# Krabbens/edge-diffusion-tts

Measured on AMD Instinct MI355X. Metric: mel-frames/sec (whole node), 4-step DDIM, hidden=160 L=4, B=256 T=512, higher is better.
Workload: dtype f32

## Files before the change

### edge-diffusion-tts_amd/csrc/edtts_device.h

```cpp
#pragma once
#include <hip/hip_runtime.h>
#include <stdint.h>
#include <type_traits>

#if !defined(EDTTS_EXPERIMENTS) && (                                                                                               \
    defined(EDTTS_ABLATE_QKVSTORES) || defined(EDTTS_ABLATE_KVLOADS) || defined(EDTTS_DIAG) || defined(EDTTS_KV2) ||                \
    defined(EDTTS_H_DMA) || defined(EDTTS_SPLITLOAD) || defined(EDTTS_STAMPS) || defined(EDTTS_DS_ABL) ||                           \
    defined(EDTTS_FAST_BUILD) || defined(EDTTS_W2) || defined(EDTTS_WAVELOG) || defined(EDTTS_PIN_MASK) || defined(EDTTS_HANDOVER) || defined(EDTTS_DS_BURST) || defined(EDTTS16_MFMA_SUM) || defined(EDTTS_DS_STAMPS) || defined(EDTTS_TAIL_RING2) || defined(EDTTS_RB) || defined(EDTTS_WMAX) ||        \
    defined(EDTTS_STAMP_THREAD) || defined(EDTTS_STAMP_HEAD) ||                                                                     \
    defined(EDTTS16_ABLATE_BARRIER) || defined(EDTTS16_ABLATE_DMA) || defined(EDTTS16_PHASES) || defined(EDTTS16_NF) ||             \
    defined(EDTTS16_W1) || defined(EDTTS16_QLDS) || defined(EDTTS16_KVDEPTH) || defined(EDTTS16_IMG) || defined(EDTTS16_HP) ||      \
    defined(EDTTS16_EVEN_STEPS))
#error "tuning / ablation / diagnostic / measured-and-rejected variant switches are scratch-only: add -DEDTTS_EXPERIMENTS"
#endif

#ifndef EDTTS_PIN_MASK
#define EDTTS_PIN_MASK 0x4
#endif
#ifndef EDTTS_W2
#define EDTTS_W2 0
#endif
#if EDTTS_W2
#define EDTTS_PIN_ACC(x) asm volatile("" : "+v"(x))
#else
// ... 57 lines not shown
}

template <int NT, int NF>
EDTTS_DEV void dma_tile_to_lds(const float* src, int ld, f4* lds_wave) {
  typedef __attribute__((address_space(3))) char* lds_char_t;
  const unsigned base = __builtin_amdgcn_readfirstlane((unsigned)(size_t)(lds_char_t)(char*)lds_wave);
#pragma unroll
  for (int nt = 0; nt < NT; ++nt)
#pragma unroll
    for (int ft = 0; ft < NF; ++ft) {
      const float* p = src + 16 * nt + (size_t)ft * 16 * ld;
      asm volatile("s_mov_b32 m0, %1\n\ts_nop 0\n\tglobal_load_lds_dwordx4 %0, off" ::"v"(p), "s"(base + (unsigned)(nt * NF + ft) * 1024u) : "m0", "memory");
    }
}

typedef unsigned u4v __attribute__((ext_vector_type(4)));
typedef unsigned u2v __attribute__((ext_vector_type(2)));
EDTTS_DEV __amdgpu_buffer_rsrc_t make_rsrc(const void* base) {
  return __builtin_amdgcn_make_buffer_rsrc(const_cast<void*>(base), 0, 0xFFFFFFFF, 0x00020000);
}
EDTTS_DEV f4 bufld4(__amdgpu_buffer_rsrc_t r, unsigned voff, unsigned soff) {
  return __builtin_bit_cast(f4, __builtin_amdgcn_raw_buffer_load_b128(r, voff, soff, 0));
}
EDTTS_DEV f2 bufld2(__amdgpu_buffer_rsrc_t r, unsigned voff, unsigned soff) {
  return __builtin_bit_cast(f2, __builtin_amdgcn_raw_buffer_load_b64(r, voff, soff, 0));
}

EDTTS_DEV float sqrt_rn(float x) { return (float)sqrt((double)x); }
EDTTS_DEV float div_rn(float a, float b) { return (float)((double)a / (double)b); }

EDTTS_DEV float group_sum(float v) {
  unsigned u = __float_as_uint(v);
  auto a = __builtin_amdgcn_permlane16_swap(u, u, false, false);
  v = __uint_as_float(a[0]) + __uint_as_float(a[1]);
  u = __float_as_uint(v);
  auto b = __builtin_amdgcn_permlane32_swap(u, u, false, false);
  return __uint_as_float(b[0]) + __uint_as_float(b[1]);
}
EDTTS_DEV float group_max(float v) {
  unsigned u = __float_as_uint(v);
  auto a = __builtin_amdgcn_permlane16_swap(u, u, false, false);
  v = fmaxf(__uint_as_float(a[0]), __uint_as_float(a[1]));
  u = __float_as_uint(v);
  auto b = __builtin_amdgcn_permlane32_swap(u, u, false, false);
  return fmaxf(__uint_as_float(b[0]), __uint_as_float(b[1]));
}
EDTTS_DEV float hsum(f4 v) { return (v[0] + v[1]) + (v[2] + v[3]); }
EDTTS_DEV float hmax(f4 v) { return fmaxf(fmaxf(v[0], v[1]), fmaxf(v[2], v[3])); }

#ifndef EDTTS_RB
#define EDTTS_RB 2
#endif
constexpr int kRefillBurst = EDTTS_RB;
template <int RN>
struct FragRing {
  static constexpr int RN_ = RN;
  __amdgpu_buffer_rsrc_t rs;
  unsigned soff;
  unsigned voff;
  f4 r[RN];
  EDTTS_DEV f4 frag(int i) const {
    return bufld4(rs, voff, soff + (unsigned)i * 1024u);
  }
  EDTTS_DEV void prime(const float* base, int lane) {
    rs = make_rsrc(base);
    soff = 0;
    voff = (unsigned)lane * 16u;
#pragma unroll
    for (int i = 0; i < RN; ++i) r[i] = frag(i);
  }
  EDTTS_DEV const f4& at(int i) const { return r[i % RN]; }
  EDTTS_DEV void refill(int lo, int hi) {
#pragma unroll
    for (int i = lo; i < hi; ++i) r[i % RN] = frag(i + RN);
    __builtin_amdgcn_sched_barrier(0);
  }
  template <int N>
  EDTTS_DEV void refill_after(int i) {
    constexpr int B = kRefillBurst < RN ? kRefillBurst : RN;
    if ((i + 1) % B == 0) refill(i + 1 - B, i + 1);
    else if (i == N - 1) refill(N - N % B, N);
  }
  EDTTS_DEV void advance(int n) { soff += (unsigned)n * 1024u; }
};

template <int KT, int RN, int NF>
EDTTS_DEV void gemm_phase(FragRing<RN>& ring, const f4 (&in)[KT][NF], f4 (&acc)[NF]) {
  static_assert(KT % RN == 0, "phase length must be a multiple of the ring size");
  constexpr bool SPLIT = NF < 4;
  f4 b[NF];
  if (SPLIT) {
#pragma unroll
    for (int ft = 0; ft < NF; ++ft) b[ft] = splat(0.f);
  }
#pragma unroll
  for (int kt = 0; kt < KT; ++kt) {
    const f4& a = ring.at(kt);
#pragma unroll
    for (int r = 0; r < 4; ++r)
#pragma unroll
      for (int ft = 0; ft < NF; ++ft) {
        if (SPLIT && (kt & 1)) b[ft] = EDTTS_MFMA(a[r], in[kt][ft][r], b[ft]);
        else acc[ft] = EDTTS_MFMA(a[r], in[kt][ft][r], acc[ft]);
      }
    ring.template refill_after<KT>(kt);
  }
  if (SPLIT) {
#pragma unroll
    for (int ft = 0; ft < NF; ++ft) acc[ft] += b[ft];
  }
  ring.advance(KT);
}

template <int KT, int RN, int NF>
EDTTS_DEV void gemm_phase_pair(FragRing<RN>& ring, const f4 (&in)[KT][NF], f4 (&a)[NF], f4 (&b)[NF]) {
  static_assert((2 * KT) % RN == 0, "phase length must be a multiple of the ring size");
#pragma unroll
  for (int kt = 0; kt < KT; ++kt) {
    const f4& fa = ring.at(2 * kt);
    const f4& fb = ring.at(2 * kt + 1);
#pragma unroll
    for (int r = 0; r < 4; ++r) {
#pragma unroll
      for (int ft = 0; ft < NF; ++ft) a[ft] = EDTTS_MFMA(fa[r], in[kt][ft][r], a[ft]);
#pragma unroll
      for (int ft = 0; ft < NF; ++ft) b[ft] = EDTTS_MFMA(fb[r], in[kt][ft][r], b[ft]);
    }
    ring.template refill_after<2 * KT>(2 * kt);
    ring.template refill_after<2 * KT>(2 * kt + 1);
  }
  ring.advance(2 * KT);
}

template <int NT, int RN, int NF, int NR = 4>
EDTTS_DEV void ktile_phase(FragRing<RN>& ring, const f4 (&in)[NF], f4 (&acc)[NT][NF]) {
  static_assert(NT % RN == 0, "phase length must be a multiple of the ring size");
  constexpr int STEP = NF < 4 ? 2 : 1;
#pragma unroll
  for (int nt = 0; nt < NT; nt += STEP) {
#pragma unroll
    for (int r = 0; r < NR; ++r)
#pragma unroll
      for (int u = 0; u < STEP; ++u)
        if (nt + u < NT) {
          const f4& fa = ring.at(nt + u);
#pragma unroll
          for (int ft = 0; ft < NF; ++ft) acc[nt + u][ft] = EDTTS_MFMA(fa[r], in[ft][r], acc[nt + u][ft]);
        }
#pragma unroll
    for (int u = 0; u < STEP; ++u)
      if (nt + u < NT) ring.template refill_after<NT>(nt + u);
  }
  ring.advance(NT);
}

template <int NT, int NF>
EDTTS_DEV void rms_norm_tile(const f4 (&x)[NT][NF], const float* __restrict__ w, const float* __restrict__ mod, int g,
                             f4 (&y)[NT][NF]) {
  constexpr int N = NT * 16;
  float rs[NF];
#pragma unroll
  for (int ft = 0; ft < NF; ++ft) {
    float ss = 0.f;
#pragma unroll
    for (int t = 0; t < NT; ++t) ss += hsum(x[t][ft] * x[t][ft]);
    rs[ft] = rsqrtf(group_sum(ss) * (1.0f / N) + 1e-6f);
  }
#pragma unroll
  for (int t = 0; t < NT; ++t) {
    const f4 wv = ldg4(w + 16 * t + 4 * g);
    f4 sc = splat(1.f), sh = splat(0.f);
    if (mod != nullptr) {
      sc = ldg4(mod + 16 * t + 4 * g);
      sh = ldg4(mod + N + 16 * t + 4 * g);
    }
#pragma unroll
    for (int ft = 0; ft < NF; ++ft) {
      f4 a = x[t][ft] * rs[ft] * wv;
      if (mod != nullptr) a = a * sc + sh;
      y[t][ft] = a;
    }
  }
}

template <int NT, int NF>
EDTTS_DEV void layer_norm_tile(const f4 (&x)[NT][NF], const float* __restrict__ w, const float* __restrict__ b, int g,
                               f4 (&y)[NT][NF]) {
  constexpr int N = NT * 16;
  float mu[NF], rs[NF];
#pragma unroll
  for (int ft = 0; ft < NF; ++ft) {
    float s = 0.f;
#pragma unroll
    for (int t = 0; t < NT; ++t) s += hsum(x[t][ft]);
// ... 419 lines not shown
#endif
      };
      const int cd = q.cdiag;
      auto chunk_of = [&](int st) { return st >= nchunk ? nchunk - 1 : (st == 0 ? cd : (st <= cd ? st - 1 : st)); };
#if EDTTS_KV2
      step(No{}, cd, chunk_of(2), KA, VA, hd);
      for (int st = 1; st < nchunk; st += 2) {
        step(Yes{}, chunk_of(st), chunk_of(st + 2), KB, VB, hd);
        if (st + 1 < nchunk) step(Yes{}, chunk_of(st + 1), chunk_of(st + 3), KA, VA, hd);
      }
#else
#ifndef EDTTS_HANDOVER
#define EDTTS_HANDOVER 1
#endif
      constexpr bool HANDOVER = EDTTS_HANDOVER && NHALF == 1;
      const bool more = HANDOVER && hd + hstep < C::HEADS;
      auto req_head = [&](int st) { return (more && st == nchunk - 1) ? hd + hstep : hd; };
      auto req_chunk = [&](int st) { return (more && st == nchunk - 1) ? cd : chunk_of(st + 1); };
      step(No{}, cd, req_chunk(0), KA, VA, req_head(0));
      for (int st = 1; st < nchunk; ++st) step(Yes{}, chunk_of(st), req_chunk(st), KA, VA, req_head(st));
#endif
#pragma unroll
      for (int ft = 0; ft < QT; ++ft) {
        const float lt = group_sum(hsum(lvec[ft]));
        const float inv = lt > 0.f ? 1.0f / lt : 0.f;
#pragma unroll
        for (int dt = 0; dt < DT; ++dt) O[dt][QT * hf + ft] *= inv;
      }
    }
#ifdef EDTTS_STAMPS
    if (hd == STAMP_SEL_HEAD(stamp_sel)) STAMPX(stamps, sidx++, stamp_sel);
#endif
    if (hd + hstep < C::HEADS) {
      if constexpr (EDTTS_HANDOVER && NHALF == 1) {
        load_q(hd + hstep, 0);
        __builtin_amdgcn_sched_barrier(0);
      } else {
        prefetch(geo[0], hd + hstep, 0);
      }
    }
    if constexpr (OMODE != O_FUSED) {
      char* ob = obuf + hd * C::OHEAD_BYTES;
#pragma unroll
      for (int dt = 0; dt < DT; ++dt)
#pragma unroll
        for (int ft = 0; ft < NF; ++ft) {
          if (DREM && dt == DT - 1) reinterpret_cast<f2*>(ob + DFULL * NF * 1024 + ft * 512)[lane] = f2{O[dt][ft][0], O[dt][ft][1]};
          else reinterpret_cast<f4*>(ob + (dt * NF + ft) * 1024)[lane] = O[dt][ft];
        }
    } else {
#pragma unroll
      for (int dt = 0; dt < DT; ++dt) {
        if (DREM && dt == DT - 1) ktile_phase<C::HT, WStream<C>::RN_, NF, 2>(ring, O[dt], h);
        else ktile_phase<C::HT>(ring, O[dt], h);
      }
    }
#ifdef EDTTS_STAMPS
    if (hd == STAMP_SEL_HEAD(stamp_sel)) STAMPX(stamps, sidx++, stamp_sel);
#endif
  }
  if constexpr (OMODE == O_DEFER) {
    before_project();
    for (int hd = 0; hd < C::HEADS; ++hd) {
      const char* ob = obuf + hd * C::OHEAD_BYTES;
#pragma unroll
      for (int dt = 0; dt < DT; ++dt) {
        f4 in[NF];
#pragma unroll
        for (int ft = 0; ft < NF; ++ft) {
          if (DREM && dt == DT - 1) {
            const f2 t = reinterpret_cast<const f2*>(ob + DFULL * NF * 1024 + ft * 512)[lane];
            in[ft] = f4{t[0], t[1], 0.f, 0.f};
          } else {
            in[ft] = reinterpret_cast<const f4*>(ob + (dt * NF + ft) * 1024)[lane];
          }
        }
        if (DREM && dt == DT - 1) ktile_phase<C::HT, WStream<C>::RN_, NF, 2>(ring, in, h);
        else ktile_phase<C::HT>(ring, in, h);
      }
    }
  }
}

EDTTS_DEV void ddim_elem(float x, float e, float s1m, float sab, float sabp, float cdir, float& x0, float& xp) {
#pragma clang fp contract(off)
  float t1 = s1m * e;
  float t2 = x - t1;
  float v = div_rn(t2, sab);
  v = fminf(fmaxf(v, -3.0f), 3.0f);
  x0 = v;
  float t3 = sabp * v;
  float t4 = cdir * e;
  xp = t3 + t4;
}
struct DdimCoef {
  float s1m, sab, sabp, cdir, sigma;
};
EDTTS_DEV DdimCoef ddim_coef(float ab, float abp, float eta) {
#pragma clang fp contract(off)
  DdimCoef c;
  c.s1m = sqrt_rn(1.0f - ab);
  c.sab = sqrt_rn(ab);
  float r1 = div_rn(1.0f - abp, 1.0f - ab);
  float r2 = 1.0f - div_rn(ab, abp);
  float pr = r1 * r2;
  c.sigma = eta * sqrt_rn(pr);
  float s2 = c.sigma * c.sigma;
  float in = 1.0f - abp;
  in = in - s2;
  c.cdir = sqrt_rn(in);
  c.sabp = sqrt_rn(abp);
  return c;
}
EDTTS_DEV float add_mul_rn(float p, float s, float n) {
#pragma clang fp contract(off)
  float t = s * n;
  return p + t;
}

struct DdpmCoef {
  float coef1, coef2, sd;
};
EDTTS_DEV DdpmCoef ddpm_coef(float al, float ab, float be, float var, bool nonzero) {
#pragma clang fp contract(off)
  DdpmCoef c;
  c.coef1 = div_rn(1.0f, sqrt_rn(al));
  float om = 1.0f - ab;
  c.coef2 = div_rn(be, sqrt_rn(om));
  c.sd = (nonzero ? 1.0f : 0.0f) * sqrt_rn(var);
  return c;
}
EDTTS_DEV float ddpm_elem(float x, float e, float n, DdpmCoef c) {
#pragma clang fp contract(off)
  float t1 = c.coef2 * e;
  float t2 = x - t1;
  float mean = c.coef1 * t2;
  float t3 = c.sd * n;
  return mean + t3;
}

struct LmsCoef {
  int mode;
  float p0, p1, c0, c1, rinv, cB, cC;
};
EDTTS_DEV void lms_elem(float x, float out, float h_new, float h_old, const LmsCoef& k, float& x0, float& xn) {
#pragma clang fp contract(off)
  float a = k.p0 * x;
  float b = k.p1 * out;
  float v = a + b;
  v = fminf(fmaxf(v, -3.0f), 3.0f);
  x0 = v;
  float t0 = k.c0 * x;
  float t1 = k.c1 * v;
  float acc = t0 + t1;
  if (k.mode == 2) {
    float d = v - h_new;
    float d1 = k.rinv * d;
    float t2 = k.cB * d1;
    t2 = t2 * 0.5f;
    acc = acc + t2;
  } else if (k.mode == 3) {
    float d1 = v - h_old;
    float two = 2.0f * h_old;
    float d2 = v - two;
    d2 = d2 + h_new;
    float t2 = k.cB * d1;
    t2 = t2 * 0.5f;
    float t3 = k.cC * d2;
    t3 = t3 / 6.0f;
    acc = acc + t2;
    acc = acc + t3;
// ... 114 lines not shown
```

### edge-diffusion-tts_amd/csrc/edtts_generic.h

```cpp
#pragma once

namespace edtts_gen {

enum { EPI_BIAS = 0, EPI_PE = 1, EPI_RESID = 2, EPI_SWIGLU = 3 };

struct GemmArgs {
  const float* X;
  const float* W;
  const float* bias;
  float* Y;
  const float* pe;
  int M, N, K, ldx, ldy, T;
  int vec_x, vec_w, vec_y;
  DropArgs dr;
};
constexpr int kGBM = 64, kGBN = 64, kGBK = 16, kGLd = kGBK + 1;

template <int EPI, bool DROP = false>
__global__ __launch_bounds__(256) void k_gen_gemm(GemmArgs a) {
  __shared__ float xs[kGBM][kGLd];
  __shared__ float ws[kGBN][kGLd];
  const int tid = threadIdx.x, lane = tid & 63, w = tid >> 6, fq = lane & 15, g = lane >> 4;
  const int m0 = blockIdx.x * kGBM;
  const int n0 = blockIdx.y * (EPI == EPI_SWIGLU ? kGBN / 2 : kGBN);
// ... 249 lines not shown
      const f4 dm = drop_attn_keys4(a.dr, (unsigned)(b * gridDim.y + hd), qi, j0 + 4 * g, (lo & 3) == 0);
#pragma unroll
      for (int r = 0; r < 4; ++r) p[r] *= dm[r];
    }
#pragma unroll
    for (int s = 0; s < 4; ++s) {
      const int key = j0 + 4 * g + s;
      const float* vrow = vb + (size_t)(key < hi ? key : 0) * a.ldkv;
#pragma unroll
      for (int t = 0; t < DT; ++t) {
        const int d = 16 * t + fq;
        const float va = (key < hi && d < a.DH) ? vrow[d] : 0.f;
        acc[t] = EDTTS_MFMA(va, p[s], acc[t]);
      }
    }
  }
  if (!qok) return;
  if (a.lse != nullptr && g == 0) a.lse[((size_t)b * gridDim.y + hd) * a.Tq + qi] = m + log2f(l);
  const float inv = 1.0f / l;
  float* orow = a.o + (size_t)(b * a.Tq + qi) * a.ldo + hd * a.DH;
#pragma unroll
  for (int t = 0; t < DT; ++t)
#pragma unroll
    for (int r = 0; r < 4; ++r) {
      const int d = 16 * t + 4 * g + r;
      if (d < a.DH) orow[d] = acc[t][r] * inv;
    }
}

__global__ __launch_bounds__(256) void k_gen_embed(const int64_t* sem_idx, const float* tok, const float* cpe, float* ctx, int rows, int S,
                                                   int H, int n_tok, unsigned* err, const int64_t* s_len) {
  const size_t n = (size_t)rows * H;
  for (size_t i = (size_t)blockIdx.x * blockDim.x + threadIdx.x; i < n; i += (size_t)gridDim.x * blockDim.x) {
    const size_t row = i / H;
    const int c = (int)(i - row * H);
    long tk = (s_len && (int)(row % S) >= utt_len_lane(s_len, (int)(row / S), S)) ? 0 : (long)sem_idx[row];
    if (tk < 0 || tk >= n_tok) {
      if (c == 0) atomicOr(err, (unsigned)EDTTS_IDX_SEM);
      tk = tk < 0 ? 0 : n_tok - 1;
    }
    ctx[i] = tok[(size_t)tk * H + c] + cpe[(size_t)(row % S) * H + c];
  }
}

template <int TAIL>
EDTTS_DEV void tail_elem(const KArgs& a, size_t idx, float e) {
  if (TAIL == TAIL_LMS) {
    const float hn = a.lms.mode >= 2 ? a.h_new[idx] : 0.f, ho = a.lms.mode >= 3 ? a.h_old[idx] : 0.f;
    float v0, vn;
    lms_elem(a.x[idx], e, hn, ho, a.lms, v0, vn);
    a.x0_hist[idx] = v0;
    if (a.x0_all) a.x0_all[idx] = v0;
    a.x_prev[idx] = vn;
  } else if (TAIL == TAIL_VLMS) {
    const float v = a.v_uncond ? cfg_combine(e, a.v_uncond[idx], a.vp.cfg) : e;
    const float hn = a.lms.mode >= 2 ? a.h_new[idx] : 0.f, ho = a.lms.mode >= 3 ? a.h_old[idx] : 0.f;
    float v0, vn;
    lms_elem(a.x[idx], v, hn, ho, a.lms, v0, vn);
    a.x0_hist[idx] = v0;
    if (a.x0_all) a.x0_all[idx] = v0;
    if (a.known != nullptr) {
      const size_t row = (size_t)a.T * a.inj_mel, b = idx / row, r = idx - b * row, per = (size_t)a.inj_frames * a.inj_mel;
      if (r < per) {
        const size_t ki = b * per + r;
        vn = a.known[ki];
        if (a.p_coef2 != 0.f) {
          const float nz = a.noise ? a.noise[ki]
                                   : (a.seeds ? philox_normal4(a.seeds[b], a.step, r >> 2)[(int)(r & 3)] : philox_normal4(a.seed, a.step, ki >> 2)[(int)(ki & 3)]);
          vn = qsample_elem(vn, a.p_coef1, nz, a.p_coef2);
        }
      }
    }
    a.x_prev[idx] = vn;
  } else if (TAIL == TAIL_VPRED) {
    const float v = a.v_uncond ? cfg_combine(e, a.v_uncond[idx], a.vp.cfg) : e;
    a.x_prev[idx] = vpred_elem(a.x[idx], v, a.vp);
  } else if (TAIL == TAIL_DDPM) {
    const unsigned long long ge = a.philox_base + idx;
    const float nz = a.noise ? a.noise[idx] : philox_normal4(a.seed, a.step, ge >> 2)[(int)(ge & 3)];
    const DdpmCoef cf{a.p_coef1, a.p_coef2, a.p_sd};
    a.x_prev[idx] = ddpm_elem(a.x[idx], e, nz, cf);
  } else {
    float v0, vp;
    ddim_elem(a.x[idx], e, a.c_s1m, a.c_sab, a.c_sabp, a.c_dir, v0, vp);
    a.x0[idx] = v0;
    a.x_prev[idx] = vp;
  }
}
template <int TAIL>
EDTTS_DEV void tail_zero_elem(const KArgs& a, size_t idx) {
  if (TAIL == TAIL_LMS || TAIL == TAIL_VLMS) {
    a.x0_hist[idx] = 0.f;
    if (a.x0_all) a.x0_all[idx] = 0.f;
  } else if (TAIL == TAIL_DDIM) {
    a.x0[idx] = 0.f;
  }
  a.x_prev[idx] = 0.f;
}
EDTTS_DEV bool past_len(const int64_t* t_len, bool dbl, size_t idx, int T, int MEL) {
  if (t_len == nullptr) return false;
  const size_t row = idx / MEL;
  return (int)(row % T) >= utt_len_lane(t_len, (int)(row / T), T, dbl);
}
template <int TAIL>
__global__ __launch_bounds__(256) void k_gen_tail(KArgs a, const float* eps, size_t n, int vec, int MEL) {
  const size_t stride = (size_t)gridDim.x * blockDim.x;
  if (vec) {
    for (size_t i = (size_t)blockIdx.x * blockDim.x + threadIdx.x; i < n / 4; i += stride) {
      if constexpr (TAIL == TAIL_VLMS) {
        const size_t row = 4 * i / MEL;
        const int f = (int)(row % a.T);
        const int Tb = a.t_len ? utt_len_of(a.t_len[row / a.T], a.T, a.t_dbl) : a.T;
        tail_store<TAIL>(a, f, Tb, 4 * i, ldg4(eps + 4 * i));
        continue;
      }
      if (past_len(a.t_len, a.t_dbl, 4 * i, a.T, MEL)) tail_zero<TAIL>(a, 4 * i);
      else tail_apply<TAIL>(a, 4 * i, ldg4(eps + 4 * i));
    }
  } else {
    for (size_t i = (size_t)blockIdx.x * blockDim.x + threadIdx.x; i < n; i += stride) {
      if (past_len(a.t_len, a.t_dbl, i, a.T, MEL)) tail_zero_elem<TAIL>(a, i);
      else tail_elem<TAIL>(a, i, eps[i]);
    }
  }
}
__global__ __launch_bounds__(256) void k_gen_zero_past(float* y, const int64_t* t_len, int dbl, size_t n, int T, int MEL) {
  for (size_t i = (size_t)blockIdx.x * blockDim.x + threadIdx.x; i < n; i += (size_t)gridDim.x * blockDim.x)
    if (past_len(t_len, dbl, i, T, MEL)) y[i] = 0.f;
}

}

struct GenericLauncher {
  static int set_attrs() { return EDTTS_OK; }

  static bool al16(const void* p) { return ((uintptr_t)p & 15) == 0; }
  static unsigned grid_1d(size_t n) { const size_t nb = (n + 255) / 256; return (unsigned)(nb > 4096 ? 4096 : (nb < 1 ? 1 : nb)); }
  template <int EPI>
  static int gemm(hipStream_t st, const float* X, int ldx, const float* W, const float* bias, float* Y, int ldy, int M, int N, int K,
                  const float* pe = nullptr, int T = 1, const edtts::DropArgs* dr = nullptr) {
    using namespace edtts_gen;
    GemmArgs a;
    a.X = X; a.W = W; a.bias = bias; a.Y = Y; a.pe = pe; a.M = M; a.N = N; a.K = K; a.ldx = ldx; a.ldy = ldy; a.T = T;
    a.vec_x = (K % 4 == 0) && (ldx % 4 == 0) && al16(X);
    a.vec_w = (K % 4 == 0) && al16(W);
    a.vec_y = (ldy % 4 == 0) && al16(Y);
    const int nb = EPI == EPI_SWIGLU ? kGBN / 2 : kGBN;
    a.dr = dr ? *dr : edtts::DropArgs{};
    const dim3 grid((M + kGBM - 1) / kGBM, (N + nb - 1) / nb);
    if constexpr (EPI == EPI_SWIGLU || EPI == EPI_RESID) {
      if (dr) {
        hipLaunchKernelGGL((k_gen_gemm<EPI, true>), grid, dim3(256), 0, st, a);
        LAUNCH_CHECK("k_gen_gemm");
        return EDTTS_OK;
      }
    }
    hipLaunchKernelGGL(k_gen_gemm<EPI>, grid, dim3(256), 0, st, a);
    LAUNCH_CHECK("k_gen_gemm");
    return EDTTS_OK;
  }
  template <int MODE>
  static int norm(hipStream_t st, const float* x, float* y, int rows, int W, const float* w, const float* b, float eps,
                  const float* mod = nullptr, int rows_per_b = 1, int mod_bstride = 0) {
    edtts_gen::NormArgs a{x, y, w, b, mod, rows, W, W, rows_per_b, mod_bstride, eps};
    hipLaunchKernelGGL(edtts_gen::k_gen_norm<MODE>, dim3((rows + 3) / 4), dim3(256), 0, st, a);
    LAUNCH_CHECK("k_gen_norm");
    return EDTTS_OK;
// ... 121 lines not shown
```

### edge-diffusion-tts_amd/csrc/edtts_kernels.hip

```cpp
#include <hip/hip_runtime.h>
#include <math.h>
#include <stdarg.h>
#include <stdlib.h>
#include <stdio.h>
#include <string.h>

#include "../../include/edtts.h"
#include "edtts_device.h"

using namespace edtts;

static thread_local char g_err[512] = "";
static int fail(int code, const char* fmt, ...) __attribute__((format(printf, 2, 3)));
static int fail(int code, const char* fmt, ...) {
  va_list ap;
  va_start(ap, fmt);
  vsnprintf(g_err, sizeof(g_err), fmt, ap);
  va_end(ap);
  return code;
}
#define HIP_TRY(expr)                                                                                   \
  do {                                                                                                  \
    hipError_t e_ = (expr);                                                                             \
    if (e_ != hipSuccess) return fail(EDTTS_ERR_HIP, "%s failed: %s", #expr, hipGetErrorString(e_));    \
// ... 331 lines not shown
  float* e = sm;
  float* u = sm + a.H;
  const int row = blockIdx.x, tid = threadIdx.x, H = a.H, half = H / 2;
  const float tf = a.use_host ? (float)a.t_host[row] : (float)a.t[row];
  for (int j = tid; j < H; j += blockDim.x) {
    const float arg = tf * a.freqs[j < half ? j : j - half];
    e[j] = j < half ? sinf(arg) : cosf(arg);
  }
  __syncthreads();
  for (int n = tid; n < H; n += blockDim.x) {
    float acc = a.t1b[n];
#pragma unroll 8
    for (int k = 0; k < H; ++k) acc = fmaf(e[k], a.t1T[(size_t)k * H + n], acc);
    u[n] = 0.5f * acc * (1.0f + erff(acc * 0.70710678118654752440f));
  }
  __syncthreads();
  long sidx = -1;
  if (a.use_host ? a.host_has_step : (a.step_idx != nullptr)) {
    sidx = a.use_host ? (long)a.step_host[row] : (long)a.step_idx[row];
    if (sidx < 0 || sidx >= a.n_step) {
      if (tid == 0) atomicOr(a.err, (unsigned)EDTTS_IDX_STEP);
      sidx = sidx < 0 ? 0 : a.n_step - 1;
    }
  }
  for (int n = tid; n < H; n += blockDim.x) {
    float acc = a.t3b[n];
#pragma unroll 8
    for (int k = 0; k < H; ++k) acc = fmaf(u[k], a.t3T[(size_t)k * H + n], acc);
    if (sidx >= 0) acc += a.step[(size_t)sidx * H + n];
    a.tcond[(size_t)row * H + n] = acc;
  }
}
__global__ __launch_bounds__(256) void k_cond_ada(CondArgs a) {
  extern __shared__ float sm[];
  const int row = blockIdx.x, lw = blockIdx.y, l = lw >> 1, which = lw & 1, H = a.H;
  for (int k = threadIdx.x; k < H; k += blockDim.x) sm[k] = a.tcond[(size_t)row * H + k];
  __syncthreads();
  const float* WT = a.blob + (which ? a.ada3T[l] : a.ada1T[l]);
  const float* bb = a.blob + (which ? a.ada3b[l] : a.ada1b[l]);
  float* out = a.cond + (((size_t)row * a.L + l) * 2 + which) * 2 * H;
  for (int n = blockIdx.z * blockDim.x + threadIdx.x; n < 2 * H; n += gridDim.z * blockDim.x) {
    float acc = bb[n];
#pragma unroll 8
    for (int k = 0; k < H; ++k) acc = fmaf(sm[k], WT[(size_t)k * 2 * H + n], acc);
    out[n] = n < H ? 1.0f + acc : acc;
  }
}

struct KArgs {
  int B, T, Tp, S, Sp, window, max_pos, max_cpos, n_tok, SD, L;
  const float* x;
  float* h;
  const float *q, *k, *vT;
  float *q_out, *k_out, *vT_out;
  float *kc, *vcT;
  const float* known;
  const unsigned long long* seeds;
  int inj_frames, inj_mel;
  const int64_t* sem_idx;
  const float* sem_feat;
  const float* cond;
  int cond_bstride;
  int layer;
  int ffn_tiles;
  int diag_skip;
  unsigned long long* stamps;
  const float *tok, *semp, *semp_b, *cpe, *inp, *inp_b, *pe;
  const float *n1w, *proj_b, *n2w, *n3w, *up_b, *down_b, *fnw, *fnb, *outp_b;
  const float* stream;
  float *eps, *x_prev, *x0;
  float c_s1m, c_sab, c_sabp, c_dir;
  float p_coef1, p_coef2, p_sd;
  const float* noise;
  unsigned long long seed;
  unsigned long long philox_base;
  unsigned step;
  LmsCoef lms;
  VpredCoef vp;
  const float* v_uncond;
  const float *h_new, *h_old;
  float *x0_hist, *x0_all;
  const int64_t *t_len, *s_len;
  int t_dbl;
};

EDTTS_DEV int utt_len_of(int64_t v, int full, bool dbl) {
  const int hi = dbl ? full >> 1 : full;
  const int n = v < 1 ? 1 : (v > hi ? hi : (int)v);
  return dbl ? 2 * n : n;
}
EDTTS_DEV int utt_len(const int64_t* len, int b, int full, bool dbl = false) {
  if (len == nullptr) return full;
  return utt_len_of(len[__builtin_amdgcn_readfirstlane(b)], full, dbl);
}
EDTTS_DEV int utt_len_lane(const int64_t* len, int b, int full, bool dbl = false) {
  return len == nullptr ? full : utt_len_of(len[b], full, dbl);
}
EDTTS_DEV int live_end(int n) { return (n + 31) & ~31; }

EDTTS_DEV int remap_block(int bid, int nblk) {
  const int q = nblk >> 3, r = nblk & 7, xcd = bid & 7, idx = bid >> 3;
  const int base = xcd < r ? xcd * (q + 1) : r * (q + 1) + (xcd - r) * q;
  return base + idx;
}

struct TileId {
  int b, m0;
  bool valid;
};
EDTTS_DEV TileId wave_tile(int B, int Tp, int waves_per_block, int wave_frames) {
  const int wave = __builtin_amdgcn_readfirstlane(threadIdx.x >> 6);
  const int tpu = Tp / wave_frames;
  int w = remap_block(blockIdx.x, gridDim.x) * waves_per_block + wave;
  TileId t;
  t.valid = w < B * tpu;
  w = t.valid ? w : B * tpu - 1;
  t.b = w / tpu;
  t.m0 = (w - t.b * tpu) * wave_frames;
  return t;
}

#ifndef EDTTS_TAIL_RING2
#define EDTTS_TAIL_RING2 1
#endif
template <class C>
EDTTS_DEV void qkv_tail(WStream<C>& ring0, const f4 (&hn)[C::HT][C::NF], const KArgs& a, int b, int m0, int lane) {
  constexpr int NF = C::NF;
  static_assert(C::HT % 2 == 0, "hidden must be a multiple of 32 (n-tile pairs)");
#if EDTTS_TAIL_RING2
  constexpr int RN0 = WStream<C>::RN_;
  static_assert((2 * C::HT) % (2 * RN0) == 0, "a pair phase must be a whole number of turns of the doubled ring");
  FragRing<2 * RN0> ring;
  ring.rs = ring0.rs; ring.soff = ring0.soff; ring.voff = ring0.voff;
#pragma unroll
  for (int i = 0; i < RN0; ++i) ring.r[i] = ring0.at(i);
#pragma unroll
  for (int i = RN0; i < 2 * RN0; ++i) ring.r[i] = ring.frag(i);
  __builtin_amdgcn_sched_barrier(0);
#else
  WStream<C>& ring = ring0;
#endif
  const int fq = lane & 15, g = lane >> 4;
  const size_t rowbase = (size_t)b * a.Tp + m0 + fq;
#pragma unroll
  for (int which = 0; which < 3; ++which) {
    for (int nt = 0; nt < C::HT; nt += 2) {
      f4 acc[2][NF];
#pragma unroll
      for (int ft = 0; ft < NF; ++ft) acc[0][ft] = acc[1][ft] = splat(0.f);
      gemm_phase_pair<C::HT>(ring, hn, acc[0], acc[1]);
#ifdef EDTTS_ABLATE_QKVSTORES
      if (a.T > 0) continue;
#endif
#pragma unroll
      for (int u = 0; u < 2; ++u) {
        if (which < 2) {
          float* dst = (which == 0 ? a.q_out : a.k_out) + rowbase * C::H + 16 * (nt + u) + 4 * g;
#pragma unroll
          for (int ft = 0; ft < NF; ++ft) {
            __builtin_nontemporal_store(acc[u][ft], reinterpret_cast<f4*>(dst + (size_t)ft * 16 * C::H));
          }
        } else {
          float* dst = a.vT_out + ((size_t)b * C::VR + 16 * (nt + u) + 4 * g) * a.Tp + m0 + fq;
#pragma unroll
          for (int r = 0; r < 4; ++r)
#pragma unroll
            for (int ft = 0; ft < NF; ++ft) {
              __builtin_nontemporal_store(acc[u][ft][r], dst + (size_t)r * a.Tp + 16 * ft);
            }
        }
      }
    }
  }
}

template <class C>
__global__ __launch_bounds__(C::THREADS) void k_prologue(KArgs a) {
  constexpr int NF = C::NF;
  const TileId tl = wave_tile(a.B, a.Tp, C::WAVES, C::WF);
  if (!tl.valid) return;
  const int lane = threadIdx.x & 63, fq = lane & 15, g = lane >> 4;
  const int b = tl.b, m0 = tl.m0;
  const int Tb = utt_len(a.t_len, b, a.T, a.t_dbl);
  if (m0 >= live_end(Tb)) return;
  WStream<C> ring;
  ring.prime(a.stream, lane);
  f4 xin[C::MT][NF];
#pragma unroll
  for (int ft = 0; ft < NF; ++ft) {
    const int f = m0 + 16 * ft + fq;
#pragma unroll
    for (int t = 0; t < C::MT; ++t)
      xin[t][ft] = f < Tb ? ldg4(a.x + ((size_t)b * a.T + f) * C::MEL + 16 * t + 4 * g) : splat(0.f);
  }
  f4 h[C::HT][NF];
#pragma unroll
  for (int nt = 0; nt < C::HT; ++nt) {
    const f4 bias = ldg4(a.inp_b + 16 * nt + 4 * g);
#pragma unroll
    for (int ft = 0; ft < NF; ++ft) h[nt][ft] = bias;
  }
  {
    constexpr int N = C::HT * C::MT;
    static_assert(N % WStream<C>::RN_ == 0 && C::HT % 2 == 0, "in_proj must be a whole number of ring turns");
#pragma unroll
    for (int nt = 0; nt < C::HT; nt += 2)
#pragma unroll
      for (int kt = 0; kt < C::MT; ++kt) {
        const int i = nt * C::MT + 2 * kt;
        const f4& fa = ring.at(i);
        const f4& fb = ring.at(i + 1);
#pragma unroll
        for (int r = 0; r < 4; ++r) {
#pragma unroll
          for (int ft = 0; ft < NF; ++ft) h[nt][ft] = EDTTS_MFMA(fa[r], xin[kt][ft][r], h[nt][ft]);
#pragma unroll
          for (int ft = 0; ft < NF; ++ft) h[nt + 1][ft] = EDTTS_MFMA(fb[r], xin[kt][ft][r], h[nt + 1][ft]);
        }
        ring.template refill_after<N>(i);
        ring.template refill_after<N>(i + 1);
      }
    ring.advance(N);
  }
#pragma unroll
  for (int ft = 0; ft < NF; ++ft) {
    int f = m0 + 16 * ft + fq;
    f = f < a.max_pos ? f : a.max_pos - 1;
#pragma unroll
    for (int nt = 0; nt < C::HT; ++nt) h[nt][ft] += ldg4(a.pe + (size_t)f * C::H + 16 * nt + 4 * g);
  }
  {
    float* hp = a.h + ((size_t)b * a.Tp + m0 + fq) * C::H + 4 * g;
#pragma unroll
    for (int nt = 0; nt < C::HT; ++nt)
#pragma unroll
      for (int ft = 0; ft < NF; ++ft) stg4(hp + 16 * nt + (size_t)ft * 16 * C::H, h[nt][ft]);
  }
  f4 hn[C::HT][NF];
  const float* mod = a.cond + (size_t)b * a.cond_bstride;
  rms_norm_tile<C::HT, NF>(h, a.n1w, mod, g, hn);
  qkv_tail<C>(ring, hn, a, b, m0, lane);
}

enum { TAIL_QKV = 0, TAIL_EPS = 1, TAIL_DDIM = 2, TAIL_DDPM = 3, TAIL_LMS = 4, TAIL_VPRED = 5, TAIL_VLMS = 6 };

template <int TAIL>
EDTTS_DEV void tail_apply(const KArgs& a, size_t idx, f4 ev, bool blend = false) {
  if (TAIL == TAIL_EPS) {
    stg4(a.eps + idx, ev);
  } else if (TAIL == TAIL_LMS) {
    const f4 xv = ldg4(a.x + idx);
    f4 hn = splat(0.f), ho = splat(0.f);
    if (a.lms.mode >= 2) hn = ldg4(a.h_new + idx);
    if (a.lms.mode >= 3) ho = ldg4(a.h_old + idx);
    f4 x0, xn;
#pragma unroll
    for (int r = 0; r < 4; ++r) {
      float v0, vn;
      lms_elem(xv[r], ev[r], hn[r], ho[r], a.lms, v0, vn);
      x0[r] = v0;
      xn[r] = vn;
    }
    stg4(a.x0_hist + idx, x0);
    if (a.x0_all) stg4(a.x0_all + idx, x0);
    stg4(a.x_prev + idx, xn);
  } else if (TAIL == TAIL_VLMS) {
    const bool guided = a.v_uncond != nullptr;
    const f4 xv = ldg4(a.x + idx);
    const f4 vu = ldg4((guided ? a.v_uncond : a.x) + idx);
    f4 hn = splat(0.f), ho = splat(0.f);
    if (a.lms.mode >= 2) hn = ldg4(a.h_new + idx);
    if (a.lms.mode >= 3) ho = ldg4(a.h_old + idx);
    f4 x0, xn;
#pragma unroll
    for (int r = 0; r < 4; ++r) {
      const float v = guided ? cfg_combine(ev[r], vu[r], a.vp.cfg) : ev[r];
      float v0, vn;
      lms_elem(xv[r], v, hn[r], ho[r], a.lms, v0, vn);
      x0[r] = v0;
      xn[r] = vn;
    }
    stg4(a.x0_hist + idx, x0);
    if (a.x0_all) stg4(a.x0_all + idx, x0);
    if (!blend) stg4(a.x_prev + idx, xn);
  } else if (TAIL == TAIL_VPRED) {
    const bool guided = a.v_uncond != nullptr;
    const f4 xv = ldg4(a.x + idx);
    const f4 vu = ldg4((guided ? a.v_uncond : a.x) + idx);
    f4 v, xn;
#pragma unroll
    for (int r = 0; r < 4; ++r) v[r] = guided ? cfg_combine(ev[r], vu[r], a.vp.cfg) : ev[r];
#pragma unroll
    for (int r = 0; r < 4; ++r) xn[r] = vpred_elem(xv[r], v[r], a.vp);
    stg4(a.x_prev + idx, xn);
  } else if (TAIL == TAIL_DDPM) {
    const f4 xv = ldg4(a.x + idx);
    const f4 nz = a.noise ? ldg4(a.noise + idx) : philox_normal4(a.seed, a.step, (a.philox_base + idx) >> 2);
    const DdpmCoef cf{a.p_coef1, a.p_coef2, a.p_sd};
    f4 xp;
#pragma unroll
    for (int r = 0; r < 4; ++r) xp[r] = ddpm_elem(xv[r], ev[r], nz[r], cf);
    stg4(a.x_prev + idx, xp);
  } else {
    const f4 xv = ldg4(a.x + idx);
    f4 x0, xp;
#pragma unroll
    for (int r = 0; r < 4; ++r) {
      float v0, vp;
      ddim_elem(xv[r], ev[r], a.c_s1m, a.c_sab, a.c_sabp, a.c_dir, v0, vp);
      x0[r] = v0;
      xp[r] = vp;
    }
    stg4(a.x0 + idx, x0);
    stg4(a.x_prev + idx, xp);
  }
}
template <int TAIL>
EDTTS_DEV void tail_zero(const KArgs& a, size_t idx) {
  const f4 z = splat(0.f);
  if (TAIL == TAIL_EPS) {
    stg4(a.eps + idx, z);
  } else if (TAIL == TAIL_LMS || TAIL == TAIL_VLMS) {
    stg4(a.x0_hist + idx, z);
    if (a.x0_all) stg4(a.x0_all + idx, z);
    stg4(a.x_prev + idx, z);
  } else if (TAIL == TAIL_DDIM) {
    stg4(a.x0 + idx, z);
    stg4(a.x_prev + idx, z);
  } else {
    stg4(a.x_prev + idx, z);
  }
}
EDTTS_DEV void vlms_blend(const KArgs& a, size_t idx) {
  const size_t row = (size_t)a.T * a.inj_mel, b = idx / row, r = idx - b * row;
  const size_t ki = b * ((size_t)a.inj_frames * a.inj_mel) + r;
  const f4 kv = ldg4(a.known + ki);
  f4 o = kv;
  if (a.p_coef2 != 0.f) {
    const unsigned long long sd = a.seeds ? a.seeds[b] : a.seed;
    const f4 nz = a.noise ? ldg4(a.noise + ki) : philox_normal4(sd, a.step, (a.seeds ? r : ki) >> 2);
#pragma unroll
    for (int e = 0; e < 4; ++e) o[e] = qsample_elem(kv[e], a.p_coef1, nz[e], a.p_coef2);
  }
  stg4(a.x_prev + idx, o);
}
template <int TAIL>
EDTTS_DEV void tail_store(const KArgs& a, int f, int Tb, size_t idx, f4 ev) {
  if constexpr (TAIL == TAIL_VLMS) {
    const bool blend = a.known != nullptr && f < Tb && f < a.inj_frames;
    if (f < Tb) tail_apply<TAIL>(a, idx, ev, blend);
    else tail_zero<TAIL>(a, idx);
    if (blend) vlms_blend(a, idx);
  } else {
    if (f < Tb) tail_apply<TAIL>(a, idx, ev);
    else tail_zero<TAIL>(a, idx);
  }
}

struct QGlobal {
  __amdgpu_buffer_rsrc_t rs;
  unsigned v4, v2;
  int H;
  EDTTS_DEV QGlobal(const float* row_m0, int H_, int fq, int g) : rs(make_rsrc(row_m0)), v4((unsigned)(fq * H_ + 4 * g) * 4u), v2((unsigned)(fq * H_ + 2 * g) * 4u), H(H_) {}
  EDTTS_DEV f4 q4(int ft, int col) const { return bufld4(rs, v4, (unsigned)(ft * 16 * H + col) * 4u); }
  EDTTS_DEV f2 q2(int ft, int col) const { return bufld2(rs, v2, (unsigned)(ft * 16 * H + col) * 4u); }
};
struct QLds {
  const float* b4;
  const float* b2;
  int ld;
  EDTTS_DEV QLds(const float* tile, int ld_, int fq, int g) : b4(tile + fq * ld_ + 4 * g), b2(tile + fq * ld_ + 2 * g), ld(ld_) {}
  EDTTS_DEV f4 q4(int ft, int col) const { return *reinterpret_cast<const f4*>(b4 + ft * 16 * ld + col); }
  EDTTS_DEV f2 q2(int ft, int col) const { return *reinterpret_cast<const f2*>(b2 + ft * 16 * ld + col); }
};

template <class C, int TAIL>
EDTTS_DEV void layer_tile(const KArgs& a, float* smem, int wave, int lane, int b, int m0, int Tb, int Sb) {
  constexpr int NF = C::NF;
  const int fq = lane & 15, g = lane >> 4;
  f4* const stash = reinterpret_cast<f4*>(smem) + (size_t)wave * C::HT * NF * 64 + lane;
  char* const obuf = reinterpret_cast<char*>(smem) + (size_t)wave * C::HT * NF * 1024;
  static_assert(!C::DEFER || C::HEADS * C::OHEAD_BYTES <= C::HT * NF * 1024, "attention outputs must fit the wave's parking place");
  constexpr int QLDS = C::H;
  float* qtile = smem + (size_t)C::WAVES * C::HT * NF * 256 + (size_t)wave * C::WF * QLDS;
  const size_t rowbase = (size_t)b * a.Tp + m0 + fq;

  STAMPX(a.stamps, 0, a.diag_skip);
  WStream<C> ring;
  ring.prime(a.stream, lane);

  f4 h[C::HT][NF];
  float* const hp = a.h + rowbase * C::H + 4 * g;
  auto park_h = [&]() {
#pragma unroll
    for (int nt = 0; nt < C::HT; ++nt)
#pragma unroll
      for (int ft = 0; ft < NF; ++ft) stash[(nt * NF + ft) * 64] = h[nt][ft];
  };
  auto add_parked_h = [&]() {
#pragma unroll
    for (int nt = 0; nt < C::HT; ++nt)
#pragma unroll
      for (int ft = 0; ft < NF; ++ft) h[nt][ft] += stash[(nt * NF + ft) * 64];
  };
#ifdef EDTTS_DIAG
#define DIAG_ON(bit) (!(a.diag_skip & (bit)))
#else
#define DIAG_ON(bit) true
#endif
  {
#ifndef EDTTS_H_DMA
#define EDTTS_H_DMA 0
#endif
#if EDTTS_H_DMA
    dma_tile_to_lds<C::HT, NF>(hp, C::H, reinterpret_cast<f4*>(smem) + (size_t)wave * C::HT * NF * 64);
#else
    if constexpr (!C::DEFER) {
#pragma unroll
      for (int nt = 0; nt < C::HT; ++nt)
#pragma unroll
        for (int ft = 0; ft < NF; ++ft) h[nt][ft] = ldg4(hp + 16 * nt + (size_t)ft * 16 * C::H);
      park_h();
    }
#endif
    auto init_proj_bias = [&]() {
#pragma unroll
      for (int nt = 0; nt < C::HT; ++nt) {
        const f4 pb = ldg4(a.proj_b + 16 * nt + 4 * g);
#pragma unroll
        for (int ft = 0; ft < NF; ++ft) h[nt][ft] = pb;
      }
    };
    if constexpr (!C::DEFER) init_proj_bias();
    if (DIAG_ON(1)) {
      QGlobal ql(a.q + ((size_t)b * a.Tp + m0) * C::H, C::H, fq, g);
      attention_fused<C, true, C::DEFER ? O_DEFER : O_FUSED>(ql, a.k + (size_t)b * a.Tp * C::H, a.vT + (size_t)b * C::VR * a.Tp, a.Tp, Tb, a.window, m0,
                               lane, ring, h, obuf, init_proj_bias, a.stamps ? a.stamps + 8 : nullptr, a.diag_skip);
    }
    if constexpr (C::DEFER) {
// ... 18 lines not shown
      } else {
        park_h();
      }
      for (int nt = 0; nt < C::HT; nt += 2) {
        f4 acc[2][NF];
#pragma unroll
        for (int ft = 0; ft < NF; ++ft) acc[0][ft] = acc[1][ft] = splat(0.f);
        gemm_phase_pair<C::HT>(ring, hn, acc[0], acc[1]);
#pragma unroll
        for (int u = 0; u < 2; ++u)
#pragma unroll
          for (int ft = 0; ft < NF; ++ft) {
            if (C::Q_IN_LDS) stg4(qtile + (16 * ft + fq) * QLDS + 16 * (nt + u) + 4 * g, acc[u][ft]);
            else stg4(const_cast<float*>(a.q) + (rowbase + 16 * ft) * C::H + 16 * (nt + u) + 4 * g, acc[u][ft]);
          }
      }
    }
    STAMPX(a.stamps, 2, a.diag_skip);
    auto zero_h = [&]() {
#pragma unroll
      for (int nt = 0; nt < C::HT; ++nt)
#pragma unroll
        for (int ft = 0; ft < NF; ++ft) h[nt][ft] = splat(0.f);
    };
    if constexpr (!C::DEFER) zero_h();
    if constexpr (C::Q_IN_LDS) {
      QLds ql(qtile, QLDS, fq, g);
      attention_fused<C, false, C::DEFER ? O_DEFER : O_FUSED>(ql, a.kc + (size_t)b * a.Sp * C::H, a.vcT + (size_t)b * C::VR * a.Sp, a.Sp, Sb, -1, m0, lane,
                                ring, h, obuf, zero_h, a.stamps ? a.stamps + 40 : nullptr, a.diag_skip);
    } else {
      QGlobal ql(a.q + ((size_t)b * a.Tp + m0) * C::H, C::H, fq, g);
      attention_fused<C, false, C::DEFER ? O_DEFER : O_FUSED>(ql, a.kc + (size_t)b * a.Sp * C::H, a.vcT + (size_t)b * C::VR * a.Sp, a.Sp, Sb, -1, m0, lane,
                                ring, h, obuf, zero_h);
    }
    if constexpr (C::DEFER) {
#pragma unroll
      for (int nt = 0; nt < C::HT; ++nt)
#pragma unroll
        for (int ft = 0; ft < NF; ++ft) h[nt][ft] += ldg4(hp + 16 * nt + (size_t)ft * 16 * C::H);
    } else {
      add_parked_h();
    }
    STAMPX(a.stamps, 3, a.diag_skip);
  }
  if (DIAG_ON(4)) {
    f4 hn[C::HT][NF];
    const float* mod = a.cond + (size_t)b * a.cond_bstride + ((size_t)a.layer * 2 + 1) * 2 * C::H;
    rms_norm_tile<C::HT, NF>(h, a.n3w, mod, g, hn);
    park_h();
#pragma unroll
    for (int nt = 0; nt < C::HT; ++nt) {
      const f4 db = ldg4(a.down_b + 16 * nt + 4 * g);
#pragma unroll
      for (int ft = 0; ft < NF; ++ft) h[nt][ft] = db;
    }
    for (int j = 0; j < a.ffn_tiles; ++j) {
      const f4 vb = ldg4(a.up_b + 32 * j + 4 * g), gb = ldg4(a.up_b + 32 * j + 16 + 4 * g);
      f4 v[NF], gt[NF], act[NF];
#pragma unroll
      for (int ft = 0; ft < NF; ++ft) v[ft] = gt[ft] = splat(0.f);
      gemm_phase_pair<C::HT>(ring, hn, v, gt);
      __builtin_amdgcn_sched_barrier(0);
#pragma unroll
      for (int ft = 0; ft < NF; ++ft) act[ft] = swiglu_tile(v[ft], gt[ft], vb, gb);
      __builtin_amdgcn_sched_barrier(0);
      ktile_phase<C::HT>(ring, act, h);
    }
    add_parked_h();
    STAMPX(a.stamps, 4, a.diag_skip);
  }
  if (!DIAG_ON(8)) return;
  if (TAIL == TAIL_QKV) {
    {
      float* hp = a.h + rowbase * C::H + 4 * g;
#pragma unroll
      for (int nt = 0; nt < C::HT; ++nt)
#pragma unroll
        for (int ft = 0; ft < NF; ++ft) stg4(hp + 16 * nt + (size_t)ft * 16 * C::H, h[nt][ft]);
    }
    const float* mod = a.cond + (size_t)b * a.cond_bstride + ((size_t)(a.layer + 1) * 2) * 2 * C::H;
    rms_norm_tile<C::HT, NF>(h, a.n1w, mod, g, h);
    qkv_tail<C>(ring, h, a, b, m0, lane);
  } else {
    f4 hn[C::HT][NF];
    layer_norm_tile<C::HT, NF>(h, a.fnw, a.fnb, g, hn);
#pragma unroll
    for (int nt = 0; nt < C::MT; ++nt) {
      const f4 ob = ldg4(a.outp_b + 16 * nt + 4 * g);
      f4 e[NF];
#pragma unroll
      for (int ft = 0; ft < NF; ++ft) e[ft] = splat(0.f);
      gemm_phase<C::HT>(ring, hn, e);
#pragma unroll
      for (int ft = 0; ft < NF; ++ft) {
        const int f = m0 + 16 * ft + fq;
        if (f >= a.T) continue;
        const size_t idx = ((size_t)b * a.T + f) * C::MEL + 16 * nt + 4 * g;
        tail_store<TAIL>(a, f, Tb, idx, e[ft] + ob);
      }
    }
  }
  STAMPX(a.stamps, 5, a.diag_skip);
#ifdef EDTTS_STAMPS
  asm volatile("s_waitcnt vmcnt(0)" ::: "memory");
#endif
  STAMPX(a.stamps, 6, a.diag_skip);
}

template <class C, int TAIL>
EDTTS_DEV void tail_zero_tile(const KArgs& a, int b, int m0, int lane) {
  const int fq = lane & 15, g = lane >> 4;
#pragma unroll
  for (int ft = 0; ft < C::NF; ++ft) {
    const int f = m0 + 16 * ft + fq;
    if (f >= a.T) continue;
#pragma unroll
    for (int nt = 0; nt < C::MT; ++nt) tail_zero<TAIL>(a, ((size_t)b * a.T + f) * C::MEL + 16 * nt + 4 * g);
  }
}
template <class C, int TAIL>
__global__ __launch_bounds__(C::THREADS, C::DEFER ? 2 : 1) void k_layer(KArgs a) {
  extern __shared__ __attribute__((aligned(16))) float smem[];
  const int lane = threadIdx.x & 63;
  const int wave = __builtin_amdgcn_readfirstlane(threadIdx.x >> 6);
  const TileId tl = wave_tile(a.B, a.Tp, C::WAVES, C::WF);
  if (!tl.valid) return;
  const int Tb = utt_len(a.t_len, tl.b, a.T, a.t_dbl);
  if (tl.m0 >= live_end(Tb)) {
    if constexpr (TAIL != TAIL_QKV) tail_zero_tile<C, TAIL>(a, tl.b, tl.m0, lane);
    return;
  }
  const int Sb = utt_len(a.s_len, tl.b, a.S);
#ifdef EDTTS_WAVELOG
  const unsigned long long wl_r0 = __builtin_amdgcn_s_memrealtime(), wl_c0 = __builtin_amdgcn_s_memtime();
#endif
  layer_tile<C, TAIL>(a, smem, wave, lane, tl.b, tl.m0, Tb, Sb);
#ifdef EDTTS_WAVELOG
  if (a.stamps && lane == 0) {
    asm volatile("s_waitcnt vmcnt(0)" ::: "memory");
    unsigned long long* p = a.stamps + 6 * ((size_t)a.diag_skip + (size_t)tl.b * (a.Tp / C::WF) + tl.m0 / C::WF);
    p[0] = wl_r0; p[1] = wl_c0; p[2] = __builtin_amdgcn_s_memrealtime(); p[3] = __builtin_amdgcn_s_memtime();
    p[4] = __builtin_amdgcn_s_getreg((31 << 11) | 4);
    p[5] = __builtin_amdgcn_s_getreg((31 << 11) | 20);
  }
#endif
}

#include "edtts_coop.h"
#include "edtts_bf16.h"
#include "edtts_melpost.h"

struct CtxArgs {
  int B, S, Sp, L, SD, n_tok, max_cpos;
  const int64_t* sem_idx;
  const float* sem_feat;
  const float *tok, *semp, *semp_b, *cpe;
  const float* blob;
  unsigned kvd[kMaxLayers], kvn[kMaxLayers], kvu[kMaxLayers];
  float *kc, *vcT;
  unsigned* err;
  const float* stream16;
  const int64_t* s_len;
};
template <class C>
__global__ __launch_bounds__(64 * kCtxWaves) void k_ctx(CtxArgs a) {
  const TileId tl = wave_tile(a.B, a.Sp, kCtxWaves, 32);
  if (!tl.valid) return;
  const int lane = threadIdx.x & 63, fq = lane & 15, g = lane >> 4;
  const int b = tl.b, m0 = tl.m0;
  const int Sb = utt_len(a.s_len, b, a.S);
  if (m0 >= live_end(Sb)) return;
  f4 ctx[C::HT][2];
  if (a.sem_feat != nullptr) {
    const int KT = a.SD / 16;
    const f4* wp = reinterpret_cast<const f4*>(a.semp) + lane;
#pragma unroll
    for (int nt = 0; nt < C::HT; ++nt) ctx[nt][0] = ctx[nt][1] = ldg4(a.semp_b + 16 * nt + 4 * g);
    for (int kt = 0; kt < KT; ++kt) {
      f4 xin[2];
#pragma unroll
      for (int ft = 0; ft < 2; ++ft) {
        const int s = m0 + 16 * ft + fq;
        xin[ft] = s < Sb ? ldg4(a.sem_feat + ((size_t)b * a.S + s) * a.SD + 16 * kt + 4 * g) : splat(0.f);
      }
#pragma unroll
      for (int nt = 0; nt < C::HT; ++nt) {
        const f4 w = wp[(nt * KT + kt) * 64];
#pragma unroll
        for (int r = 0; r < 4; ++r) {
          ctx[nt][0] = EDTTS_MFMA(w[r], xin[0][r], ctx[nt][0]);
          ctx[nt][1] = EDTTS_MFMA(w[r], xin[1][r], ctx[nt][1]);
        }
      }
    }
  } else {
#pragma unroll
    for (int ft = 0; ft < 2; ++ft) {
      const int s = m0 + 16 * ft + fq;
      long tk = s < Sb ? (long)a.sem_idx[(size_t)b * a.S + s] : 0;
      if (tk < 0 || tk >= a.n_tok) {
        atomicOr(a.err, (unsigned)EDTTS_IDX_SEM);
        tk = tk < 0 ? 0 : a.n_tok - 1;
      }
      const float* row = a.tok + (size_t)tk * C::H + 4 * g;
#pragma unroll
      for (int nt = 0; nt < C::HT; ++nt) ctx[nt][ft] = ldg4(row + 16 * nt);
    }
  }
#pragma unroll
  for (int ft = 0; ft < 2; ++ft) {
    int s = m0 + 16 * ft + fq;
    s = s < a.max_cpos ? s : a.max_cpos - 1;
// ... 119 lines not shown
#pragma unroll
      for (int ft = 0; ft < 2; ++ft) {
        float ss = 0.f;
#pragma unroll
        for (int t = 0; t < RT; ++t) ss += hsum(c[t][ft] * c[t][ft]);
        rs[ft] = rsqrtf(group_sum(ss) * (1.0f / C::R) + 1e-6f);
      }
      const float* w = a.blob + a.kvn[l];
#pragma unroll
      for (int kt = 0; kt < RK; ++kt) {
        const f4 w0 = ldg4(w + 32 * kt + 4 * g), w1 = ldg4(w + 32 * kt + 16 + 4 * g);
#pragma unroll
        for (int ft = 0; ft < 2; ++ft) cn[kt][ft] = pack8(c[2 * kt][ft] * rs[ft] * w0, c[2 * kt + 1][ft] * rs[ft] * w1);
      }
    }
    __bf16* const kimg = reinterpret_cast<__bf16*>(a.kc) + ((size_t)l * a.B + b) * a.Sp * C::H;
    __bf16* const vimg = reinterpret_cast<__bf16*>(a.vcT) + ((size_t)l * a.B + b) * a.Sp * C::H;
    for (int ph = 0; ph < 2 * C::HEADS / PPP; ++ph) {
      const lds_cf4_t fr = phase_base(ring.acquire());
      f4 fg[C::PH];
#pragma unroll
      for (int i = 0; i < C::PH; ++i) fg[i] = fr[i * 64];
      __builtin_amdgcn_sched_barrier(0);
      const bool isv = ph >= C::HEADS / PPP;
#pragma unroll
      for (int pp = 0; pp < PPP; ++pp) {
        const int head = (isv ? ph - C::HEADS / PPP : ph) * PPP + pp;
        f4 acc[2][2] = {{splat(0.f), splat(0.f)}, {splat(0.f), splat(0.f)}};
        if (!isv) {
#pragma unroll
          for (int kt = 0; kt < RK; ++kt)
#pragma unroll
            for (int u = 0; u < 2; ++u)
#pragma unroll
              for (int ft = 0; ft < 2; ++ft)
                acc[u][ft] = EDTTS_MFMA16(as_bf8(fg[pp * 2 * RK + 2 * kt + u]), cn[kt][ft], acc[u][ft]);
          __bf16* d = kimg + head * hstride + (size_t)(m0 >> 4) * 512 + fq * 32 + 8 * g;
          if (valid)
#pragma unroll
            for (int ft = 0; ft < 2; ++ft) *reinterpret_cast<f4*>(d + ft * 512) = as_f4(pack8(acc[0][ft], acc[1][ft]));
        } else {
#pragma unroll
          for (int kt = 0; kt < RK; ++kt)
#pragma unroll
            for (int u = 0; u < 2; ++u)
#pragma unroll
              for (int ft = 0; ft < 2; ++ft)
                acc[u][ft] = EDTTS_MFMA16(cn[kt][ft], as_bf8(fg[pp * 2 * RK + 2 * kt + u]), acc[u][ft]);
          __bf16* d = vimg + head * hstride + (size_t)(m0 >> 5) * 1024 + fq * 32 + 8 * g;
          if (valid)
#pragma unroll
            for (int u = 0; u < 2; ++u) *reinterpret_cast<f4*>(d + u * 512) = as_f4(pack8(acc[u][0], acc[u][1]));
        }
      }
    }
  }
  ring.drain();
}


struct StepArgs {
  const float *alphas, *alpha_bar, *betas, *post_var;
  int n_table;
  const float *x, *eps, *noise;
  const int64_t *t, *t_prev;
  size_t n_per_batch;
  float eta;
  float *x_prev, *x0;
  int vec4;
};
static int step_vec4(size_t n_per_batch, std::initializer_list<const void*> ptrs) {
  uintptr_t m = 0;
  for (const void* p : ptrs) m |= (uintptr_t)p;
  return (n_per_batch & 3) == 0 && (m & 15) == 0;
}
EDTTS_DEV long clamp_idx(long v, int n) { return v < 0 ? 0 : (v >= n ? n - 1 : v); }

__global__ __launch_bounds__(256) void k_ddim(StepArgs a) {
  const int b = blockIdx.y;
  const float ab = a.alpha_bar[clamp_idx((long)a.t[b], a.n_table)];
  const long tp = (long)a.t_prev[b];
  const float abp = tp >= 0 ? a.alpha_bar[clamp_idx(tp, a.n_table)] : 1.0f;
  const DdimCoef cf = ddim_coef(ab, abp, a.eta);
  const float s1m = cf.s1m, sab = cf.sab, sabp = cf.sabp, cdir = cf.cdir, sigma = cf.sigma;
  const size_t base = (size_t)b * a.n_per_batch;
  const size_t n4 = a.vec4 ? a.n_per_batch >> 2 : 0;
  for (size_t i = (size_t)blockIdx.x * blockDim.x + threadIdx.x; i < n4; i += (size_t)gridDim.x * blockDim.x) {
    const size_t o = base + 4 * i;
    const f4 xv = ldg4(a.x + o), e = ldg4(a.eps + o);
    f4 nz = splat(0.f);
    if (a.noise) nz = ldg4(a.noise + o);
    f4 x0, xp;
#pragma unroll
    for (int r = 0; r < 4; ++r) {
      float v, p;
      ddim_elem(xv[r], e[r], s1m, sab, sabp, cdir, v, p);
      if (a.noise) p = add_mul_rn(p, sigma, nz[r]);
      x0[r] = v;
      xp[r] = p;
    }
    stg4(a.x0 + o, x0);
    stg4(a.x_prev + o, xp);
  }
  for (size_t i = (n4 << 2) + (size_t)blockIdx.x * blockDim.x + threadIdx.x; i < a.n_per_batch; i += (size_t)gridDim.x * blockDim.x) {
    const size_t o = base + i;
    float v, p;
    ddim_elem(a.x[o], a.eps[o], s1m, sab, sabp, cdir, v, p);
    if (a.noise) p = add_mul_rn(p, sigma, a.noise[o]);
    a.x0[o] = v;
    a.x_prev[o] = p;
  }
}

__global__ __launch_bounds__(256) void k_ddpm(StepArgs a) {
  const int b = blockIdx.y;
  const long tt = clamp_idx((long)a.t[b], a.n_table);
  const float al = a.alphas[tt], ab = a.alpha_bar[tt], be = a.betas[tt];
  const DdpmCoef cf = ddpm_coef(al, ab, be, a.post_var[tt], (long)a.t[b] > 0);
  const size_t base = (size_t)b * a.n_per_batch;
  const size_t n4 = a.vec4 ? a.n_per_batch >> 2 : 0;
  for (size_t i = (size_t)blockIdx.x * blockDim.x + threadIdx.x; i < n4; i += (size_t)gridDim.x * blockDim.x) {
    const size_t o = base + 4 * i;
    const f4 xv = ldg4(a.x + o), e = ldg4(a.eps + o), nz = ldg4(a.noise + o);
    f4 xp;
#pragma unroll
    for (int r = 0; r < 4; ++r) xp[r] = ddpm_elem(xv[r], e[r], nz[r], cf);
    stg4(a.x_prev + o, xp);
  }
  for (size_t i = (n4 << 2) + (size_t)blockIdx.x * blockDim.x + threadIdx.x; i < a.n_per_batch; i += (size_t)gridDim.x * blockDim.x) {
    const size_t o = base + i;
    a.x_prev[o] = ddpm_elem(a.x[o], a.eps[o], a.noise[o], cf);
  }
}

constexpr int kDsTileT = 64, kDsLd = kDsTileT + 4;
__global__ __launch_bounds__(256) void k_dsconv_pw(const float* __restrict__ x, const float* __restrict__ dw, const float* __restrict__ pw,
                                                   const float* __restrict__ pb, int B, int Ci, int Co, int Tin, int T, int ks, int stride,
                                                   float* __restrict__ z) {
  extern __shared__ float dsm[];
  const int b = blockIdx.y, t0 = blockIdx.x * kDsTileT, pad = ks / 2;
  const int Cip = (Ci + 15) & ~15;
  for (int i = threadIdx.x; i < Cip * kDsTileT; i += blockDim.x) {
    const int ci = i / kDsTileT, tl = i % kDsTileT, tt = t0 + tl;
    float acc = 0.f;
    if (ci < Ci && tt < T) {
      const float* xr = x + ((size_t)b * Ci + ci) * Tin;
      for (int j = 0; j < ks; ++j) {
        const int ts = tt * stride + j - pad;
        if (ts >= 0 && ts < Tin) acc = fmaf(xr[ts], dw[ci * ks + j], acc);
      }
    }
    dsm[ci * kDsLd + tl] = acc;
  }
  __syncthreads();
  const int lane = threadIdx.x & 63, wave = threadIdx.x >> 6, fq = lane & 15, g = lane >> 4;
  const int tl = 16 * wave + fq, tt = t0 + tl;
  const int KT = Cip >> 4;
  constexpr int kMaxKT = 16;
  f4 bt[kMaxKT];
#pragma unroll
  for (int kt = 0; kt < kMaxKT; ++kt) {
    if (kt < KT) {
#pragma unroll
      for (int r = 0; r < 4; ++r) bt[kt][r] = dsm[(16 * kt + 4 * g + r) * kDsLd + tl];
    }
  }
  for (int co0 = 0; co0 < Co; co0 += 16) {
    const int row = co0 + fq;
    const float* wr = pw + (size_t)(row < Co ? row : Co - 1) * Ci;
    f4 acc = splat(0.f);
#pragma unroll
    for (int kt = 0; kt < kMaxKT; ++kt) {
      if (kt < KT) {
        const int c0 = 16 * kt + 4 * g;
        f4 a;
        if (row < Co && c0 + 3 < Ci && (Ci & 3) == 0) a = ldg4(wr + c0);
        else {
#pragma unroll
          for (int r = 0; r < 4; ++r) a[r] = (row < Co && c0 + r < Ci) ? wr[c0 + r] : 0.f;
        }
#pragma unroll
        for (int r = 0; r < 4; ++r) acc = EDTTS_MFMA(a[r], bt[kt][r], acc);
      }
    }
    if (tt < T) {
#pragma unroll
      for (int r = 0; r < 4; ++r) {
        const int co = co0 + 4 * g + r;
        if (co < Co) z[((size_t)b * Co + co) * T + tt] = acc[r] + pb[co];
      }
// ... 625 lines not shown
      }
    });
    DS_SUB(t, 7);
    dsg_static_for<0, t + 1>([&](auto uc) {
      constexpr int tt = decltype(uc)::value;
      if constexpr ((CPG * ((16 * tt + 15) / CPG) + CPG - 1) / 16 == t) store_tile(tt);
    });
    DS_SUB(t, 8);
    DS_TILE(t);
  });
#ifdef EDTTS_DS_STAMPS
  __builtin_amdgcn_s_waitcnt(0);
  DS_STAMP(13);
  if (threadIdx.x == 0) g_ds_stamps[blockIdx.x * 16 + 15] = __builtin_amdgcn_s_memrealtime();
#endif
}

struct Workspace {
  size_t err, h, q, k, vT, kc, vcT, cond, total;
  size_t g_xn, g_big, g_att, g_ctx, g_cr, g_kv, g_eps;
  int Tp, Sp, VR;
  unsigned* errp;
};
constexpr int kWaveFrames = 32;

static void make_workspace(const Layout& lo, int B, int T, int S, int cond_rows, Workspace* w) {
  const size_t H = lo.H;
  if (lo.GEN) {
    memset(w, 0, sizeof(*w));
    w->Tp = T; w->Sp = S; w->VR = lo.H;
    const size_t M = (size_t)B * T, CS = (size_t)B * S, FH = (size_t)lo.FM * H;
    size_t o = 0;
    auto take = [&](size_t n) { size_t r = o; o = align64(o + n); return r; };
    w->err = take(64);
    w->h = take(M * H); w->g_xn = take(M * H); w->g_big = take(M * (FH > 3 * H ? FH : 3 * H)); w->g_att = take(M * H);
    w->g_ctx = take(CS * H); w->g_cr = take(CS * lo.R); w->g_kv = take((size_t)lo.L * CS * 2 * H); w->g_eps = take(M * lo.MEL);
    w->cond = take((size_t)cond_rows * lo.L * 2 * 2 * H + (size_t)cond_rows * H);
    w->total = o;
    w->errp = nullptr;
    return;
  }
  w->Tp = (T + kWaveFrames - 1) / kWaveFrames * kWaveFrames;
  w->Sp = (S + 31) / 32 * 32;
  w->VR = (lo.HEADS - 1) * lo.DH + lo.DHP;
  size_t o = 0;
  auto take = [&](size_t n) { size_t r = o; o = align64(o + n); return r; };
  w->err = take(64);
  const size_t es = lo.BF16 ? 2 : 1;
  w->h = take((size_t)B * w->Tp * H);
  w->q = take((size_t)2 * B * w->Tp * H / es);
  w->k = take((size_t)2 * B * w->Tp * H / es);
  w->vT = take((size_t)2 * B * w->VR * w->Tp / es);
  w->kc = take((size_t)lo.L * B * w->Sp * H / es);
  w->vcT = take((size_t)lo.L * B * w->VR * w->Sp / es);
  w->cond = take((size_t)cond_rows * lo.L * 2 * 2 * H + (size_t)cond_rows * H);
  w->total = o;
  w->errp = nullptr;
}

static int device_simds() {
  static std::atomic<int> n[64];
  int dev = 0;
  if (hipGetDevice(&dev) != hipSuccess || dev < 0 || dev >= 64) return 1024;
  int v = n[dev].load(std::memory_order_relaxed);
  if (!v) {
    int cus = 0;
    v = (hipDeviceGetAttribute(&cus, hipDeviceAttributeMultiprocessorCount, dev) == hipSuccess && cus > 0) ? 4 * cus : 1024;
    n[dev].store(v, std::memory_order_relaxed);
  }
  return v;
}

constexpr int kMaxSub = 8;
struct SubBatches {
  int n;
  int B[kMaxSub], off[kMaxSub];
  Workspace ws[kMaxSub];
  size_t base[kMaxSub];
  size_t cond;
  size_t total;
};
static std::atomic<int> g_coop{[] { const char* e = getenv("EDTTS_COOP"); return e ? atoi(e) : -1; }()};
static std::atomic<int> g_substreams{[] { const char* e = getenv("EDTTS_SUBSTREAMS"); const int v = e ? atoi(e) : 4; return v < 1 ? 1 : (v > kMaxSub ? kMaxSub : v); }()};
struct Settings {
  int substreams, coop;
};
static thread_local const Settings* t_settings = nullptr;
struct SettingsScope {
  Settings snap;
  const Settings* prev;
  SettingsScope() : snap{g_substreams.load(std::memory_order_relaxed), g_coop.load(std::memory_order_relaxed)}, prev(t_settings) {
    t_settings = &snap;
  }
  ~SettingsScope() { t_settings = prev; }
};
static Settings current_settings() {
  return t_settings ? *t_settings : Settings{g_substreams.load(std::memory_order_relaxed), g_coop.load(std::memory_order_relaxed)};
}

static void plan_sub(const Layout& lo, int B, int T, int S, int cond_rows, int n, SubBatches* sb) {
  sb->n = n;
  if (n == 1) {
    make_workspace(lo, B, T, S, cond_rows, &sb->ws[0]);
    sb->B[0] = B; sb->off[0] = 0; sb->base[0] = 0; sb->cond = sb->ws[0].cond; sb->total = sb->ws[0].total;
    return;
  }
  size_t o = 0;
  int off = 0;
  for (int j = 0; j < n; ++j) {
    sb->B[j] = B / n + (j < B % n ? 1 : 0);
    sb->off[j] = off;
    off += sb->B[j];
    make_workspace(lo, sb->B[j], T, S, 1, &sb->ws[j]);
    sb->base[j] = o;
    o += sb->ws[j].total;
  }
  sb->cond = o;
  sb->total = align64(o + (size_t)cond_rows * lo.L * 2 * 2 * lo.H + (size_t)cond_rows * lo.H);
}
static int substreams_for(const Layout& lo, int B, int T, int S) {
  if (lo.GEN) return 1;
  Workspace w;
  make_workspace(lo, 1, T, S, 1, &w);
  const long waves = (long)B * (w.Tp / 32), slots = device_simds();
  const int max_sub = current_settings().substreams;
  if (max_sub < 2 || B < 2 || waves < 2 * slots) return 1;
  long n = waves / (2 * slots);
  if (n < 2) n = 2;
  if (n > max_sub) n = max_sub;
  if (n > B) n = B;
  return (int)n;
}
static void plan_call(const Layout& lo, int B, int T, int S, int cond_rows, float* wsb, SubBatches* sb) {
  plan_sub(lo, B, T, S, cond_rows, substreams_for(lo, B, T, S), sb);
  for (int j = 0; j < sb->n; ++j) sb->ws[j].errp = reinterpret_cast<unsigned*>(wsb);
}

struct SideStream {
  int dev = -1;
  hipStream_t caller = nullptr;
  bool bound = false;
  unsigned long long last_use = 0;
  hipStream_t s[kMaxSub - 1] = {};
  hipEvent_t fork = nullptr, join[kMaxSub - 1] = {};
};
constexpr int kSideSets = 8;
static std::mutex g_side_pool_mu;
static std::vector<SideStream>& side_pool() {
  static auto* pool = new std::vector<SideStream>;
  return *pool;
}
struct ThreadSides {
  SideStream set[kSideSets];
  unsigned long long tick = 0;
  ~ThreadSides() {
    std::lock_guard<std::mutex> lock(g_side_pool_mu);
    for (SideStream& sd : set)
      if (sd.dev >= 0) release(sd);
  }
  static void release(SideStream& sd) {
    sd.bound = false;
    side_pool().push_back(sd);
    sd = SideStream();
  }
  SideStream& get(int dev, hipStream_t caller) {
    SideStream* pick = nullptr;
    for (SideStream& sd : set) {
      if (sd.bound && sd.dev == dev && sd.caller == caller) { pick = &sd; break; }
      if (!pick || (pick->bound && (!sd.bound || sd.last_use < pick->last_use))) pick = &sd;
    }
    if (!(pick->bound && pick->dev == dev && pick->caller == caller)) {
      if (pick->dev != dev) {
        std::lock_guard<std::mutex> lock(g_side_pool_mu);
        if (pick->dev >= 0) release(*pick);
        auto& pool = side_pool();
        for (size_t i = 0; i < pool.size(); ++i)
          if (pool[i].dev == dev) {
            *pick = pool[i];
            pool.erase(pool.begin() + (long)i);
            break;
          }
      }
      pick->caller = caller;
      pick->bound = true;
    }
    pick->last_use = ++tick;
    return *pick;
  }
};
static thread_local ThreadSides g_sides;
struct ForkJoin {
  hipStream_t st[kMaxSub];
  SideStream* side = nullptr;
  int n = 1;
  int init(const SubBatches& sb, hipStream_t main) {
    for (int j = 0; j < kMaxSub; ++j) st[j] = main;
    if (sb.n < 2) return EDTTS_OK;
    int dev = 0;
    HIP_TRY(hipGetDevice(&dev));
    if (dev < 0 || dev >= 64) return fail(EDTTS_ERR_UNSUPPORTED, "device ordinal %d out of range", dev);
    SideStream& sd = g_sides.get(dev, main);
    sd.dev = dev;
    if (!sd.fork) HIP_TRY(hipEventCreateWithFlags(&sd.fork, hipEventDisableTiming));
    for (int j = 0; j + 1 < sb.n; ++j) {
      if (!sd.s[j]) HIP_TRY(hipStreamCreateWithFlags(&sd.s[j], hipStreamNonBlocking));
      if (!sd.join[j]) HIP_TRY(hipEventCreateWithFlags(&sd.join[j], hipEventDisableTiming));
    }
    HIP_TRY(hipEventRecord(sd.fork, main));
    side = &sd;
    for (int j = 0; j + 1 < sb.n; ++j) {
      HIP_TRY(hipStreamWaitEvent(sd.s[j], sd.fork, 0));
      st[j + 1] = sd.s[j];
      n = j + 2;
    }
    return EDTTS_OK;
  }
  ~ForkJoin() {
    if (side)
      for (int j = 0; j + 1 < n; ++j) {
        (void)hipEventRecord(side->join[j], side->s[j]);
        (void)hipStreamWaitEvent(st[0], side->join[j], 0);
      }
  }
};

constexpr unsigned kStreamDdpmStep = 0x10000u;
constexpr unsigned kStreamInpaintStep = 0x20000u;
struct DdpmStepArgs {
  const float* noise;
  unsigned long long seed, base;
  unsigned step;
};
struct VpredStepArgs {
  VpredCoef k;
  const float* v_uncond;
};
struct LmsStepArgs {
  LmsCoef k;
  const float *h_new, *h_old;
  float *x0_hist, *x0_all;
};
struct BlendStepArgs {
  const float *known, *noise;
  int frames, mel;
  float c_known, c_noise;
  unsigned long long seed;
  const unsigned long long* seeds;
  unsigned step;
};
struct StepTail {
  int kind = TAIL_EPS;
  float* eps = nullptr;
  float* x_prev = nullptr;
  float* x0 = nullptr;
  const float* coef = nullptr;
  DdpmStepArgs ddpm{};
  LmsStepArgs lms{};
  VpredStepArgs vp{};
  BlendStepArgs blend{};
};
static void set_tail_args(const StepTail& t, KArgs* a) {
  if (t.kind == TAIL_EPS) {
    a->eps = t.eps;
    return;
  }
  a->x_prev = t.x_prev;
  if (t.kind == TAIL_LMS || t.kind == TAIL_VLMS) {
    a->lms = t.lms.k; a->h_new = t.lms.h_new; a->h_old = t.lms.h_old; a->x0_hist = t.lms.x0_hist; a->x0_all = t.lms.x0_all;
    if (t.kind == TAIL_LMS) return;
    a->vp = t.vp.k; a->v_uncond = t.vp.v_uncond;
    a->known = t.blend.known; a->noise = t.blend.noise; a->inj_frames = t.blend.frames; a->inj_mel = t.blend.mel;
    a->p_coef1 = t.blend.c_known; a->p_coef2 = t.blend.c_noise; a->seed = t.blend.seed; a->seeds = t.blend.seeds; a->step = t.blend.step;
  } else if (t.kind == TAIL_VPRED) {
    a->vp = t.vp.k; a->v_uncond = t.vp.v_uncond;
  } else if (t.kind == TAIL_DDPM) {
    a->p_coef1 = t.coef[0]; a->p_coef2 = t.coef[1]; a->p_sd = t.coef[2];
    a->noise = t.ddpm.noise; a->seed = t.ddpm.seed; a->philox_base = t.ddpm.base; a->step = t.ddpm.step;
  } else {
    a->x0 = t.x0;
    a->c_s1m = t.coef[0]; a->c_sab = t.coef[1]; a->c_sabp = t.coef[2]; a->c_dir = t.coef[3];
  }
}
template <class F>
static int with_tail(int kind, F&& f) {
  switch (kind) {
    case TAIL_QKV: return f(std::integral_constant<int, TAIL_QKV>{});
    case TAIL_EPS: return f(std::integral_constant<int, TAIL_EPS>{});
    case TAIL_LMS: return f(std::integral_constant<int, TAIL_LMS>{});
    case TAIL_DDPM: return f(std::integral_constant<int, TAIL_DDPM>{});
    case TAIL_VPRED: return f(std::integral_constant<int, TAIL_VPRED>{});
    case TAIL_VLMS: return f(std::integral_constant<int, TAIL_VLMS>{});
    default: return f(std::integral_constant<int, TAIL_DDIM>{});
  }
}
#define TRY_G(x) do { int rc_ = (x); if (rc_) return rc_; } while (0)
#define TRY(x) do { int rc_ = (x); if (rc_) return rc_; } while (0)
template <class F>
static int for_each_tail(F&& f) {
  for (int kind : {TAIL_QKV, TAIL_EPS, TAIL_DDIM, TAIL_DDPM, TAIL_LMS, TAIL_VPRED, TAIL_VLMS}) TRY_G(with_tail(kind, f));
  return EDTTS_OK;
}
struct Lens {
  const int64_t *t = nullptr, *s = nullptr;
  bool t_dbl = false;
  Lens at(int off) const { return Lens{t ? t + off : nullptr, s ? s + off : nullptr, t_dbl}; }
};
struct CallCtx {
  const Layout& lo;
  const float* blob;
  Workspace ws;
  float* wsb;
  int B, T, S, window;
  Lens ln;
  hipStream_t st;
};

#ifdef EDTTS_STAMPS
static unsigned long long* g_stamps_fwd = nullptr;
#endif
#ifdef EDTTS_WAVELOG
static unsigned long long* g_wavelog = nullptr;
static thread_local int g_wavelog_base = 0;
#endif

static CtxArgs ctx_args(const CallCtx& c, const int64_t* sem_idx, const float* sem_feat) {
  const Layout& lo = c.lo;
  CtxArgs a;
  memset(&a, 0, sizeof(a));
  a.B = c.B; a.S = c.S; a.Sp = c.ws.Sp; a.L = lo.L; a.SD = lo.SD; a.n_tok = lo.NTOK; a.max_cpos = lo.MAXCPOS;
  a.sem_idx = sem_idx; a.sem_feat = sem_feat; a.s_len = c.ln.s;
  a.tok = c.blob + lo.tok; a.semp = c.blob + lo.semp; a.semp_b = c.blob + lo.semp_b; a.cpe = c.blob + lo.cpe; a.blob = c.blob;
  for (int l = 0; l < lo.L; ++l) {
    a.kvd[l] = (unsigned)lo.layer[l].kvd; a.kvn[l] = (unsigned)lo.layer[l].kvn; a.kvu[l] = (unsigned)lo.layer[l].kvu;
  }
  a.kc = c.wsb + c.ws.kc; a.vcT = c.wsb + c.ws.vcT;
  a.err = c.ws.errp ? c.ws.errp : reinterpret_cast<unsigned*>(c.wsb + c.ws.err);
  return a;
}

template <int ES>
struct ForwardArgs {
  KArgs a;
  const CallCtx& c;
  size_t qk_set, v_set;
  ForwardArgs(const CallCtx& c_, const float* x, const float* cond_row, int cond_bstride) : c(c_) {
    const Layout& lo = c.lo;
    const float* blob = c.blob;
    memset(&a, 0, sizeof(a));
    a.B = c.B; a.T = c.T; a.Tp = c.ws.Tp; a.S = c.S; a.Sp = c.ws.Sp; a.window = c.window; a.max_pos = lo.MAXPOS;
    a.max_cpos = lo.MAXCPOS; a.n_tok = lo.NTOK; a.SD = lo.SD; a.L = lo.L; a.ffn_tiles = lo.FM * lo.HT;
    a.h = c.wsb + c.ws.h;
    a.inp = blob + lo.inp; a.inp_b = blob + lo.inp_b; a.pe = blob + lo.pe;
    a.fnw = blob + lo.fnw; a.fnb = blob + lo.fnb; a.outp_b = blob + lo.outp_b;
#ifdef EDTTS_DIAG
    const char* e = getenv("EDTTS_DIAG_SKIP");
    a.diag_skip = e ? atoi(e) : 0;
#endif
#ifdef EDTTS_STAMPS
    {
      auto env = [](const char* n, int d) { const char* e = getenv(n); return e ? atoi(e) : d; };
      a.diag_skip = env("EDTTS_STAMP_HEAD", 1) | (env("EDTTS_STAMP_WAVE", 0) << 8) | (env("EDTTS_STAMP_BLOCK", 8) << 16);
    }
#endif
    a.x = x; a.cond = cond_row; a.cond_bstride = cond_bstride;
    a.t_len = c.ln.t; a.s_len = c.ln.s; a.t_dbl = c.ln.t_dbl;
    qk_set = (size_t)c.B * c.ws.Tp * lo.H / ES;
    v_set = (size_t)c.B * c.ws.VR * c.ws.Tp / ES;
    set_qkv(1, 0);
    a.n1w = blob + lo.layer[0].n1w; a.stream = blob + lo.inp; a.layer = 0;
  }
  void set_qkv(int in_set, int out_set) {
    const Workspace& ws = c.ws;
    a.q = c.wsb + ws.q + in_set * qk_set; a.k = c.wsb + ws.k + in_set * qk_set; a.vT = c.wsb + ws.vT + in_set * v_set;
    a.q_out = c.wsb + ws.q + out_set * qk_set; a.k_out = c.wsb + ws.k + out_set * qk_set; a.vT_out = c.wsb + ws.vT + out_set * v_set;
  }
  int layer(int l, const StepTail& tail) {
    const Layout& lo = c.lo;
    const LayerLayout& y = lo.layer[l];
    a.layer = l;
    set_qkv(l & 1, (l + 1) & 1);
    a.proj_b = c.blob + y.proj_b; a.n2w = c.blob + y.n2w; a.n3w = c.blob + y.n3w; a.up_b = c.blob + y.up_b;
    a.down_b = c.blob + y.down_b; a.stream = c.blob + y.s_body;
    a.kc = c.wsb + c.ws.kc + (size_t)l * c.B * c.ws.Sp * lo.H / ES;
    a.vcT = c.wsb + c.ws.vcT + (size_t)l * c.B * c.ws.VR * c.ws.Sp / ES;
#ifdef EDTTS_WAVELOG
    a.stamps = g_wavelog ? g_wavelog + (size_t)6 * 8192 * l : nullptr;
    a.diag_skip = g_wavelog_base;
#endif
#ifdef EDTTS_STAMPS
    a.stamps = g_stamps_fwd ? g_stamps_fwd + 128 * l : nullptr;
#endif
    if (l + 1 < lo.L) {
      a.n1w = c.blob + lo.layer[l + 1].n1w;
      return TAIL_QKV;
    }
    set_tail_args(tail, &a);
    return tail.kind;
  }
};

template <class LN>
static int set_attrs_once() {
  static std::atomic<bool> done[64];
  int dev = 0;
  HIP_TRY(hipGetDevice(&dev));
  if (dev < 0 || dev >= 64) return fail(EDTTS_ERR_UNSUPPORTED, "device ordinal %d out of range", dev);
  if (done[dev].load(std::memory_order_acquire)) return EDTTS_OK;
  TRY_G(LN::set_attrs());
  done[dev].store(true, std::memory_order_release);
  return EDTTS_OK;
}

template <class C>
struct Launcher {
  static size_t occupancy_lds() { return C::DEFER ? 0 : (size_t)C::WAVES * 40 * 1024; }
  static size_t ring_lds() { return occupancy_lds(); }
  template <class CC> static size_t stash_lds() { return (size_t)CC::WAVES * CC::HT * CC::NF * 1024; }
  static size_t layer_lds() {
    const size_t need = stash_lds<C>() + (C::Q_IN_LDS ? (size_t)C::WAVES * C::WF * C::H * sizeof(float) : 0);
    return need > occupancy_lds() ? need : occupancy_lds();
  }
  static int grid(int B, int Tp) { return (B * (Tp / C::WF) + C::WAVES - 1) / C::WAVES; }
  static int ctx_grid(int B, int Sp) { return (B * (Sp / 32) + kCtxWaves - 1) / kCtxWaves; }
  using C2 = Cfg<C::H, C::HEADS, C::MEL, 2>;
  static constexpr bool HAS_SMALL = C::NF == 2 && (C::H == 160 || C::H == 256);
  using Small = Cfg<C::H, C::HEADS, C::MEL, 1>;
  static int wave_slots() { return device_simds(); }

  static int ctx(const CallCtx& c, const int64_t* sem_idx, const float* sem_feat) {
    const CtxArgs a = ctx_args(c, sem_idx, sem_feat);
    const int gx = ctx_grid(c.B, c.ws.Sp);
    const int gy = (gx * 4 <= wave_slots() / 4) ? c.lo.L : 1;
    hipLaunchKernelGGL(k_ctx<C2>, dim3(gx, gy), dim3(64 * kCtxWaves), 0, c.st, a);
    LAUNCH_CHECK("k_ctx");
    return EDTTS_OK;
  }

  static constexpr bool HAS_COOP = C::NF == 2 && ((C::H == 160 && C::HEADS == 4) || (C::H == 256 && C::HEADS == 8)) && C::MEL == 80;
  static constexpr bool HAS_CO22 = HAS_COOP && Coop<C, 2>::FITS;
  static int coop_choice(int B, int Tp) {
    int co = current_settings().coop;
    if (co < 0) {
      const int t32 = B * (Tp / 32), slots = wave_slots();
      co = 8 * t32 <= slots ? 14 : (4 * t32 <= slots ? 24 : (2 * t32 <= slots ? 22 : 0));
    }
    return (co == 22 && !HAS_CO22) ? 0 : co;
  }
  template <int COW = 0>
  static int forward(const CallCtx& c, const float* x, const float* cond_row, int cond_bstride, const StepTail& tail) {
    if constexpr (HAS_COOP && COW == 0) {
      const int co = coop_choice(c.B, c.ws.Tp);
      if (co == 14) return Launcher<Small>::template forward<4>(c, x, cond_row, cond_bstride, tail);
      if (co == 24) return forward<4>(c, x, cond_row, cond_bstride, tail);
      if constexpr (HAS_CO22) {
        if (co == 22) return forward<2>(c, x, cond_row, cond_bstride, tail);
      }
    }
    if constexpr (HAS_SMALL && COW == 0) {
      if (2 * c.B * (c.ws.Tp / C::WF) <= wave_slots())
        return Launcher<Small>::template forward<0>(c, x, cond_row, cond_bstride, tail);
    }
    ForwardArgs<1> f(c, x, cond_row, cond_bstride);
    const KArgs& a = f.a;
    const hipStream_t st = c.st;
    const int g = grid(c.B, c.ws.Tp);
    if constexpr (COW != 0) {
      hipLaunchKernelGGL((k_prologue_co<C, COW>), dim3(c.B * (c.ws.Tp / C::WF)), dim3(64 * COW), C::HT * C::NF * 1024, st, a);
    } else {
      hipLaunchKernelGGL(k_prologue<C>, dim3(g), dim3(C::THREADS), ring_lds(), st, a);
    }
    LAUNCH_CHECK("k_prologue");
    for (int l = 0; l < c.lo.L; ++l) {
      TRY_G(with_tail(f.layer(l, tail), [&](auto t) -> int {
        constexpr int TL = decltype(t)::value;
        if constexpr (COW != 0) {
          using CO = Coop<C, COW>;
          const int tiles = c.B * (c.ws.Tp / C::WF);
          PROF_LAUNCH(st, hipLaunchKernelGGL((k_layer_co<C, TL, COW>), dim3((tiles + CO::TILES - 1) / CO::TILES), dim3(CO::THREADS), CO::LDS_BYTES, st, a));
        } else {
          PROF_LAUNCH(st, hipLaunchKernelGGL((k_layer<C, TL>), dim3(g), dim3(C::THREADS), layer_lds(), st, a));
        }
        LAUNCH_CHECK("k_layer");
        return EDTTS_OK;
      }));
    }
    return EDTTS_OK;
  }

  static int set_attrs() {
    if constexpr (HAS_SMALL) TRY_G(Launcher<Small>::set_attrs());
    const int lds = (int)layer_lds();
    HIP_TRY(hipFuncSetAttribute((const void*)k_prologue<C>, hipFuncAttributeMaxDynamicSharedMemorySize, (int)ring_lds()));
    return for_each_tail([&](auto t) -> int {
      constexpr int TL = decltype(t)::value;
      HIP_TRY(hipFuncSetAttribute((const void*)k_layer<C, TL>, hipFuncAttributeMaxDynamicSharedMemorySize, lds));
      if constexpr (HAS_COOP) {
        HIP_TRY(hipFuncSetAttribute((const void*)k_layer_co<Small, TL, 4>, hipFuncAttributeMaxDynamicSharedMemorySize, Coop<Small, 4>::LDS_BYTES));
        HIP_TRY(hipFuncSetAttribute((const void*)k_layer_co<C, TL, 4>, hipFuncAttributeMaxDynamicSharedMemorySize, Coop<C, 4>::LDS_BYTES));
        if constexpr (HAS_CO22)
          HIP_TRY(hipFuncSetAttribute((const void*)k_layer_co<C, TL, 2>, hipFuncAttributeMaxDynamicSharedMemorySize, Coop<C, 2>::LDS_BYTES));
      }
      return EDTTS_OK;
    });
  }
};

#ifndef EDTTS16_NF
#define EDTTS16_NF 2
#endif
template <class C>
struct Launcher16 {
  static int grid(int B, int Tp) { return (B * (Tp / C::WF) + C::WAVES - 1) / C::WAVES; }
  static constexpr bool HAS_SMALL = C::NF == 2 && C::H == 256;
  using Small = edtts16::Cfg16<C::H, C::HEADS, C::MEL, 1>;
  static int simds() { return device_simds(); }
  static int set_attrs() {
    if constexpr (HAS_SMALL) TRY_G(Launcher16<Small>::set_attrs());
    const int lds = C::LDS_BYTES;
    HIP_TRY(hipFuncSetAttribute((const void*)edtts16::k_prologue16<C>, hipFuncAttributeMaxDynamicSharedMemorySize, lds));
    if constexpr (C::NF == 2) HIP_TRY(hipFuncSetAttribute((const void*)k_ctx16<C>, hipFuncAttributeMaxDynamicSharedMemorySize, lds));
    return for_each_tail([&](auto t) -> int {
      HIP_TRY(hipFuncSetAttribute((const void*)edtts16::k_layer16<C, decltype(t)::value>, hipFuncAttributeMaxDynamicSharedMemorySize, lds));
      return EDTTS_OK;
    });
  }
  static int ctx(const CallCtx& c, const int64_t* sem_idx, const float* sem_feat) {
    if constexpr (C::NF == 2) {
      CtxArgs a = ctx_args(c, sem_idx, sem_feat);
      a.stream16 = c.blob + c.lo.s_ctx16;
      hipLaunchKernelGGL((k_ctx16<C>), dim3((c.B * (c.ws.Sp / 32) + C::WAVES - 1) / C::WAVES), dim3(C::THREADS), C::LDS_BYTES, c.st, a);
      LAUNCH_CHECK("k_ctx16");
      return EDTTS_OK;
    } else {
      return fail(EDTTS_ERR_UNSUPPORTED, "internal: context cache requested from the 16-frame launcher");
    }
  }
  static int forward(const CallCtx& c, const float* x, const float* cond_row, int cond_bstride, const StepTail& tail) {
    if constexpr (HAS_SMALL) {
      if (2 * c.B * (c.ws.Tp / C::WF) <= simds())
        return Launcher16<Small>::forward(c, x, cond_row, cond_bstride, tail);
    }
    ForwardArgs<2> f(c, x, cond_row, cond_bstride);
    const KArgs& a = f.a;
    const hipStream_t st = c.st;
    const int g = grid(c.B, c.ws.Tp);
    hipLaunchKernelGGL(edtts16::k_prologue16<C>, dim3(g), dim3(C::THREADS), C::LDS_BYTES, st, a);
    LAUNCH_CHECK("k_prologue16");
    for (int l = 0; l < c.lo.L; ++l) {
      TRY_G(with_tail(f.layer(l, tail), [&](auto t) -> int {
        PROF_LAUNCH(st, hipLaunchKernelGGL((edtts16::k_layer16<C, decltype(t)::value>), dim3(g), dim3(C::THREADS), C::LDS_BYTES, st, a));
        LAUNCH_CHECK("k_layer16");
        return EDTTS_OK;
      }));
    }
    return EDTTS_OK;
  }
};

#include "edtts_generic.h"
#include "edtts_generic_bwd.h"
#include "edtts_semantic.h"
#include "edtts_semantic_bwd.h"
#include "edtts_hubert.h"
#include "edtts_hubert16.h"
#include "edtts_audio.h"
#include "edtts_optim.h"

static int no_instance16(const Layout& lo);
static int no_instance32(const Layout& lo);
#ifdef EDTTS_FAST_BUILD
#define EDTTS_FUSED_CHAIN(lo, MISS16, MISS32, ...)                                                       \
    if (!(lo).BF16 && (lo).H == 160 && (lo).HEADS == 4 && (lo).MEL == 80) { using LN = Launcher<Cfg<160, 4, 80>>; __VA_ARGS__; } \
    else if ((lo).BF16) { MISS16; }                                                                      \
    else { MISS32; }
static int no_instance16(const Layout&) { return fail(EDTTS_ERR_UNSUPPORTED, "EDTTS_FAST_BUILD: only the 160/4/80 fp32 instance is compiled"); }
// ... 5 lines not shown
#endif
#ifndef EDTTS_EXTRA_INSTANCES16
#define EDTTS_EXTRA_INSTANCES16(lo, ...)
#define EDTTS_EXTRA_NAMES16 ""
#endif
#define EDTTS_X16(lo, HH, HD, MM, ...) else if ((lo).H == HH && (lo).HEADS == HD && (lo).MEL == MM) { using LN = Launcher16<edtts16::Cfg16<HH, HD, MM>>; __VA_ARGS__; }
#define EDTTS_X(lo, HH, HD, MM, ...) else if ((lo).H == HH && (lo).HEADS == HD && (lo).MEL == MM) { using LN = Launcher<Cfg<HH, HD, MM>>; __VA_ARGS__; }
#define EDTTS_FUSED_CHAIN(lo, MISS16, MISS32, ...)                                                       \
    if ((lo).BF16) {                                                                                     \
      if ((lo).H == 256 && (lo).HEADS == 8 && (lo).MEL == 80) { using LN = Launcher16<edtts16::Cfg16<256, 8, 80, EDTTS16_NF>>; __VA_ARGS__; } \
      else if ((lo).H == 64 && (lo).HEADS == 2 && (lo).MEL == 80) { using LN = Launcher16<edtts16::Cfg16<64, 2, 80>>; __VA_ARGS__; } \
      EDTTS_EXTRA_INSTANCES16(lo, __VA_ARGS__)                                                           \
      else { MISS16; }                                                                                   \
    }                                                                                                    \
    else if ((lo).H == 160 && (lo).HEADS == 4 && (lo).MEL == 80) { using LN = Launcher<Cfg<160, 4, 80>>; __VA_ARGS__; } \
    else if ((lo).H == 256 && (lo).HEADS == 8 && (lo).MEL == 80) { using LN = Launcher<Cfg<256, 8, 80>>; __VA_ARGS__; }     \
    else if ((lo).H == 32 && (lo).HEADS == 2 && (lo).MEL == 80) { using LN = Launcher<Cfg<32, 2, 80>>; __VA_ARGS__; }       \
    else if ((lo).H == 64 && (lo).HEADS == 4 && (lo).MEL == 16) { using LN = Launcher<Cfg<64, 4, 16>>; __VA_ARGS__; }       \
    EDTTS_EXTRA_INSTANCES(lo, __VA_ARGS__)                                                               \
    else { MISS32; }
static int no_instance16(const Layout& lo) {
  return fail(EDTTS_ERR_UNSUPPORTED, "no bf16 kernel instance for hidden=%d heads=%d n_mels=%d "
              "(compiled: 256/8/80, 64/2/80" EDTTS_EXTRA_NAMES16 "; more: EDTTS_INSTANCES_BF16 at build time)", lo.H, lo.HEADS, lo.MEL);
}
static int no_instance32(const Layout& lo) {
  return fail(EDTTS_ERR_UNSUPPORTED, "no kernel instance for hidden=%d heads=%d n_mels=%d "
              "(compiled: 160/4/80, 256/8/80, 32/2/80, 64/4/16" EDTTS_EXTRA_NAMES "; more: EDTTS_INSTANCES at build time)", lo.H, lo.HEADS, lo.MEL);
}
#endif
#define EDTTS_DISPATCH(lo, ...)                                                                          \
  do {                                                                                                   \
    if ((lo).GEN) { using LN = GenericLauncher; __VA_ARGS__; }                                           \
    else { EDTTS_FUSED_CHAIN(lo, return no_instance16(lo), return no_instance32(lo), __VA_ARGS__) }      \
  } while (0)
static bool has_instance(const Layout& lo) {
  EDTTS_FUSED_CHAIN(lo, return false, return false, return true)
}

static int launch_cond(const Layout& lo, const float* blob, const int64_t* t, const int64_t* step_idx, const int64_t* t_host,
                       int rows, float* cond, float* wsb, hipStream_t st) {
  CondArgs a;
  memset(&a, 0, sizeof(a));
  a.t = t; a.step_idx = step_idx; a.H = lo.H; a.L = lo.L; a.n_step = lo.NSTEP;
  if (t_host) {
    if (rows > kMaxHostRows) return fail(EDTTS_ERR_ARG, "num_steps=%d > %d", rows, kMaxHostRows);
    a.use_host = 1; a.host_has_step = 1;
    for (int i = 0; i < rows; ++i) { a.t_host[i] = (int)t_host[i]; a.step_host[i] = i; }
  }
  a.freqs = blob + lo.freqs; a.t1T = blob + lo.t1T; a.t1b = blob + lo.t1b; a.t3T = blob + lo.t3T; a.t3b = blob + lo.t3b;
  a.step = blob + lo.step; a.blob = blob;
  for (int l = 0; l < lo.L; ++l) {
    a.ada1T[l] = (unsigned)lo.layer[l].ada1T; a.ada1b[l] = (unsigned)lo.layer[l].ada1b;
    a.ada3T[l] = (unsigned)lo.layer[l].ada3T; a.ada3b[l] = (unsigned)lo.layer[l].ada3b;
  }
  a.cond = cond;
  a.err = reinterpret_cast<unsigned*>(wsb);
  a.tcond = cond + (size_t)rows * lo.L * 2 * 2 * lo.H;
  hipLaunchKernelGGL(k_cond_mlp, dim3(rows), dim3(256), 2 * lo.H * sizeof(float), st, a);
  LAUNCH_CHECK("k_cond_mlp");
  hipLaunchKernelGGL(k_cond_ada, dim3(rows, 2 * lo.L, (2 * lo.H + 255) / 256), dim3(256), lo.H * sizeof(float), st, a);
  LAUNCH_CHECK("k_cond_ada");
  return EDTTS_OK;
}

extern "C" __global__ __launch_bounds__(256) void k_len_check(const int64_t* t_len, const int64_t* s_len, int B, int T, int S, int t_min, unsigned* err) {
  const int i = blockIdx.x * blockDim.x + threadIdx.x;
  if (i >= B) return;
  if ((t_len && (t_len[i] < t_min || t_len[i] > T)) || (s_len && (s_len[i] < 1 || s_len[i] > S))) atomicOr(err, (unsigned)EDTTS_IDX_LEN);
}
static int launch_len_check(const int64_t* t_len, const int64_t* s_len, int B, int T, int S, float* wsb, hipStream_t st, int t_min = 1) {
  if (!t_len && !s_len) return EDTTS_OK;
  hipLaunchKernelGGL(k_len_check, dim3((B + 255) / 256), dim3(256), 0, st, t_len, s_len, B, T, S, t_min, reinterpret_cast<unsigned*>(wsb));
  LAUNCH_CHECK("k_len_check");
  return EDTTS_OK;
}

static int check_shapes(const Layout& lo, int B, int T, int S) {
  if (B < 1 || T < 1 || S < 1) return fail(EDTTS_ERR_ARG, "B=%d T=%d S=%d must be positive", B, T, S);
  if (T > lo.MAXPOS) return fail(EDTTS_ERR_ARG, "T=%d exceeds the positional table (%d rows) -- the reference raises here too", T, lo.MAXPOS);
  if (S > lo.MAXCPOS) return fail(EDTTS_ERR_ARG, "S=%d exceeds the context positional table (%d rows)", S, lo.MAXCPOS);
  return EDTTS_OK;
}

struct SamplerInputs {
  const int64_t* t_dev = nullptr;
  const int64_t* t_host = nullptr;
  const int64_t* sem_idx = nullptr;
  const float* sem_features = nullptr;
  Lens ln;
  const float* x_T = nullptr;
  const float* x = nullptr;
};
template <class TailOf>
static int run_sampler(const EdttsDims* dims, const Layout& lo, const void* packed, void* workspace, int B, int T, int S, int num_steps,
                       const SamplerInputs& in, void* stream, TailOf&& tail_of) {
  hipStream_t st = (hipStream_t)stream;
  const float* blob = (const float*)packed;
  float* wsb = (float*)workspace;
  SubBatches sb;
  plan_call(lo, B, T, S, num_steps, wsb, &sb);
  TRY(launch_len_check(in.ln.t_dbl ? nullptr : in.ln.t, in.ln.s, B, T, S, wsb, st));
  TRY(launch_cond(lo, blob, in.t_dev, nullptr, in.t_host, num_steps, wsb + sb.cond, wsb, st));
  const size_t row = (size_t)lo.L * 2 * 2 * lo.H;
  const size_t per_utt = (size_t)T * lo.MEL;
  ForkJoin fj;
  TRY(fj.init(sb, st));
  auto call = [&](int j) { return CallCtx{lo, blob, sb.ws[j], wsb + sb.base[j], sb.B[j], T, S, dims->window, in.ln.at(sb.off[j]), fj.st[j]}; };
  EDTTS_DISPATCH(lo, {
    TRY(set_attrs_once<LN>());
    for (int j = 0; j < sb.n; ++j) {
      const size_t off = sb.off[j];
      TRY(LN::ctx(call(j), (in.sem_features || !in.sem_idx) ? nullptr : in.sem_idx + off * S,
                  in.sem_features ? in.sem_features + off * S * lo.SD : nullptr));
    }
    for (int i = 0; i < num_steps; ++i)
      for (int j = 0; j < sb.n; ++j) {
        const size_t o = (size_t)sb.off[j] * per_utt;
#ifdef EDTTS_WAVELOG
        g_wavelog_base = sb.off[j] * (sb.ws[j].Tp / 32);
#endif
        TRY(LN::forward(call(j), (i == 0 ? in.x_T : in.x) + o, wsb + sb.cond + i * row, 0, tail_of(i, sb.off[j], o)));
      }
  });
  return EDTTS_OK;
}

static int check_lms_modes(const float* coef_host, int num_steps) {
  for (int i = 0; i < num_steps; ++i) {
    const int mode = (int)coef_host[8 * i];
    if (mode < 1 || mode > 3 || mode > i + 1) return fail(EDTTS_ERR_ARG, "step %d: bad solver mode %d", i, mode);
  }
  return EDTTS_OK;
}
static LmsStepArgs lms_step_args(const float* c, float* hist, float* x0_all, size_t per, int i, size_t o) {
  LmsStepArgs ls;
  ls.k = LmsCoef{(int)c[0], c[1], c[2], c[3], c[4], c[5], c[6], c[7]};
  ls.x0_hist = hist + (size_t)(i & 1) * per + o;
  ls.h_new = hist + (size_t)((i + 1) & 1) * per + o;
  ls.h_old = hist + (size_t)(i & 1) * per + o;
  ls.x0_all = x0_all ? x0_all + (size_t)i * per + o : nullptr;
  return ls;
}

struct InpaintArgs {
  const EdttsDims* dims; const void* packed; void *workspace, *workspace_uncond; int B, T, S;
  const float *sem_features, *zero_features; float* x; int num_steps; const int64_t *t_all, *step_all;
  const float *coef_host, *known_mel; int overlap_len; const float* noise_k; uint64_t seed; float cfg_scale; float* v_uncond;
  const int64_t *t_len, *s_len; const uint64_t* seeds; void* stream;
};
template <class Checks, class InjectBefore, class TailOf, class InjectAfter>
static int run_inpaint(const InpaintArgs& a, const Layout& lo, bool own_ptrs, Checks&& own_checks, InjectBefore&& inject_before,
                       TailOf&& tail_of, InjectAfter&& inject_after) {
  if (!a.packed || !a.workspace || !a.sem_features || !a.x || !a.t_all || !a.step_all || !a.coef_host || !own_ptrs) return fail(EDTTS_ERR_ARG, "NULL pointer argument");
  if (a.num_steps < 1) return fail(EDTTS_ERR_ARG, "num_steps=%d < 1", a.num_steps);
  const bool guided = a.cfg_scale != 1.0f;
  if (guided && (!a.workspace_uncond || !a.zero_features || !a.v_uncond)) return fail(EDTTS_ERR_ARG, "cfg_scale != 1 needs workspace_uncond, zero_features and v_uncond");
  if (a.known_mel && (a.overlap_len < 1 || a.overlap_len > a.T)) return fail(EDTTS_ERR_ARG, "overlap_len=%d outside [1,%d]", a.overlap_len, a.T);
  TRY(check_shapes(lo, a.B, a.T, a.S));
  TRY(own_checks());
  hipStream_t st = (hipStream_t)a.stream;
  const float* blob = (const float*)a.packed;
  float* wsb = (float*)a.workspace;
  Workspace ws;
  make_workspace(lo, a.B, a.T, a.S, a.num_steps, &ws);
  TRY(launch_len_check(a.t_len, a.s_len, a.B, a.T, a.S, wsb, st, a.known_mel ? a.overlap_len : 1));
  TRY(launch_cond(lo, blob, a.t_all, a.step_all, nullptr, a.num_steps, wsb + ws.cond, wsb, st));
  const size_t row = (size_t)lo.L * 2 * 2 * lo.H;
  const CallCtx c{lo, blob, ws, wsb, a.B, a.T, a.S, a.dims->window, Lens{a.t_len, a.s_len}, st};
  CallCtx cu = c;
  cu.wsb = (float*)a.workspace_uncond;
  EDTTS_DISPATCH(lo, {
    TRY(set_attrs_once<LN>());
    TRY(LN::ctx(c, nullptr, a.sem_features));
    if (guided) TRY(LN::ctx(cu, nullptr, a.zero_features));
    for (int i = 0; i < a.num_steps; ++i) {
      if (a.known_mel) TRY(inject_before(i));
      StepTail tail = tail_of(i);
      if (guided) {
        StepTail eps_tail;
        eps_tail.eps = a.v_uncond;
        TRY(LN::forward(cu, a.x, wsb + ws.cond + i * row, 0, eps_tail));
        tail.vp.v_uncond = a.v_uncond;
      }
      TRY(LN::forward(c, a.x, wsb + ws.cond + i * row, 0, tail));
    }
    if (a.known_mel) TRY(inject_after());
  });
  return EDTTS_OK;
}

extern "C" {

int edtts_version(void) { return EDTTS_VERSION; }
const char* edtts_last_error(void) { return g_err; }
int edtts_num_global_slots(void) { return G_COUNT; }
int edtts_num_layer_slots(void) { return L_COUNT; }
const char* edtts_global_slot_name(int i) { return (i >= 0 && i < G_COUNT) ? kGlobalNames[i] : nullptr; }
const char* edtts_layer_slot_name(int i) { return (i >= 0 && i < L_COUNT) ? kLayerNames[i] : nullptr; }

int edtts_packed_bytes(const EdttsDims* dims, size_t* out_bytes) {
  Layout lo;
  int rc = make_layout(dims, &lo);
  if (rc) return rc;
  if (!out_bytes) return fail(EDTTS_ERR_ARG, "out_bytes is NULL");
// ... 800 lines not shown
}

int edtts_griffin_lim_scratch_floats(int B, int T, int n_fft, int hop, size_t* out_floats) {
  if (!out_floats || B < 1 || T < 2 || hop < 1) return fail(EDTTS_ERR_ARG, "bad sizes");
  if (n_fft != melpost::kNfft) return fail(EDTTS_ERR_UNSUPPORTED, "n_fft=%d (compiled: %d)", n_fft, melpost::kNfft);
  const size_t bt = (size_t)B * T, Lp = (size_t)n_fft + (size_t)hop * (T - 1);
  *out_floats = bt * melpost::kBins * 5 + bt * n_fft + (size_t)B * Lp;
  return EDTTS_OK;
}

static int griffin_lim_run(const float* spec, int B, int T, int n_fft, int hop, const float* window, const float* twiddle, int n_iter,
                           float momentum, float power, const float* angles0, uint64_t seed, const int64_t* t_len, const uint64_t* seeds,
                           void* idx_err, float* scratch, float* wave_out, void* stream) {
  if (!spec || !window || !twiddle || !scratch || !wave_out) return fail(EDTTS_ERR_ARG, "NULL pointer argument");
  if (B < 1 || T < 2 || hop < 1 || hop > n_fft || n_iter < 0 || power <= 0.f) return fail(EDTTS_ERR_ARG, "bad sizes");
  if (n_fft != melpost::kNfft) return fail(EDTTS_ERR_UNSUPPORTED, "n_fft=%d (compiled: %d, win_length = n_fft)", n_fft, melpost::kNfft);
  if (hop * (T - 1) <= n_fft / 2) return fail(EDTTS_ERR_ARG, "signal of %d samples is shorter than the reflect padding (torch.stft raises too)", hop * (T - 1));
  using namespace melpost;
  hipStream_t st = (hipStream_t)stream;
  TRY(melpost_len_check(t_len, B, T, (n_fft / 2) / hop + 2, idx_err, st));
  const size_t bt = (size_t)B * T;
  const int Lp = n_fft + hop * (T - 1);
  float* mag = scratch;
  cplx* ang = reinterpret_cast<cplx*>(mag + bt * kBins);
  cplx* tprev = ang + bt * kBins;
  float* frames = reinterpret_cast<float*>(tprev + bt * kBins);
  float* wave = frames + bt * n_fft;
  const cplx* tw = reinterpret_cast<const cplx*>(twiddle);
  const float mom = momentum / (1.0f + momentum);
  hipLaunchKernelGGL(k_gl_init, dim3(T, B), dim3(kThreads), 0, st, spec, angles0, T, 1.0f / power, (unsigned long long)seed, t_len,
                     reinterpret_cast<const unsigned long long*>(seeds), mag, ang, tprev);
  LAUNCH_CHECK("k_gl_init");
  int gx = (Lp + kThreads - 1) / kThreads;
  for (int it = 0; it <= n_iter; ++it) {
    hipLaunchKernelGGL(k_gl_istft, dim3(T, B), dim3(kThreads), 0, st, mag, ang, window, tw, T, t_len, frames);
    hipLaunchKernelGGL(k_gl_ola, dim3(gx, B), dim3(kThreads), 0, st, frames, window, T, hop, Lp, t_len, wave);
    if (it < n_iter) hipLaunchKernelGGL(k_gl_stft, dim3(T, B), dim3(kThreads), 0, st, wave, window, tw, T, hop, Lp, mom, t_len, ang, tprev);
  }
  LAUNCH_CHECK("griffin-lim kernels");
  if (t_len) {
    hipLaunchKernelGGL(k_gl_trim, dim3((hop * (T - 1) + kThreads - 1) / kThreads, B), dim3(kThreads), 0, st, wave, T, hop, Lp, t_len, wave_out);
    LAUNCH_CHECK("k_gl_trim");
    return EDTTS_OK;
  }
  HIP_TRY(hipMemcpy2DAsync(wave_out, (size_t)hop * (T - 1) * sizeof(float), wave + n_fft / 2, (size_t)Lp * sizeof(float),
                           (size_t)hop * (T - 1) * sizeof(float), B, hipMemcpyDeviceToDevice, st));
  return EDTTS_OK;
}

int edtts_griffin_lim(const float* spec, int B, int T, int n_fft, int hop, const float* window, const float* twiddle, int n_iter,
                      float momentum, float power, const float* angles0, uint64_t seed, float* scratch, float* wave_out, void* stream) {
  return griffin_lim_run(spec, B, T, n_fft, hop, window, twiddle, n_iter, momentum, power, angles0, seed, nullptr, nullptr, nullptr, scratch,
                         wave_out, stream);
}

int edtts_griffin_lim_len(const float* spec, int B, int T, int n_fft, int hop, const float* window, const float* twiddle, int n_iter,
                          float momentum, float power, const float* angles0, const int64_t* t_len, const uint64_t* seeds, void* idx_err,
                          float* scratch, float* wave_out, void* stream) {
  if (!t_len) return fail(EDTTS_ERR_ARG, "t_len is NULL (edtts_griffin_lim is the call without lengths)");
  if (!angles0 && !seeds) return fail(EDTTS_ERR_ARG, "seeds is NULL: without angles0, t_len and seeds come together");
  return griffin_lim_run(spec, B, T, n_fft, hop, window, twiddle, n_iter, momentum, power, angles0, 0, t_len, seeds, idx_err, scratch, wave_out,
                         stream);
}

#ifdef EDTTS_STAMPS
int edtts_debug_set_stamps(void* device_buffer) {
  g_stamps_fwd = (unsigned long long*)device_buffer;
  return EDTTS_OK;
}
#endif

#ifdef EDTTS_WAVELOG
int edtts_debug_set_wavelog(void* device_buffer) {
  g_wavelog = (unsigned long long*)device_buffer;
  return EDTTS_OK;
}
#endif

int edtts_set_coop(int mode) {
  if (mode == -1 || mode == 0 || mode == 14 || mode == 24 || mode == 22) return g_coop.exchange(mode);
  return g_coop.load();
}

int edtts_set_substreams(int n) {
  if (n >= 1 && n <= kMaxSub) return g_substreams.exchange(n);
  return g_substreams.load();
}

int edtts_substreams_for(const EdttsDims* dims, int B, int T) {
  const SettingsScope settings;
  Layout lo;
  if (make_layout(dims, &lo) || B < 1 || T < 1) return 1;
  return substreams_for(lo, B, T, (T + 1) / 2);
}

int edtts_profile_enable(int max_records) {
  std::lock_guard<std::mutex> lock(g_prof.mu);
  g_prof.on.store(false);
  for (hipEvent_t e : g_prof.start) (void)hipEventDestroy(e);
  for (hipEvent_t e : g_prof.stop) (void)hipEventDestroy(e);
  g_prof.start.clear(); g_prof.stop.clear(); g_prof.used = 0;
  if (max_records < 0) return fail(EDTTS_ERR_ARG, "max_records < 0");
  for (int i = 0; i < max_records; ++i) {
    hipEvent_t a, b;
    HIP_TRY(hipEventCreate(&a));
    HIP_TRY(hipEventCreate(&b));
    g_prof.start.push_back(a); g_prof.stop.push_back(b);
  }
  g_prof.on.store(max_records > 0);
  return EDTTS_OK;
}

int edtts_profile_collect(double* ms_by_kind, int* launches_by_kind) {
  if (!ms_by_kind || !launches_by_kind) return fail(EDTTS_ERR_ARG, "NULL pointer argument");
  std::lock_guard<std::mutex> lock(g_prof.mu);
  ms_by_kind[0] = ms_by_kind[1] = 0.0;
  launches_by_kind[0] = launches_by_kind[1] = 0;
  for (int i = 0; i < g_prof.used; ++i) {
    HIP_TRY(hipEventSynchronize(g_prof.stop[i]));
    float ms = 0.f;
    HIP_TRY(hipEventElapsedTime(&ms, g_prof.start[i], g_prof.stop[i]));
    ms_by_kind[0] += ms;
    launches_by_kind[0] += 1;
  }
  g_prof.used = 0;
  return EDTTS_OK;
}

int edtts_optim_chunk_size(void) { return edtts_opt::kOptChunk; }

int edtts_optim_chunk_table(const int64_t* numels, int n_tensors, int cap, int32_t* tensor, int64_t* offset, int32_t* count, int* n_chunks) {
  if (!numels || !n_chunks || n_tensors < 0) return fail(EDTTS_ERR_ARG, "edtts_optim_chunk_table: NULL pointer argument or n_tensors < 0");
  long long n = 0;
  for (int i = 0; i < n_tensors; ++i) {
    if (numels[i] < 0) return fail(EDTTS_ERR_ARG, "edtts_optim_chunk_table: numels[%d] = %lld < 0", i, (long long)numels[i]);
    for (long long o = 0; o < numels[i]; o += edtts_opt::kOptChunk, ++n) {
      if (n >= cap) continue;
      if (!tensor || !offset || !count) return fail(EDTTS_ERR_ARG, "edtts_optim_chunk_table: cap > 0 needs the three output arrays");
      const long long left = numels[i] - o;
      tensor[n] = i;
      offset[n] = o;
      count[n] = (int32_t)(left < edtts_opt::kOptChunk ? left : edtts_opt::kOptChunk);
    }
  }
  if (n > 0x7fffffff) return fail(EDTTS_ERR_UNSUPPORTED, "edtts_optim_chunk_table: %lld chunks", n);
  *n_chunks = (int)n;
  return EDTTS_OK;
}

int edtts_optim_scratch_bytes(int n_chunks, int n_groups, size_t* out_bytes) {
  if (!out_bytes || n_chunks < 0 || n_groups < 1) return fail(EDTTS_ERR_ARG, "edtts_optim_scratch_bytes: n_chunks=%d n_groups=%d", n_chunks, n_groups);
  edtts_opt::OptScratch s;
  edtts_opt::opt_scratch((size_t)n_chunks, (size_t)n_groups, &s);
  *out_bytes = s.total;
  return EDTTS_OK;
}

int edtts_optim_step(const EdttsOptimTensor* tensors, int n_tensors, const EdttsOptimGroup* groups, int n_groups, double max_norm, int flags,
                     void* scratch, size_t scratch_bytes, void* stream) {
  using namespace edtts_opt;
  if (n_tensors < 0 || n_groups < 1 || (n_tensors && !tensors) || !groups || !scratch)
    return fail(EDTTS_ERR_ARG, "edtts_optim_step: NULL pointer argument, n_tensors=%d or n_groups=%d", n_tensors, n_groups);
  if (flags & ~(EDTTS_OPT_CLIP | EDTTS_OPT_SKIP_NONFINITE | EDTTS_OPT_ZERO_GRADS | EDTTS_OPT_EMA_ONLY))
    return fail(EDTTS_ERR_ARG, "edtts_optim_step: unknown flag bits 0x%x", flags);
  const bool ema_only = flags & EDTTS_OPT_EMA_ONLY;
  if (ema_only && (flags & ~EDTTS_OPT_EMA_ONLY)) return fail(EDTTS_ERR_ARG, "edtts_optim_step: EDTTS_OPT_EMA_ONLY excludes the other flags");
// ... 97 lines not shown
```

### edge-diffusion-tts_amd/edge_diffusion_tts_amd/native.py

```python
from __future__ import annotations

import ctypes as C
import os
from typing import List, Optional, Sequence, Tuple

import torch

_PKG_DIR = os.path.dirname(os.path.abspath(__file__))
LIB_PATH = os.environ.get("EDTTS_LIB", os.path.join(os.path.dirname(_PKG_DIR), "lib", "libedtts_hip.so"))

EXPORTED_SYMBOLS = (
    "edtts_version", "edtts_last_error", "edtts_num_global_slots", "edtts_num_layer_slots", "edtts_global_slot_name",
    "edtts_layer_slot_name", "edtts_packed_bytes", "edtts_pack_weights", "edtts_workspace_bytes", "edtts_decoder_forward",
    "edtts_ddim_step", "edtts_ddpm_step", "edtts_generate", "edtts_sample_ddpm", "edtts_sample_multistep", "edtts_dsconv_forward", "edtts_profile_enable",
    "edtts_profile_collect", "edtts_randn", "edtts_index_errors", "edtts_sample_inpaint",
    "edtts_mel_to_spec", "edtts_griffin_lim_scratch_floats", "edtts_griffin_lim", "edtts_set_substreams", "edtts_set_coop", "edtts_dsconv_scratch_floats", "edtts_substreams_for",
    "edtts_decoder_forward_len", "edtts_generate_len", "edtts_sample_ddpm_len", "edtts_sample_multistep_len",
    "edtts_sample_inpaint_len", "edtts_randn_rows", "edtts_sample_inpaint_multistep_len",
    "edtts_sem_packed_bytes", "edtts_sem_num_codes", "edtts_sem_pack", "edtts_sem_encode", "edtts_sem_decode", "edtts_sem_stats",
    "edtts_hubert_frames", "edtts_hubert_packed_bytes", "edtts_hubert_pack", "edtts_hubert_workspace_bytes", "edtts_hubert_forward",
    "edtts_hubert_packed_bytes_dt", "edtts_hubert_pack_dt", "edtts_hubert_workspace_bytes_dt", "edtts_hubert_forward_dt",
    "edtts_melspec", "edtts_mel_segment_stats", "edtts_logmel_stats", "edtts_resample",
    "edtts_mel_to_spec_len", "edtts_griffin_lim_len",
    "edtts_train_tape_bytes", "edtts_train_scratch_bytes", "edtts_train_dw_slab_rows", "edtts_decoder_forward_train",
    "edtts_decoder_backward",
    "edtts_decoder_forward_train_drop", "edtts_decoder_backward_drop", "edtts_dropout_mask",
    "edtts_sem_train_packed_bytes", "edtts_sem_train_pack", "edtts_sem_train_tape_bytes", "edtts_sem_train_scratch_bytes",
    "edtts_sem_encode_train", "edtts_sem_backward", "edtts_sem_dropout_mask",
    "edtts_sem_vq_train_packed_bytes", "edtts_sem_vq_train_pack", "edtts_sem_vq_tape_bytes", "edtts_sem_vq_scratch_bytes",
    "edtts_sem_vq_encode_train", "edtts_sem_vq_ema_update", "edtts_sem_vq_backward",
    "edtts_decoder_forward_train_len", "edtts_decoder_backward_len",
    "edtts_optim_chunk_size", "edtts_optim_chunk_table", "edtts_optim_scratch_bytes", "edtts_optim_step", "edtts_generic_slot_dest",
)

EDTTS_IDX_SEM, EDTTS_IDX_STEP, EDTTS_IDX_LEN = 1, 2, 4


class EdttsDims(C.Structure):
    _fields_ = [(n, C.c_int32) for n in (
        "hidden", "layers", "heads", "n_mels", "ffn_mult", "codebook_size", "semantic_dim", "window", "max_pos",
        "max_ctx_pos", "n_step_emb", "compute_dtype")]


class EdttsDropout(C.Structure):
    _fields_ = [("p", C.c_float), ("seed", C.c_uint64)]


DROP_SITES = {"attn": 0, "cross_attn": 1, "ffn_act": 2, "ffn_out": 3}


SEM_FSQ, SEM_VQ = 0, 1


class EdttsSemDims(C.Structure):
    _fields_ = [("in_dim", C.c_int32), ("semantic_dim", C.c_int32), ("quantizer", C.c_int32), ("codebook_size", C.c_int32),
                ("n_levels", C.c_int32), ("levels", C.c_int32 * 16)]


def sem_dims(in_dim: int, semantic_dim: int, levels: Optional[Sequence[int]] = None, codebook_size: int = 0) -> EdttsSemDims:
    d = EdttsSemDims()
    d.in_dim, d.semantic_dim = int(in_dim), int(semantic_dim)
    if levels is not None:
        levels = [int(v) for v in levels]
        d.quantizer, d.n_levels = SEM_FSQ, len(levels)
        for i, v in enumerate(levels[:16]):
            d.levels[i] = v
    else:
        d.quantizer, d.codebook_size = SEM_VQ, int(codebook_size)
    return d


class EdttsOptimState(C.Structure):
    _fields_ = [("step", C.c_int64), ("skipped", C.c_int64), ("total_norm", C.c_float), ("clip_coef", C.c_float), ("skip", C.c_int32),
                ("reserved", C.c_int32)]


class EdttsOptimGroup(C.Structure):
    _fields_ = [(n, C.c_double) for n in ("lr", "beta1", "beta2", "eps", "weight_decay")]


class EdttsOptimTensor(C.Structure):
    _fields_ = [(n, C.c_void_p) for n in ("p", "g", "m", "v", "ema", "mirror", "ema_mirror")] + [
        ("numel", C.c_int64), ("group", C.c_int32), ("rows", C.c_int32), ("cols", C.c_int32), ("ema_decay", C.c_float)]


OPT_CLIP, OPT_SKIP_NONFINITE, OPT_ZERO_GRADS, OPT_EMA_ONLY = 1, 2, 4, 8


class EdttsHubertDims(C.Structure):
    _fields_ = [("n_conv", C.c_int32), ("conv_dim", C.c_int32 * 16), ("conv_kernel", C.c_int32 * 16), ("conv_stride", C.c_int32 * 16),
                ("hidden", C.c_int32), ("heads", C.c_int32), ("intermediate", C.c_int32), ("num_layers", C.c_int32),
                ("pos_kernel", C.c_int32), ("pos_groups", C.c_int32), ("layer_norm_eps", C.c_float)]


COMPUTE_DTYPES = {"f32": 0, "fp32": 0, "float32": 0, "bf16": 1, "bfloat16": 1}
KERNELS = {"compiled": 0, "generic": 0x100, "auto": 0x200}


class EdttsError(RuntimeError):
# ... 36 lines not shown
    L.edtts_griffin_lim_scratch_floats.argtypes = [i32, i32, i32, i32, C.POINTER(sz)]
    L.edtts_griffin_lim.argtypes = [vp, i32, i32, i32, i32, vp, vp, i32, f32, f32, vp, C.c_uint64, vp, vp, vp]
    L.edtts_mel_to_spec_len.argtypes = [vp, vp, vp, vp, i32, i32, i32, i32, vp, i32, i32, vp, vp, vp]
    L.edtts_griffin_lim_len.argtypes = [vp, i32, i32, i32, i32, vp, vp, i32, f32, f32, vp, vp, vp, vp, vp, vp, vp]
    L.edtts_sample_inpaint.argtypes = [C.POINTER(EdttsDims), vp, vp, vp, i32, i32, i32, vp, vp, vp, i32, vp, vp, C.POINTER(f32), vp, i32,
                                       vp, C.c_uint64, f32, vp, vp]
    L.edtts_sample_inpaint_len.argtypes = [C.POINTER(EdttsDims), vp, vp, vp, i32, i32, i32, vp, vp, vp, i32, vp, vp, C.POINTER(f32),
                                           vp, i32, vp, C.c_uint64, f32, vp, vp, vp, vp, vp]
    L.edtts_sample_inpaint_multistep_len.argtypes = [C.POINTER(EdttsDims), vp, vp, vp, i32, i32, i32, vp, vp, vp, i32, vp, vp,
                                                     C.POINTER(f32), vp, i32, vp, C.c_uint64, f32, vp, vp, vp, vp, vp, vp, vp]
    L.edtts_randn_rows.argtypes = [vp, i32, sz, vp, C.c_uint32, f32, vp]
    L.edtts_sample_multistep.argtypes = [C.POINTER(EdttsDims), vp, vp, i32, i32, i32, vp, vp, vp, i32, C.POINTER(C.c_int64),
                                         C.POINTER(f32), vp, vp, vp, vp]
    L.edtts_decoder_forward_len.argtypes = [C.POINTER(EdttsDims), vp, vp, i32, i32, i32, vp, vp, vp, vp, vp, vp, vp, vp, vp]
    L.edtts_generate_len.argtypes = [C.POINTER(EdttsDims), vp, vp, i32, i32, vp, vp, vp, i32, C.POINTER(C.c_int64),
                                     C.POINTER(f32), vp, vp, vp]
    L.edtts_sample_ddpm_len.argtypes = [C.POINTER(EdttsDims), vp, vp, i32, i32, vp, vp, vp, i32, vp, C.POINTER(f32), vp, C.c_uint64,
                                        C.c_int64, vp, vp]
    L.edtts_sample_multistep_len.argtypes = [C.POINTER(EdttsDims), vp, vp, i32, i32, i32, vp, vp, vp, vp, vp, i32,
                                             C.POINTER(C.c_int64), C.POINTER(f32), vp, vp, vp, vp]
    L.edtts_dsconv_forward.argtypes = [vp] * 6 + [i32] * 7 + [vp, vp, vp]
    L.edtts_dsconv_scratch_floats.argtypes = [i32] * 7 + [C.POINTER(sz)]
    sdp = C.POINTER(EdttsSemDims)
    L.edtts_sem_packed_bytes.argtypes = [sdp, C.POINTER(sz)]
    L.edtts_sem_num_codes.argtypes = [sdp, C.POINTER(C.c_int64)]
    L.edtts_sem_pack.argtypes = [sdp, C.POINTER(vp), i32, vp, vp]
    L.edtts_sem_encode.argtypes = [sdp, vp, vp, i32, i32, vp, vp, vp, vp, vp, vp]
    L.edtts_sem_decode.argtypes = [sdp, vp, vp, C.c_int64, vp, vp]
    L.edtts_sem_stats.argtypes = [vp, C.c_int64, vp, vp, vp]
    hdp = C.POINTER(EdttsHubertDims)
    L.edtts_hubert_frames.argtypes = [hdp, C.c_int64, C.POINTER(C.c_int64)]
    L.edtts_hubert_packed_bytes.argtypes = [hdp, C.POINTER(sz)]
    L.edtts_hubert_pack.argtypes = [hdp, C.POINTER(vp), i32, vp, vp]
    L.edtts_hubert_workspace_bytes.argtypes = [hdp, i32, i32, C.POINTER(sz)]
    L.edtts_hubert_forward.argtypes = [hdp, vp, vp, i32, i32, vp, vp, vp, vp]
    L.edtts_hubert_packed_bytes_dt.argtypes = [hdp, i32, C.POINTER(sz)]
    L.edtts_hubert_pack_dt.argtypes = [hdp, i32, C.POINTER(vp), i32, vp, vp]
    L.edtts_hubert_workspace_bytes_dt.argtypes = [hdp, i32, i32, i32, C.POINTER(sz)]
    L.edtts_hubert_forward_dt.argtypes = [hdp, i32, vp, vp, i32, i32, vp, vp, vp, vp]
    L.edtts_melspec.argtypes = [vp, i32, i32, vp, i32, i32, vp, vp, vp, vp, i32, i32, i32, vp, vp]
    L.edtts_mel_segment_stats.argtypes = [vp, i32, i32, vp, vp, i32, i32, i32, vp, vp, vp, vp, i32, vp, vp, vp]
    L.edtts_logmel_stats.argtypes = [vp, i32, i32, i32, i32, vp, i32, vp, vp, vp]
    L.edtts_resample.argtypes = [vp, i32, i32, vp, i32, i32, i32, i32, vp, C.c_int64, vp, vp]
    L.edtts_train_tape_bytes.argtypes = [C.POINTER(EdttsDims), i32, i32, i32, C.POINTER(sz)]
    L.edtts_train_scratch_bytes.argtypes = [C.POINTER(EdttsDims), i32, i32, i32, C.POINTER(sz)]
    L.edtts_train_dw_slab_rows.argtypes = [i32]
    L.edtts_train_dw_slab_rows.restype = i32
    L.edtts_decoder_forward_train.argtypes = [C.POINTER(EdttsDims), vp, vp, vp, i32, i32, i32, vp, vp, vp, vp, vp, vp, vp]
    L.edtts_decoder_backward.argtypes = [C.POINTER(EdttsDims), vp, vp, vp, i32, i32, i32, vp, vp, vp, vp, vp, vp, C.POINTER(vp), i32,
                                         vp, vp, vp, vp]
    dpp = C.POINTER(EdttsDropout)
    L.edtts_decoder_forward_train_drop.argtypes = [C.POINTER(EdttsDims), vp, vp, vp, i32, i32, i32, vp, vp, vp, vp, vp, vp, dpp, vp]
    L.edtts_decoder_backward_drop.argtypes = [C.POINTER(EdttsDims), vp, vp, vp, i32, i32, i32, vp, vp, vp, vp, vp, vp, C.POINTER(vp), i32,
                                              vp, vp, vp, dpp, vp]
    L.edtts_dropout_mask.argtypes = [C.POINTER(EdttsDims), i32, i32, i32, i32, i32, dpp, vp, vp]
    L.edtts_decoder_forward_train_len.argtypes = [C.POINTER(EdttsDims), vp, vp, vp, i32, i32, i32, vp, vp, vp, vp, vp, vp, dpp, vp, vp, vp]
    L.edtts_decoder_backward_len.argtypes = [C.POINTER(EdttsDims), vp, vp, vp, i32, i32, i32, vp, vp, vp, vp, vp, vp, C.POINTER(vp), i32,
                                             vp, vp, vp, dpp, vp, vp, vp]
    L.edtts_sem_train_packed_bytes.argtypes = [sdp, C.POINTER(sz)]
    L.edtts_sem_train_pack.argtypes = [sdp, C.POINTER(vp), i32, vp, vp]
    L.edtts_sem_train_tape_bytes.argtypes = [sdp, i32, i32, C.POINTER(sz)]
    L.edtts_sem_train_scratch_bytes.argtypes = [sdp, i32, i32, C.POINTER(sz)]
    L.edtts_sem_encode_train.argtypes = [sdp, vp, vp, i32, i32, vp, vp, vp, vp, vp, dpp, vp]
    L.edtts_sem_backward.argtypes = [sdp, vp, vp, vp, vp, i32, i32, vp, vp, C.POINTER(vp), i32, vp, vp, dpp, vp]
    L.edtts_sem_dropout_mask.argtypes = [sdp, i32, i32, dpp, vp, vp]
    L.edtts_sem_vq_train_packed_bytes.argtypes = [sdp, C.POINTER(sz)]
    L.edtts_sem_vq_train_pack.argtypes = [sdp, C.POINTER(vp), i32, vp, vp]
    L.edtts_sem_vq_tape_bytes.argtypes = [sdp, i32, i32, C.POINTER(sz)]
    L.edtts_sem_vq_scratch_bytes.argtypes = [sdp, i32, i32, C.POINTER(sz)]
    L.edtts_sem_vq_encode_train.argtypes = [sdp, vp, vp, i32, i32, vp, vp, vp, vp, vp, vp, i32, C.c_double, dpp, vp]
    L.edtts_sem_vq_ema_update.argtypes = [sdp, vp, vp, i32, i32, vp, vp, C.c_double, C.c_double, vp, vp, vp, vp, vp]
    L.edtts_sem_vq_backward.argtypes = [sdp, vp, vp, vp, vp, vp, i32, i32, vp, vp, vp, C.c_double, C.POINTER(vp), i32, vp, vp, dpp, vp]
    L.edtts_optim_chunk_size.restype = i32
    L.edtts_optim_chunk_table.argtypes = [C.POINTER(C.c_int64), i32, i32, C.POINTER(C.c_int32), C.POINTER(C.c_int64), C.POINTER(C.c_int32),
                                          C.POINTER(i32)]
    L.edtts_optim_scratch_bytes.argtypes = [i32, i32, C.POINTER(sz)]
    L.edtts_optim_step.argtypes = [C.POINTER(EdttsOptimTensor), i32, C.POINTER(EdttsOptimGroup), i32, C.c_double, i32, vp, sz, vp]
    L.edtts_generic_slot_dest.argtypes = [C.POINTER(EdttsDims), i32, C.POINTER(sz), C.POINTER(i32), C.POINTER(i32), C.POINTER(i32)]
    L.edtts_profile_enable.argtypes = [i32]
    L.edtts_set_substreams.argtypes = [i32]
    L.edtts_set_substreams.restype = i32
    L.edtts_set_coop.argtypes = [i32]
    L.edtts_set_coop.restype = i32
    L.edtts_substreams_for.argtypes = [C.POINTER(EdttsDims), i32, i32]
    L.edtts_substreams_for.restype = i32
    L.edtts_profile_collect.argtypes = [C.POINTER(C.c_double), C.POINTER(i32)]
    for name in EXPORTED_SYMBOLS:
        fn = getattr(L, name)
        if fn.restype is C.c_int and name not in ("edtts_version", "edtts_num_global_slots", "edtts_num_layer_slots", "edtts_set_substreams", "edtts_set_coop", "edtts_substreams_for",
                                                  "edtts_train_dw_slab_rows", "edtts_optim_chunk_size"):
            fn.errcheck = _errcheck
    _lib = L
    return L


def _errcheck(rc, func, args):
    if rc != 0:
        msg = _lib.edtts_last_error().decode() if _lib is not None else "?"
        if rc == -2 and "Either sem_idx or sem_features" in msg:
            raise ValueError(msg)
        raise EdttsError(f"{func.__name__} failed (code {rc}): {msg}")
    return rc


def _dev_ptr(t: Optional[torch.Tensor], dtype: torch.dtype, name: str) -> Optional[int]:
    if t is None:
        return None
    if not t.is_cuda:
        raise EdttsError(f"{name}: expected a tensor on the HIP device, got {t.device} -- the MI355X sampler path has no CPU fallback")
    if t.dtype != dtype:
        raise EdttsError(f"{name}: expected dtype {dtype}, got {t.dtype}")
    if not t.is_contiguous():
        raise EdttsError(f"{name}: tensor must be contiguous")
    return t.data_ptr()


def _stream(device) -> int:
    return torch.cuda.current_stream(device).cuda_stream


def _size_query(fn, *args, ctype=C.c_size_t) -> int:
    out = ctype(0)
    fn(*args, C.byref(out))
    return out.value


def _slot_ptrs(tensors: Sequence[Optional[torch.Tensor]], what: str):
    return (C.c_void_p * len(tensors))(*[_dev_ptr(t, torch.float32, f"{what}[{i}]") for i, t in enumerate(tensors)])


def slot_names(n_layers: int) -> List[str]:
    L = lib()
    names = [L.edtts_global_slot_name(i).decode() for i in range(L.edtts_num_global_slots())]
    per = [L.edtts_layer_slot_name(i).decode() for i in range(L.edtts_num_layer_slots())]
    for l in range(n_layers):
        names += [f"layers.{l}.{n}" for n in per]
    return names


def packed_bytes(dims: EdttsDims) -> int:
    return _size_query(lib().edtts_packed_bytes, C.byref(dims))


def workspace_bytes(dims: EdttsDims, B: int, T: int, S: int, cond_rows: int) -> int:
    return _size_query(lib().edtts_workspace_bytes, C.byref(dims), B, T, S, cond_rows)


def pack_weights(dims: EdttsDims, tensors: Sequence[torch.Tensor], packed: torch.Tensor) -> None:
    ptrs = _slot_ptrs(tensors, "weight")
    lib().edtts_pack_weights(C.byref(dims), ptrs, len(tensors), _dev_ptr(packed, torch.uint8, "packed"), _stream(packed.device))


def lengths(n: Optional[torch.Tensor], B: int, hi: int, device, name: str) -> Optional[torch.Tensor]:
    if n is None:
        return None
    if not isinstance(n, torch.Tensor):
        raise ValueError(f"{name}: expected an int64 tensor of shape [{B}], got {type(n).__name__}")
    if n.dtype != torch.int64:
        raise ValueError(f"{name}: expected dtype torch.int64, got {n.dtype}")
    if tuple(n.shape) != (B,):
        raise ValueError(f"{name}: expected shape [{B}], got {list(n.shape)}")
    if n.is_cuda:
        if device is not None and torch.device(device).type == "cuda" and n.device != torch.device(device):
            raise ValueError(f"{name}: on {n.device}, the call runs on {device}")
        return n.contiguous()
    if B and (int(n.min()) < 1 or int(n.max()) > hi):
        raise ValueError(f"{name}: lengths must be in [1, {hi}], got [{int(n.min())}, {int(n.max())}]")
    if torch.device(device).type == "cuda" and torch.cuda.is_current_stream_capturing():
        raise RuntimeError(f"{name}: a CPU length tensor cannot be copied to the device during graph capture; "
                           "pass a device tensor (and copy new lengths into it before each replay)")
    return n.to(device)

# ... 496 lines not shown
                                    None if drop is None else C.byref(drop), _stream(dev))
    return idx, zq, counts, loss


def sem_vq_ema_update(dims: EdttsSemDims, idx: torch.Tensor, z: torch.Tensor, lengths: Optional[torch.Tensor], counts: torch.Tensor,
                      decay: float, epsilon: float, ema_cluster_size: torch.Tensor, ema_w: torch.Tensor, codebook: torch.Tensor) -> None:
    B, T = idx.shape
    scratch = torch.empty(sem_vq_scratch_bytes(dims, B, T), dtype=torch.uint8, device=idx.device)
    f = torch.float32
    lib().edtts_sem_vq_ema_update(C.byref(dims), _dev_ptr(idx, torch.int64, "idx"), _dev_ptr(z, f, "z"), B, T,
                                  _dev_ptr(lengths, torch.int64, "lengths"), _dev_ptr(counts, torch.int32, "counts"), float(decay),
                                  float(epsilon), _dev_ptr(ema_cluster_size, f, "ema_cluster_size"), _dev_ptr(ema_w, f, "ema_w"),
                                  _dev_ptr(codebook, f, "codebook"), scratch.data_ptr(), _stream(idx.device))


def sem_vq_backward(dims: EdttsSemDims, packed: Optional[torch.Tensor], packed_train: Optional[torch.Tensor], tape: torch.Tensor,
                    h: torch.Tensor, idx: torch.Tensor, lengths: Optional[torch.Tensor], d_zq: Optional[torch.Tensor],
                    d_loss: Optional[torch.Tensor], commit: float, grads: Sequence[Optional[torch.Tensor]],
                    d_z: Optional[torch.Tensor] = None, drop=None) -> None:
    B, T, _ = h.shape
    ptrs = _slot_ptrs(grads, "grad")
    scratch = torch.empty(sem_vq_scratch_bytes(dims, B, T), dtype=torch.uint8, device=h.device)
    drop = _dropout(drop)
    f = torch.float32
    lib().edtts_sem_vq_backward(C.byref(dims), _dev_ptr(packed, torch.uint8, "packed"), _dev_ptr(packed_train, torch.uint8, "packed_train"),
                                _dev_ptr(tape, torch.uint8, "tape"), _dev_ptr(h, f, "features"), _dev_ptr(idx, torch.int64, "idx"), B, T,
                                _dev_ptr(lengths, torch.int64, "lengths"), _dev_ptr(d_zq, f, "d_zq"), _dev_ptr(d_loss, f, "d_loss"),
                                float(commit), ptrs, len(grads), _dev_ptr(d_z, f, "d_z"), scratch.data_ptr(),
                                None if drop is None else C.byref(drop), _stream(h.device))


def hubert_frames(dims: EdttsHubertDims, n_samples: int) -> int:
    return _size_query(lib().edtts_hubert_frames, C.byref(dims), int(n_samples), ctype=C.c_int64)


HUBERT_DTYPES = {"fp32": 0, "bf16": 1}


def hubert_packed_bytes(dims: EdttsHubertDims, compute_dtype: int = 0) -> int:
    if compute_dtype:
        return _size_query(lib().edtts_hubert_packed_bytes_dt, C.byref(dims), int(compute_dtype))
    return _size_query(lib().edtts_hubert_packed_bytes, C.byref(dims))


def hubert_workspace_bytes(dims: EdttsHubertDims, B: int, T_audio: int, compute_dtype: int = 0) -> int:
    if compute_dtype:
        return _size_query(lib().edtts_hubert_workspace_bytes_dt, C.byref(dims), int(compute_dtype), int(B), int(T_audio))
    return _size_query(lib().edtts_hubert_workspace_bytes, C.byref(dims), int(B), int(T_audio))


def hubert_pack(dims: EdttsHubertDims, tensors: Sequence[torch.Tensor], packed: torch.Tensor, compute_dtype: int = 0) -> None:
    ptrs = _slot_ptrs(tensors, "weight")
    if compute_dtype:
        lib().edtts_hubert_pack_dt(C.byref(dims), int(compute_dtype), ptrs, len(tensors), _dev_ptr(packed, torch.uint8, "packed"),
                                   _stream(packed.device))
    else:
        lib().edtts_hubert_pack(C.byref(dims), ptrs, len(tensors), _dev_ptr(packed, torch.uint8, "packed"), _stream(packed.device))


def hubert_forward(dims: EdttsHubertDims, packed: torch.Tensor, wav: torch.Tensor, lengths: Optional[torch.Tensor], out: torch.Tensor,
                   workspace: torch.Tensor, compute_dtype: int = 0) -> None:
    B, T = wav.shape
    args = (_dev_ptr(packed, torch.uint8, "packed"), _dev_ptr(wav, torch.float32, "wav"), B, T,
            _dev_ptr(lengths, torch.int64, "lengths"), _dev_ptr(out, torch.float32, "out"),
            _dev_ptr(workspace, torch.uint8, "workspace"), _stream(wav.device))
    if compute_dtype:
        lib().edtts_hubert_forward_dt(C.byref(dims), int(compute_dtype), *args)
    else:
        lib().edtts_hubert_forward(C.byref(dims), *args)


def set_substreams(n: int) -> int:
    return int(lib().edtts_set_substreams(int(n)))


def substreams_for(dims: EdttsDims, B: int, T: int) -> int:
    return int(lib().edtts_substreams_for(C.byref(dims), int(B), int(T)))


def set_coop(mode: int) -> int:
    return int(lib().edtts_set_coop(int(mode)))


def profile_enable(max_records: int) -> None:
    lib().edtts_profile_enable(int(max_records))


def profile_collect():
    ms, n = (C.c_double * 2)(), (C.c_int * 2)()
    lib().edtts_profile_collect(ms, n)
    return (ms[0], n[0]), (ms[1], n[1])
```

### include/edtts.h

```cpp
#ifndef EDTTS_H_
#define EDTTS_H_

#include <stddef.h>
#include <stdint.h>

#ifdef __cplusplus
extern "C" {
#endif

#define EDTTS_VERSION 400

enum {
  EDTTS_OK = 0,
  EDTTS_ERR_UNSUPPORTED = -1,
  EDTTS_ERR_ARG = -2,
  EDTTS_ERR_HIP = -3
};

enum {
  EDTTS_IDX_SEM = 1,
  EDTTS_IDX_STEP = 2,
  EDTTS_IDX_LEN = 4
};

// ... 72 lines not shown
                                    const int64_t* s_len, void* stream);
int edtts_decoder_backward_len(const EdttsDims* dims, const void* packed, void* workspace, const void* tape, int B, int T, int S,
                               const float* x, const int64_t* t, const int64_t* step_idx, const int64_t* sem_idx,
                               const float* sem_features, const float* d_eps, void* const* grad_slots, int n_slots, float* d_x,
                               float* d_sem_features, void* scratch, const EdttsDropout* drop, const int64_t* t_len,
                               const int64_t* s_len, void* stream);

int edtts_ddim_step(const float* alpha_bar, int n_table, const float* x, const float* eps, const int64_t* t,
                    const int64_t* t_prev, int B, size_t n_per_batch, float eta, const float* noise,
                    float* x_prev, float* x0, void* stream);

int edtts_ddpm_step(const float* alphas, const float* alpha_bar, const float* betas, const float* post_var,
                    int n_table, const float* x, const float* eps, const int64_t* t, int B, size_t n_per_batch,
                    const float* noise, float* x_prev, void* stream);

int edtts_generate(const EdttsDims* dims, const void* packed, void* workspace, int B, int S,
                   const int64_t* sem_idx, const float* x_T, int num_steps, const int64_t* timesteps_host,
                   const float* coef_host, float* x_work, float* x0_out, void* stream);
int edtts_generate_len(const EdttsDims* dims, const void* packed, void* workspace, int B, int S, const int64_t* sem_idx,
                       const int64_t* s_len, const float* x_T, int num_steps, const int64_t* timesteps_host, const float* coef_host,
                       float* x_work, float* x0_out, void* stream);

int edtts_sample_ddpm(const EdttsDims* dims, const void* packed, void* workspace, int B, int S,
                      const int64_t* sem_idx, const float* x_T, int num_steps, const int64_t* t_all,
                      const float* coef_host, const float* noise_all, uint64_t seed, int64_t batch_offset, float* x_out,
                      void* stream);
int edtts_sample_ddpm_len(const EdttsDims* dims, const void* packed, void* workspace, int B, int S, const int64_t* sem_idx,
                          const int64_t* s_len, const float* x_T, int num_steps, const int64_t* t_all, const float* coef_host,
                          const float* noise_all, uint64_t seed, int64_t batch_offset, float* x_out, void* stream);

int edtts_randn(float* out, size_t n, uint64_t seed, uint32_t stream_id, uint64_t elem_offset, float scale, void* stream);
int edtts_randn_rows(float* out, int B, size_t n_per_row, const uint64_t* seeds, uint32_t stream_id, float scale, void* stream);

int edtts_sample_multistep(const EdttsDims* dims, const void* packed, void* workspace, int B, int T, int S,
                           const int64_t* sem_idx, const float* sem_features, const float* x_T, int num_steps,
                           const int64_t* timesteps_host, const float* coef_host, float* hist, float* x0_all,
                           float* x_out, void* stream);
int edtts_sample_multistep_len(const EdttsDims* dims, const void* packed, void* workspace, int B, int T, int S,
                               const int64_t* sem_idx, const float* sem_features, const int64_t* t_len, const int64_t* s_len,
                               const float* x_T, int num_steps, const int64_t* timesteps_host, const float* coef_host, float* hist,
                               float* x0_all, float* x_out, void* stream);

int edtts_sample_inpaint(const EdttsDims* dims, const void* packed, void* workspace, void* workspace_uncond, int B, int T, int S,
                         const float* sem_features, const float* zero_features, float* x, int num_steps,
                         const int64_t* t_all, const int64_t* step_all, const float* coef_host, const float* known_mel,
                         int overlap_len, const float* noise_k, uint64_t seed, float cfg_scale, float* v_uncond, void* stream);
int edtts_sample_inpaint_len(const EdttsDims* dims, const void* packed, void* workspace, void* workspace_uncond, int B, int T, int S,
                             const float* sem_features, const float* zero_features, float* x, int num_steps,
                             const int64_t* t_all, const int64_t* step_all, const float* coef_host, const float* known_mel,
                             int overlap_len, const float* noise_k, uint64_t seed, float cfg_scale, float* v_uncond,
                             const int64_t* t_len, const int64_t* s_len, const uint64_t* seeds, void* stream);

int edtts_sample_inpaint_multistep_len(const EdttsDims* dims, const void* packed, void* workspace, void* workspace_uncond, int B, int T,
                                       int S, const float* sem_features, const float* zero_features, float* x, int num_steps,
                                       const int64_t* t_all, const int64_t* step_all, const float* coef_host, const float* known_mel,
                                       int overlap_len, const float* noise_k, uint64_t seed, float cfg_scale, float* v_uncond,
                                       const int64_t* t_len, const int64_t* s_len, const uint64_t* seeds, float* hist, float* x0_all,
                                       void* stream);

int edtts_dsconv_scratch_floats(int B, int C_in, int C_out, int T, int ksize, int stride, int groups, size_t* out_floats);
int edtts_dsconv_forward(const float* x, const float* dw, const float* pw, const float* pb, const float* gn_w,
                         const float* gn_b, int B, int C_in, int C_out, int T, int ksize, int stride, int groups,
                         float* scratch, float* y, void* stream);

int edtts_mel_to_spec(const float* mel_n, const float* mean, const float* stdv, const float* pinv, int B, int T, int n_mels,
                      int n_freqs, float* spec, void* stream);
int edtts_griffin_lim_scratch_floats(int B, int T, int n_fft, int hop, size_t* out_floats);
int edtts_griffin_lim(const float* spec, int B, int T, int n_fft, int hop, const float* window, const float* twiddle, int n_iter,
                      float momentum, float power, const float* angles0, uint64_t seed, float* scratch, float* wave_out,
                      void* stream);
int edtts_mel_to_spec_len(const float* mel_n, const float* mean, const float* stdv, const float* pinv, int B, int T, int n_mels,
                          int n_freqs, const int64_t* t_len, int smooth_h, int smooth_w, void* idx_err, float* spec, void* stream);
int edtts_griffin_lim_len(const float* spec, int B, int T, int n_fft, int hop, const float* window, const float* twiddle, int n_iter,
                          float momentum, float power, const float* angles0, const int64_t* t_len, const uint64_t* seeds,
                          void* idx_err, float* scratch, float* wave_out, void* stream);

int edtts_profile_enable(int max_records);
int edtts_profile_collect(double* ms_by_kind, int* launches_by_kind);

int edtts_set_substreams(int n);
int edtts_substreams_for(const EdttsDims* dims, int B, int T);

int edtts_set_coop(int mode);

enum { EDTTS_SEM_FSQ = 0, EDTTS_SEM_VQ = 1 };
typedef struct EdttsSemDims {
  int32_t in_dim;
  int32_t semantic_dim;
  int32_t quantizer;
  int32_t codebook_size;
  int32_t n_levels;
  int32_t levels[16];
} EdttsSemDims;
int edtts_sem_packed_bytes(const EdttsSemDims* dims, size_t* out_bytes);
int edtts_sem_num_codes(const EdttsSemDims* dims, int64_t* out_codes);
int edtts_sem_pack(const EdttsSemDims* dims, const void* const* slots, int n_slots, void* packed, void* stream);
int edtts_sem_encode(const EdttsSemDims* dims, const void* packed, const float* h, int B, int T, const int64_t* lengths,
                     int64_t* idx, float* z, float* z_q, int32_t* counts, void* stream);
int edtts_sem_decode(const EdttsSemDims* dims, const void* packed, const int64_t* idx, int64_t n, float* z_q, void* stream);
int edtts_sem_stats(const int32_t* counts, int64_t n_codes, float* perplexity, int64_t* used, void* stream);

int edtts_sem_train_packed_bytes(const EdttsSemDims* dims, size_t* out_bytes);
int edtts_sem_train_pack(const EdttsSemDims* dims, const void* const* slots, int n_slots, void* packed_train, void* stream);
int edtts_sem_train_tape_bytes(const EdttsSemDims* dims, int B, int T, size_t* out_bytes);
int edtts_sem_train_scratch_bytes(const EdttsSemDims* dims, int B, int T, size_t* out_bytes);
int edtts_sem_encode_train(const EdttsSemDims* dims, const void* packed, const float* h, int B, int T, const int64_t* lengths,
                           int64_t* idx, float* z_q, int32_t* counts, void* tape, const EdttsDropout* drop, void* stream);
int edtts_sem_backward(const EdttsSemDims* dims, const void* packed, const void* packed_train, const void* tape, const float* h, int B,
                       int T, const int64_t* lengths, const float* d_zq, void* const* grad_slots, int n_slots, float* d_z,
                       void* scratch, const EdttsDropout* drop, void* stream);
int edtts_sem_dropout_mask(const EdttsSemDims* dims, int B, int T, const EdttsDropout* drop, uint8_t* keep, void* stream);

int edtts_sem_vq_train_packed_bytes(const EdttsSemDims* dims, size_t* out_bytes);
int edtts_sem_vq_train_pack(const EdttsSemDims* dims, const void* const* slots, int n_slots, void* packed_train, void* stream);
int edtts_sem_vq_tape_bytes(const EdttsSemDims* dims, int B, int T, size_t* out_bytes);
int edtts_sem_vq_scratch_bytes(const EdttsSemDims* dims, int B, int T, size_t* out_bytes);
int edtts_sem_vq_encode_train(const EdttsSemDims* dims, const void* packed, const float* h, int B, int T, const int64_t* lengths,
                              int64_t* idx, float* z_q, int32_t* counts, float* loss, void* tape, int training, double commit,
                              const EdttsDropout* drop, void* stream);
int edtts_sem_vq_ema_update(const EdttsSemDims* dims, const int64_t* idx, const float* z, int B, int T, const int64_t* lengths,
                            const int32_t* counts, double decay, double epsilon, float* ema_cluster_size, float* ema_w,
                            float* codebook, void* scratch, void* stream);
int edtts_sem_vq_backward(const EdttsSemDims* dims, const void* packed, const void* packed_train, const void* tape, const float* h,
                          const int64_t* idx, int B, int T, const int64_t* lengths, const float* d_zq, const float* d_loss,
                          double commit, void* const* grad_slots, int n_slots, float* d_z, void* scratch, const EdttsDropout* drop,
                          void* stream);

typedef struct EdttsOptimState {
  int64_t step;
  int64_t skipped;
  float total_norm;
  float clip_coef;
  int32_t skip;
  int32_t reserved;
} EdttsOptimState;
typedef struct EdttsOptimGroup {
  double lr, beta1, beta2, eps, weight_decay;
} EdttsOptimGroup;
typedef struct EdttsOptimTensor {
  float* p;
  float* g;
  float* m;
  float* v;
  float* ema;
  float* mirror;
  float* ema_mirror;
  int64_t numel;
  int32_t group;
  int32_t rows, cols;
  float ema_decay;
} EdttsOptimTensor;
enum {
  EDTTS_OPT_CLIP = 1,
  EDTTS_OPT_SKIP_NONFINITE = 2,
  EDTTS_OPT_ZERO_GRADS = 4,
  EDTTS_OPT_EMA_ONLY = 8
};
int edtts_optim_chunk_size(void);
int edtts_optim_chunk_table(const int64_t* numels, int n_tensors, int cap, int32_t* tensor, int64_t* offset, int32_t* count, int* n_chunks);
int edtts_optim_scratch_bytes(int n_chunks, int n_groups, size_t* out_bytes);
int edtts_optim_step(const EdttsOptimTensor* tensors, int n_tensors, const EdttsOptimGroup* groups, int n_groups, double max_norm, int flags,
                     void* scratch, size_t scratch_bytes, void* stream);
int edtts_generic_slot_dest(const EdttsDims* dims, int slot, size_t* offset_floats, int* rows, int* cols, int* transposed);

typedef struct EdttsHubertDims {
  int32_t n_conv;
// ... 41 lines not shown
```

Before: 8.685 million.

## Fuse DDIM/DDPM step tail with next step's prologue across diffusion step boundary

Adds TAIL_DDIM_NEXT/TAIL_DDPM_NEXT layer variants in which the last layer's output projection computes x_prev in registers. It then runs the next step's in_proj, pos-embedding, RMS norm and QKV prologue directly, with the weight ring handed over to the next stream, and the separate k_prologue launch is skipped for later steps. It also prefetches x one tile ahead in the tail and replaces the DDIM division with a double-precision reciprocal multiply. Host setup is reordered so per-substream context launches come before the len-check and cond kernels, with a head event. The changes aim to remove a kernel launch and the x_prev/x global round trip per step, at the cost of higher register pressure in the fused last-layer kernel and a switchable default-on path.

Result: no change. 8.709 million (median of 6 runs) (+0.3%).

```diff
diff --git a/edge-diffusion-tts_amd/csrc/edtts_device.h b/edge-diffusion-tts_amd/csrc/edtts_device.h
--- a/edge-diffusion-tts_amd/csrc/edtts_device.h
+++ b/edge-diffusion-tts_amd/csrc/edtts_device.h
@@ -163,10 +163,20 @@
     else if (i == N - 1) refill(N - N % B, N);
   }
   EDTTS_DEV void advance(int n) { soff += (unsigned)n * 1024u; }
+  template <int N>
+  EDTTS_DEV void refill_after_last(int i, __amdgpu_buffer_rsrc_t nx) {
+    constexpr int B = kRefillBurst < RN ? kRefillBurst : RN;
+    const int lo = (i + 1) % B == 0 ? i + 1 - B : N - N % B, hi = (i + 1) % B == 0 ? i + 1 : N;
+    if ((i + 1) % B != 0 && i != N - 1) return;
+#pragma unroll
+    for (int j = lo; j < hi; ++j) r[j % RN] = j + RN < N ? frag(j + RN) : bufld4(nx, voff, (unsigned)(j + RN - N) * 1024u);
+    __builtin_amdgcn_sched_barrier(0);
+  }
+  EDTTS_DEV void handed_over(__amdgpu_buffer_rsrc_t nx) { rs = nx; soff = 0; }
 };
 
-template <int KT, int RN, int NF>
-EDTTS_DEV void gemm_phase(FragRing<RN>& ring, const f4 (&in)[KT][NF], f4 (&acc)[NF]) {
+template <int KT, int RN, int NF, bool LAST = false>
+EDTTS_DEV void gemm_phase(FragRing<RN>& ring, const f4 (&in)[KT][NF], f4 (&acc)[NF], __amdgpu_buffer_rsrc_t nx) {
   static_assert(KT % RN == 0, "phase length must be a multiple of the ring size");
   constexpr bool SPLIT = NF < 4;
   f4 b[NF];
@@ -184,13 +194,19 @@
         if (SPLIT && (kt & 1)) b[ft] = EDTTS_MFMA(a[r], in[kt][ft][r], b[ft]);
         else acc[ft] = EDTTS_MFMA(a[r], in[kt][ft][r], acc[ft]);
       }
-    ring.template refill_after<KT>(kt);
+    if constexpr (LAST) ring.template refill_after_last<KT>(kt, nx);
+    else ring.template refill_after<KT>(kt);
   }
   if (SPLIT) {
 #pragma unroll
     for (int ft = 0; ft < NF; ++ft) acc[ft] += b[ft];
   }
-  ring.advance(KT);
+  if constexpr (LAST) ring.handed_over(nx);
+  else ring.advance(KT);
+}
+template <int KT, int RN, int NF>
+EDTTS_DEV void gemm_phase(FragRing<RN>& ring, const f4 (&in)[KT][NF], f4 (&acc)[NF]) {
+  gemm_phase<KT, RN, NF, false>(ring, in, acc, ring.rs);
 }
 
 template <int KT, int RN, int NF>
@@ -776,11 +792,12 @@
   }
 }
 
-EDTTS_DEV void ddim_elem(float x, float e, float s1m, float sab, float sabp, float cdir, float& x0, float& xp) {
+EDTTS_DEV double recip_rn(float b) { return 1.0 / (double)b; }
+EDTTS_DEV void ddim_elem(float x, float e, float s1m, double rinv, float sabp, float cdir, float& x0, float& xp) {
 #pragma clang fp contract(off)
   float t1 = s1m * e;
   float t2 = x - t1;
-  float v = div_rn(t2, sab);
+  float v = (float)((double)t2 * rinv);
   v = fminf(fmaxf(v, -3.0f), 3.0f);
   x0 = v;
   float t3 = sabp * v;
diff --git a/edge-diffusion-tts_amd/csrc/edtts_generic.h b/edge-diffusion-tts_amd/csrc/edtts_generic.h
--- a/edge-diffusion-tts_amd/csrc/edtts_generic.h
+++ b/edge-diffusion-tts_amd/csrc/edtts_generic.h
@@ -355,7 +355,7 @@
     a.x_prev[idx] = ddpm_elem(a.x[idx], e, nz, cf);
   } else {
     float v0, vp;
-    ddim_elem(a.x[idx], e, a.c_s1m, a.c_sab, a.c_sabp, a.c_dir, v0, vp);
+    ddim_elem(a.x[idx], e, a.c_s1m, a.c_rinv, a.c_sabp, a.c_dir, v0, vp);
     a.x0[idx] = v0;
     a.x_prev[idx] = vp;
   }
diff --git a/edge-diffusion-tts_amd/csrc/edtts_kernels.hip b/edge-diffusion-tts_amd/csrc/edtts_kernels.hip
--- a/edge-diffusion-tts_amd/csrc/edtts_kernels.hip
+++ b/edge-diffusion-tts_amd/csrc/edtts_kernels.hip
@@ -437,6 +437,9 @@
   float *x0_hist, *x0_all;
   const int64_t *t_len, *s_len;
   int t_dbl;
+  double c_rinv;
+  const float* cond_next;
+  const float* stream_next;
 };
 
 EDTTS_DEV int utt_len_of(int64_t v, int full, bool dbl) {
@@ -530,6 +533,57 @@
 }
 
 template <class C>
+EDTTS_DEV void prologue_body(WStream<C>& ring, const f4 (&xin)[C::MT][C::NF], const KArgs& a, const float* mod, int b, int m0, int lane) {
+  constexpr int NF = C::NF;
+  const int fq = lane & 15, g = lane >> 4;
+  f4 h[C::HT][NF];
+#pragma unroll
+  for (int nt = 0; nt < C::HT; ++nt) {
+    const f4 bias = ldg4(a.inp_b + 16 * nt + 4 * g);
+#pragma unroll
+    for (int ft = 0; ft < NF; ++ft) h[nt][ft] = bias;
+  }
+  {
+    constexpr int N = C::HT * C::MT;
+    static_assert(N % WStream<C>::RN_ == 0 && C::HT % 2 == 0, "in_proj must be a whole number of ring turns");
+#pragma unroll
+    for (int nt = 0; nt < C::HT; nt += 2)
+#pragma unroll
+      for (int kt = 0; kt < C::MT; ++kt) {
+        const int i = nt * C::MT + 2 * kt;
+        const f4& fa = ring.at(i);
+        const f4& fb = ring.at(i + 1);
+#pragma unroll
+        for (int r = 0; r < 4; ++r) {
+#pragma unroll
+          for (int ft = 0; ft < NF; ++ft) h[nt][ft] = EDTTS_MFMA(fa[r], xin[kt][ft][r], h[nt][ft]);
+#pragma unroll
+          for (int ft = 0; ft < NF; ++ft) h[nt + 1][ft] = EDTTS_MFMA(fb[r], xin[kt][ft][r], h[nt + 1][ft]);
+        }
+        ring.template refill_after<N>(i);
+        ring.template refill_after<N>(i + 1);
+      }
+    ring.advance(N);
+  }
+#pragma unroll
+  for (int ft = 0; ft < NF; ++ft) {
+    int f = m0 + 16 * ft + fq;
+    f = f < a.max_pos ? f : a.max_pos - 1;
+#pragma unroll
+    for (int nt = 0; nt < C::HT; ++nt) h[nt][ft] += ldg4(a.pe + (size_t)f * C::H + 16 * nt + 4 * g);
+  }
+  {
+    float* hp = a.h + ((size_t)b * a.Tp + m0 + fq) * C::H + 4 * g;
+#pragma unroll
+    for (int nt = 0; nt < C::HT; ++nt)
+#pragma unroll
+      for (int ft = 0; ft < NF; ++ft) stg4(hp + 16 * nt + (size_t)ft * 16 * C::H, h[nt][ft]);
+  }
+  f4 hn[C::HT][NF];
+  rms_norm_tile<C::HT, NF>(h, a.n1w, mod, g, hn);
+  qkv_tail<C>(ring, hn, a, b, m0, lane);
+}
+template <class C>
 __global__ __launch_bounds__(C::THREADS) void k_prologue(KArgs a) {
   constexpr int NF = C::NF;
   const TileId tl = wave_tile(a.B, a.Tp, C::WAVES, C::WF);
@@ -548,63 +602,18 @@
     for (int t = 0; t < C::MT; ++t)
       xin[t][ft] = f < Tb ? ldg4(a.x + ((size_t)b * a.T + f) * C::MEL + 16 * t + 4 * g) : splat(0.f);
   }
-  f4 h[C::HT][NF];
-#pragma unroll
-  for (int nt = 0; nt < C::HT; ++nt) {
-    const f4 bias = ldg4(a.inp_b + 16 * nt + 4 * g);
-#pragma unroll
-    for (int ft = 0; ft < NF; ++ft) h[nt][ft] = bias;
-  }
-  {
-    constexpr int N = C::HT * C::MT;
-    static_assert(N % WStream<C>::RN_ == 0 && C::HT % 2 == 0, "in_proj must be a whole number of ring turns");
-#pragma unroll
-    for (int nt = 0; nt < C::HT; nt += 2)
-#pragma unroll
-      for (int kt = 0; kt < C::MT; ++kt) {
-        const int i = nt * C::MT + 2 * kt;
-        const f4& fa = ring.at(i);
-        const f4& fb = ring.at(i + 1);
-#pragma unroll
-        for (int r = 0; r < 4; ++r) {
-#pragma unroll
-          for (int ft = 0; ft < NF; ++ft) h[nt][ft] = EDTTS_MFMA(fa[r], xin[kt][ft][r], h[nt][ft]);
-#pragma unroll
-          for (int ft = 0; ft < NF; ++ft) h[nt + 1][ft] = EDTTS_MFMA(fb[r], xin[kt][ft][r], h[nt + 1][ft]);
-        }
-        ring.template refill_after<N>(i);
-        ring.template refill_after<N>(i + 1);
-      }
-    ring.advance(N);
-  }
-#pragma unroll
-  for (int ft = 0; ft < NF; ++ft) {
-    int f = m0 + 16 * ft + fq;
-    f = f < a.max_pos ? f : a.max_pos - 1;
-#pragma unroll
-    for (int nt = 0; nt < C::HT; ++nt) h[nt][ft] += ldg4(a.pe + (size_t)f * C::H + 16 * nt + 4 * g);
-  }
-  {
-    float* hp = a.h + ((size_t)b * a.Tp + m0 + fq) * C::H + 4 * g;
-#pragma unroll
-    for (int nt = 0; nt < C::HT; ++nt)
-#pragma unroll
-      for (int ft = 0; ft < NF; ++ft) stg4(hp + 16 * nt + (size_t)ft * 16 * C::H, h[nt][ft]);
-  }
-  f4 hn[C::HT][NF];
-  const float* mod = a.cond + (size_t)b * a.cond_bstride;
-  rms_norm_tile<C::HT, NF>(h, a.n1w, mod, g, hn);
-  qkv_tail<C>(ring, hn, a, b, m0, lane);
-}
-
-enum { TAIL_QKV = 0, TAIL_EPS = 1, TAIL_DDIM = 2, TAIL_DDPM = 3, TAIL_LMS = 4, TAIL_VPRED = 5, TAIL_VLMS = 6 };
+  prologue_body<C>(ring, xin, a, a.cond + (size_t)b * a.cond_bstride, b, m0, lane);
+}
+
+enum { TAIL_QKV = 0, TAIL_EPS = 1, TAIL_DDIM = 2, TAIL_DDPM = 3, TAIL_LMS = 4, TAIL_VPRED = 5, TAIL_VLMS = 6,
+       TAIL_DDIM_NEXT = 7, TAIL_DDPM_NEXT = 8 };
+constexpr int tail_base(int tail) { return tail == TAIL_DDIM_NEXT ? TAIL_DDIM : (tail == TAIL_DDPM_NEXT ? TAIL_DDPM : tail); }
 
 template <int TAIL>
-EDTTS_DEV void tail_apply(const KArgs& a, size_t idx, f4 ev, bool blend = false) {
+EDTTS_DEV f4 tail_apply(const KArgs& a, size_t idx, f4 ev, f4 xv, bool blend = false) {
   if (TAIL == TAIL_EPS) {
     stg4(a.eps + idx, ev);
   } else if (TAIL == TAIL_LMS) {
-    const f4 xv = ldg4(a.x + idx);
     f4 hn = splat(0.f), ho = splat(0.f);
     if (a.lms.mode >= 2) hn = ldg4(a.h_new + idx);
     if (a.lms.mode >= 3) ho = ldg4(a.h_old + idx);
@@ -621,7 +630,6 @@
     stg4(a.x_prev + idx, xn);
   } else if (TAIL == TAIL_VLMS) {
     const bool guided = a.v_uncond != nullptr;
-    const f4 xv = ldg4(a.x + idx);
     const f4 vu = ldg4((guided ? a.v_uncond : a.x) + idx);
     f4 hn = splat(0.f), ho = splat(0.f);
     if (a.lms.mode >= 2) hn = ldg4(a.h_new + idx);
@@ -640,7 +648,6 @@
     if (!blend) stg4(a.x_prev + idx, xn);
   } else if (TAIL == TAIL_VPRED) {
     const bool guided = a.v_uncond != nullptr;
-    const f4 xv = ldg4(a.x + idx);
     const f4 vu = ldg4((guided ? a.v_uncond : a.x) + idx);
     f4 v, xn;
 #pragma unroll
@@ -649,26 +656,31 @@
     for (int r = 0; r < 4; ++r) xn[r] = vpred_elem(xv[r], v[r], a.vp);
     stg4(a.x_prev + idx, xn);
   } else if (TAIL == TAIL_DDPM) {
-    const f4 xv = ldg4(a.x + idx);
     const f4 nz = a.noise ? ldg4(a.noise + idx) : philox_normal4(a.seed, a.step, (a.philox_base + idx) >> 2);
     const DdpmCoef cf{a.p_coef1, a.p_coef2, a.p_sd};
     f4 xp;
 #pragma unroll
     for (int r = 0; r < 4; ++r) xp[r] = ddpm_elem(xv[r], ev[r], nz[r], cf);
     stg4(a.x_prev + idx, xp);
+    return xp;
   } else {
-    const f4 xv = ldg4(a.x + idx);
     f4 x0, xp;
 #pragma unroll
     for (int r = 0; r < 4; ++r) {
       float v0, vp;
-      ddim_elem(xv[r], ev[r], a.c_s1m, a.c_sab, a.c_sabp, a.c_dir, v0, vp);
+      ddim_elem(xv[r], ev[r], a.c_s1m, a.c_rinv, a.c_sabp, a.c_dir, v0, vp);
       x0[r] = v0;
       xp[r] = vp;
     }
     stg4(a.x0 + idx, x0);
     stg4(a.x_prev + idx, xp);
-  }
+    return xp;
+  }
+  return splat(0.f);
+}
+template <int TAIL>
+EDTTS_DEV void tail_apply(const KArgs& a, size_t idx, f4 ev) {
+  tail_apply<TAIL>(a, idx, ev, TAIL == TAIL_EPS ? splat(0.f) : ldg4(a.x + idx));
 }
 template <int TAIL>
 EDTTS_DEV void tail_zero(const KArgs& a, size_t idx) {
@@ -700,16 +712,26 @@
   stg4(a.x_prev + idx, o);
 }
 template <int TAIL>
-EDTTS_DEV void tail_store(const KArgs& a, int f, int Tb, size_t idx, f4 ev) {
+EDTTS_DEV f4 tail_store(const KArgs& a, int f, int Tb, size_t idx, f4 ev, f4 xv) {
+  f4 xp = splat(0.f);
   if constexpr (TAIL == TAIL_VLMS) {
     const bool blend = a.known != nullptr && f < Tb && f < a.inj_frames;
-    if (f < Tb) tail_apply<TAIL>(a, idx, ev, blend);
+    if (f < Tb) tail_apply<TAIL>(a, idx, ev, xv, blend);
     else tail_zero<TAIL>(a, idx);
     if (blend) vlms_blend(a, idx);
   } else {
-    if (f < Tb) tail_apply<TAIL>(a, idx, ev);
+    if (f < Tb) xp = tail_apply<TAIL>(a, idx, ev, xv);
     else tail_zero<TAIL>(a, idx);
   }
+  return xp;
+}
+template <int TAIL>
+EDTTS_DEV f4 tail_x(const KArgs& a, int f, int Tb, size_t idx) {
+  return (TAIL != TAIL_EPS && f < Tb) ? ldg4(a.x + idx) : splat(0.f);
+}
+template <int TAIL>
+EDTTS_DEV void tail_store(const KArgs& a, int f, int Tb, size_t idx, f4 ev) {
+  tail_store<TAIL>(a, f, Tb, idx, ev, tail_x<TAIL>(a, f, Tb, idx));
 }
 
 struct QGlobal {
@@ -894,23 +916,45 @@
     rms_norm_tile<C::HT, NF>(h, a.n1w, mod, g, h);
     qkv_tail<C>(ring, h, a, b, m0, lane);
   } else {
+    constexpr int TB = tail_base(TAIL);
+    constexpr bool NEXT = TAIL != TB;
     f4 hn[C::HT][NF];
     layer_norm_tile<C::HT, NF>(h, a.fnw, a.fnb, g, hn);
+    auto load_x = [&](int nt, f4 (&xq)[NF]) {
+#pragma unroll
+      for (int ft = 0; ft < NF; ++ft) {
+        const int f = m0 + 16 * ft + fq;
+        xq[ft] = tail_x<TB>(a, f, Tb, ((size_t)b * a.T + f) * C::MEL + 16 * nt + 4 * g);
+      }
+    };
+    f4 xq[NF];
+    load_x(0, xq);
+    f4 xnext[C::MT][NF];
+    __amdgpu_buffer_rsrc_t nx = ring.rs;
+    if constexpr (NEXT) nx = make_rsrc(a.stream_next);
 #pragma unroll
     for (int nt = 0; nt < C::MT; ++nt) {
       const f4 ob = ldg4(a.outp_b + 16 * nt + 4 * g);
-      f4 e[NF];
-#pragma unroll
-      for (int ft = 0; ft < NF; ++ft) e[ft] = splat(0.f);
-      gemm_phase<C::HT>(ring, hn, e);
+      f4 e[NF], xn[NF];
+#pragma unroll
+      for (int ft = 0; ft < NF; ++ft) e[ft] = xn[ft] = splat(0.f);
+      if (nt + 1 < C::MT) load_x(nt + 1, xn);
+      if constexpr (NEXT) {
+        if (nt == C::MT - 1) gemm_phase<C::HT, WStream<C>::RN_, NF, true>(ring, hn, e, nx);
+        else gemm_phase<C::HT>(ring, hn, e);
+      } else {
+        gemm_phase<C::HT>(ring, hn, e);
+      }
 #pragma unroll
       for (int ft = 0; ft < NF; ++ft) {
         const int f = m0 + 16 * ft + fq;
-        if (f >= a.T) continue;
-        const size_t idx = ((size_t)b * a.T + f) * C::MEL + 16 * nt + 4 * g;
-        tail_store<TAIL>(a, f, Tb, idx, e[ft] + ob);
-      }
-    }
+        f4 xp = splat(0.f);
+        if (f < a.T) xp = tail_store<TB>(a, f, Tb, ((size_t)b * a.T + f) * C::MEL + 16 * nt + 4 * g, e[ft] + ob, xq[ft]);
+        if constexpr (NEXT) xnext[nt][ft] = xp;
+        xq[ft] = xn[ft];
+      }
+    }
+    if constexpr (NEXT) prologue_body<C>(ring, xnext, a, a.cond_next + (size_t)b * a.cond_bstride, b, m0, lane);
   }
   STAMPX(a.stamps, 5, a.diag_skip);
 #ifdef EDTTS_STAMPS
@@ -939,7 +983,7 @@
   if (!tl.valid) return;
   const int Tb = utt_len(a.t_len, tl.b, a.T, a.t_dbl);
   if (tl.m0 >= live_end(Tb)) {
-    if constexpr (TAIL != TAIL_QKV) tail_zero_tile<C, TAIL>(a, tl.b, tl.m0, lane);
+    if constexpr (TAIL != TAIL_QKV) tail_zero_tile<C, tail_base(TAIL)>(a, tl.b, tl.m0, lane);
     return;
   }
   const int Sb = utt_len(a.s_len, tl.b, a.S);
@@ -1225,7 +1269,8 @@
   const long tp = (long)a.t_prev[b];
   const float abp = tp >= 0 ? a.alpha_bar[clamp_idx(tp, a.n_table)] : 1.0f;
   const DdimCoef cf = ddim_coef(ab, abp, a.eta);
-  const float s1m = cf.s1m, sab = cf.sab, sabp = cf.sabp, cdir = cf.cdir, sigma = cf.sigma;
+  const float s1m = cf.s1m, sabp = cf.sabp, cdir = cf.cdir, sigma = cf.sigma;
+  const double rinv = recip_rn(cf.sab);
   const size_t base = (size_t)b * a.n_per_batch;
   const size_t n4 = a.vec4 ? a.n_per_batch >> 2 : 0;
   for (size_t i = (size_t)blockIdx.x * blockDim.x + threadIdx.x; i < n4; i += (size_t)gridDim.x * blockDim.x) {
@@ -1237,7 +1282,7 @@
 #pragma unroll
     for (int r = 0; r < 4; ++r) {
       float v, p;
-      ddim_elem(xv[r], e[r], s1m, sab, sabp, cdir, v, p);
+      ddim_elem(xv[r], e[r], s1m, rinv, sabp, cdir, v, p);
       if (a.noise) p = add_mul_rn(p, sigma, nz[r]);
       x0[r] = v;
       xp[r] = p;
@@ -1248,7 +1293,7 @@
   for (size_t i = (n4 << 2) + (size_t)blockIdx.x * blockDim.x + threadIdx.x; i < a.n_per_batch; i += (size_t)gridDim.x * blockDim.x) {
     const size_t o = base + i;
     float v, p;
-    ddim_elem(a.x[o], a.eps[o], s1m, sab, sabp, cdir, v, p);
+    ddim_elem(a.x[o], a.eps[o], s1m, rinv, sabp, cdir, v, p);
     if (a.noise) p = add_mul_rn(p, sigma, a.noise[o]);
     a.x0[o] = v;
     a.x_prev[o] = p;
@@ -2040,20 +2085,24 @@
 };
 static std::atomic<int> g_coop{[] { const char* e = getenv("EDTTS_COOP"); return e ? atoi(e) : -1; }()};
 static std::atomic<int> g_substreams{[] { const char* e = getenv("EDTTS_SUBSTREAMS"); const int v = e ? atoi(e) : 4; return v < 1 ? 1 : (v > kMaxSub ? kMaxSub : v); }()};
+static std::atomic<int> g_fuse_boundary{[] { const char* e = getenv("EDTTS_FUSE_BOUNDARY"); return e ? (atoi(e) != 0) : 1; }()};
 struct Settings {
-  int substreams, coop;
+  int substreams, coop, fuse_boundary;
+  static Settings load() {
+    return Settings{g_substreams.load(std::memory_order_relaxed), g_coop.load(std::memory_order_relaxed), g_fuse_boundary.load(std::memory_order_relaxed)};
+  }
 };
 static thread_local const Settings* t_settings = nullptr;
 struct SettingsScope {
   Settings snap;
   const Settings* prev;
-  SettingsScope() : snap{g_substreams.load(std::memory_order_relaxed), g_coop.load(std::memory_order_relaxed)}, prev(t_settings) {
+  SettingsScope() : snap(Settings::load()), prev(t_settings) {
     t_settings = &snap;
   }
   ~SettingsScope() { t_settings = prev; }
 };
 static Settings current_settings() {
-  return t_settings ? *t_settings : Settings{g_substreams.load(std::memory_order_relaxed), g_coop.load(std::memory_order_relaxed)};
+  return t_settings ? *t_settings : Settings::load();
 }
 
 static void plan_sub(const Layout& lo, int B, int T, int S, int cond_rows, int n, SubBatches* sb) {
@@ -2101,6 +2150,7 @@
   unsigned long long last_use = 0;
   hipStream_t s[kMaxSub - 1] = {};
   hipEvent_t fork = nullptr, join[kMaxSub - 1] = {};
+  hipEvent_t head = nullptr;
 };
 constexpr int kSideSets = 8;
 static std::mutex g_side_pool_mu;
@@ -2160,6 +2210,7 @@
     SideStream& sd = g_sides.get(dev, main);
     sd.dev = dev;
     if (!sd.fork) HIP_TRY(hipEventCreateWithFlags(&sd.fork, hipEventDisableTiming));
+    if (!sd.head) HIP_TRY(hipEventCreateWithFlags(&sd.head, hipEventDisableTiming));
     for (int j = 0; j + 1 < sb.n; ++j) {
       if (!sd.s[j]) HIP_TRY(hipStreamCreateWithFlags(&sd.s[j], hipStreamNonBlocking));
       if (!sd.join[j]) HIP_TRY(hipEventCreateWithFlags(&sd.join[j], hipEventDisableTiming));
@@ -2171,6 +2222,12 @@
       st[j + 1] = sd.s[j];
       n = j + 2;
     }
+    return EDTTS_OK;
+  }
+  int after_head() {
+    if (!side || n < 2) return EDTTS_OK;
+    HIP_TRY(hipEventRecord(side->head, st[0]));
+    for (int j = 1; j < n; ++j) HIP_TRY(hipStreamWaitEvent(st[j], side->head, 0));
     return EDTTS_OK;
   }
   ~ForkJoin() {
@@ -2237,6 +2294,7 @@
   } else {
     a->x0 = t.x0;
     a->c_s1m = t.coef[0]; a->c_sab = t.coef[1]; a->c_sabp = t.coef[2]; a->c_dir = t.coef[3];
+    a->c_rinv = 1.0 / (double)t.coef[1];
   }
 }
 template <class F>
@@ -2296,12 +2354,18 @@
   return a;
 }
 
+struct Boundary {
+  bool skip_prologue = false;
+  int parity = 0;
+  const float* cond_next = nullptr;
+};
 template <int ES>
 struct ForwardArgs {
   KArgs a;
   const CallCtx& c;
   size_t qk_set, v_set;
-  ForwardArgs(const CallCtx& c_, const float* x, const float* cond_row, int cond_bstride) : c(c_) {
+  int parity;
+  ForwardArgs(const CallCtx& c_, const float* x, const float* cond_row, int cond_bstride, int parity_ = 0) : c(c_), parity(parity_ & 1) {
     const Layout& lo = c.lo;
     const float* blob = c.blob;
     memset(&a, 0, sizeof(a));
@@ -2324,7 +2388,7 @@
     a.t_len = c.ln.t; a.s_len = c.ln.s; a.t_dbl = c.ln.t_dbl;
     qk_set = (size_t)c.B * c.ws.Tp * lo.H / ES;
     v_set = (size_t)c.B * c.ws.VR * c.ws.Tp / ES;
-    set_qkv(1, 0);
+    set_qkv(parity ^ 1, parity);
     a.n1w = blob + lo.layer[0].n1w; a.stream = blob + lo.inp; a.layer = 0;
   }
   void set_qkv(int in_set, int out_set) {
@@ -2336,7 +2400,7 @@
     const Layout& lo = c.lo;
     const LayerLayout& y = lo.layer[l];
     a.layer = l;
-    set_qkv(l & 1, (l + 1) & 1);
+    set_qkv((l + parity) & 1, (l + parity + 1) & 1);
     a.proj_b = c.blob + y.proj_b; a.n2w = c.blob + y.n2w; a.n3w = c.blob + y.n3w; a.up_b = c.blob + y.up_b;
     a.down_b = c.blob + y.down_b; a.stream = c.blob + y.s_body;
     a.kc = c.wsb + c.ws.kc + (size_t)l * c.B * c.ws.Sp * lo.H / ES;
@@ -2404,32 +2468,54 @@
     }
     return (co == 22 && !HAS_CO22) ? 0 : co;
   }
+  static bool fuses(const CallCtx& c) {
+    if constexpr (HAS_COOP) return coop_choice(c.B, c.ws.Tp) == 0;
+    return true;
+  }
   template <int COW = 0>
-  static int forward(const CallCtx& c, const float* x, const float* cond_row, int cond_bstride, const StepTail& tail) {
+  static int forward(const CallCtx& c, const float* x, const float* cond_row, int cond_bstride, const StepTail& tail, const Boundary& bd = Boundary()) {
+    const bool fused = bd.skip_prologue || bd.cond_next != nullptr || bd.parity != 0;
     if constexpr (HAS_COOP && COW == 0) {
       const int co = coop_choice(c.B, c.ws.Tp);
+      if (co != 0 && fused) return fail(EDTTS_ERR_UNSUPPORTED, "internal: fused step boundary on a cooperative instance");
       if (co == 14) return Launcher<Small>::template forward<4>(c, x, cond_row, cond_bstride, tail);
       if (co == 24) return forward<4>(c, x, cond_row, cond_bstride, tail);
       if constexpr (HAS_CO22) {
         if (co == 22) return forward<2>(c, x, cond_row, cond_bstride, tail);
       }
     }
+    if (COW != 0 && fused) return fail(EDTTS_ERR_UNSUPPORTED, "internal: fused step boundary on a cooperative instance");
+    if (bd.cond_next && tail.kind != TAIL_DDIM && tail.kind != TAIL_DDPM) return fail(EDTTS_ERR_UNSUPPORTED, "internal: fused step boundary behind tail kind %d", tail.kind);
     if constexpr (HAS_SMALL && COW == 0) {
       if (2 * c.B * (c.ws.Tp / C::WF) <= wave_slots())
-        return Launcher<Small>::template forward<0>(c, x, cond_row, cond_bstride, tail);
-    }
-    ForwardArgs<1> f(c, x, cond_row, cond_bstride);
+        return Launcher<Small>::template forward<0>(c, x, cond_row, cond_bstride, tail, bd);
+    }
+    ForwardArgs<1> f(c, x, cond_row, cond_bstride, bd.parity);
     const KArgs& a = f.a;
     const hipStream_t st = c.st;
     const int g = grid(c.B, c.ws.Tp);
     if constexpr (COW != 0) {
       hipLaunchKernelGGL((k_prologue_co<C, COW>), dim3(c.B * (c.ws.Tp / C::WF)), dim3(64 * COW), C::HT * C::NF * 1024, st, a);
-    } else {
+      LAUNCH_CHECK("k_prologue");
+    } else if (!bd.skip_prologue) {
       hipLaunchKernelGGL(k_prologue<C>, dim3(g), dim3(C::THREADS), ring_lds(), st, a);
-    }
-    LAUNCH_CHECK("k_prologue");
+      LAUNCH_CHECK("k_prologue");
+    }
     for (int l = 0; l < c.lo.L; ++l) {
-      TRY_G(with_tail(f.layer(l, tail), [&](auto t) -> int {
+      const int kind = f.layer(l, tail);
+      if constexpr (COW == 0) {
+        if (l + 1 == c.lo.L && bd.cond_next) {
+          f.a.cond_next = bd.cond_next; f.a.stream_next = c.blob + c.lo.inp; f.a.n1w = c.blob + c.lo.layer[0].n1w;
+          if (kind == TAIL_DDIM) {
+            PROF_LAUNCH(st, hipLaunchKernelGGL((k_layer<C, TAIL_DDIM_NEXT>), dim3(g), dim3(C::THREADS), layer_lds(), st, a));
+          } else {
+            PROF_LAUNCH(st, hipLaunchKernelGGL((k_layer<C, TAIL_DDPM_NEXT>), dim3(g), dim3(C::THREADS), layer_lds(), st, a));
+          }
+          LAUNCH_CHECK("k_layer");
+          continue;
+        }
+      }
+      TRY_G(with_tail(kind, [&](auto t) -> int {
         constexpr int TL = decltype(t)::value;
         if constexpr (COW != 0) {
           using CO = Coop<C, COW>;
@@ -2449,6 +2535,8 @@
     if constexpr (HAS_SMALL) TRY_G(Launcher<Small>::set_attrs());
     const int lds = (int)layer_lds();
     HIP_TRY(hipFuncSetAttribute((const void*)k_prologue<C>, hipFuncAttributeMaxDynamicSharedMemorySize, (int)ring_lds()));
+    HIP_TRY(hipFuncSetAttribute((const void*)k_layer<C, TAIL_DDIM_NEXT>, hipFuncAttributeMaxDynamicSharedMemorySize, lds));
+    HIP_TRY(hipFuncSetAttribute((const void*)k_layer<C, TAIL_DDPM_NEXT>, hipFuncAttributeMaxDynamicSharedMemorySize, lds));
     return for_each_tail([&](auto t) -> int {
       constexpr int TL = decltype(t)::value;
       HIP_TRY(hipFuncSetAttribute((const void*)k_layer<C, TL>, hipFuncAttributeMaxDynamicSharedMemorySize, lds));
@@ -2620,6 +2708,21 @@
   return EDTTS_OK;
 }
 
+template <class LN, class = void>
+struct LauncherFuses : std::false_type {};
+template <class LN>
+struct LauncherFuses<LN, std::void_t<decltype(&LN::fuses)>> : std::true_type {};
+template <class LN>
+static bool launcher_fuses(const CallCtx& c) {
+  if constexpr (LauncherFuses<LN>::value) return LN::fuses(c);
+  else return false;
+}
+template <class LN>
+static int launcher_forward(const CallCtx& c, const float* x, const float* cond_row, const StepTail& tail, const Boundary& bd) {
+  if constexpr (LauncherFuses<LN>::value) return LN::forward(c, x, cond_row, 0, tail, bd);
+  else return LN::forward(c, x, cond_row, 0, tail);
+}
+
 struct SamplerInputs {
   const int64_t* t_dev = nullptr;
   const int64_t* t_host = nullptr;
@@ -2637,27 +2740,38 @@
   float* wsb = (float*)workspace;
   SubBatches sb;
   plan_call(lo, B, T, S, num_steps, wsb, &sb);
-  TRY(launch_len_check(in.ln.t_dbl ? nullptr : in.ln.t, in.ln.s, B, T, S, wsb, st));
-  TRY(launch_cond(lo, blob, in.t_dev, nullptr, in.t_host, num_steps, wsb + sb.cond, wsb, st));
   const size_t row = (size_t)lo.L * 2 * 2 * lo.H;
   const size_t per_utt = (size_t)T * lo.MEL;
   ForkJoin fj;
   TRY(fj.init(sb, st));
   auto call = [&](int j) { return CallCtx{lo, blob, sb.ws[j], wsb + sb.base[j], sb.B[j], T, S, dims->window, in.ln.at(sb.off[j]), fj.st[j]}; };
+  const bool fuse_on = current_settings().fuse_boundary != 0;
   EDTTS_DISPATCH(lo, {
     TRY(set_attrs_once<LN>());
-    for (int j = 0; j < sb.n; ++j) {
+    for (int j = sb.n - 1; j >= 0; --j) {
       const size_t off = sb.off[j];
       TRY(LN::ctx(call(j), (in.sem_features || !in.sem_idx) ? nullptr : in.sem_idx + off * S,
                   in.sem_features ? in.sem_features + off * S * lo.SD : nullptr));
     }
+    TRY(launch_len_check(in.ln.t_dbl ? nullptr : in.ln.t, in.ln.s, B, T, S, wsb, st));
+    TRY(launch_cond(lo, blob, in.t_dev, nullptr, in.t_host, num_steps, wsb + sb.cond, wsb, st));
+    TRY(fj.after_head());
+    bool fuse[kMaxSub];
+    for (int j = 0; j < sb.n; ++j) fuse[j] = fuse_on && launcher_fuses<LN>(call(j));
     for (int i = 0; i < num_steps; ++i)
       for (int j = 0; j < sb.n; ++j) {
         const size_t o = (size_t)sb.off[j] * per_utt;
 #ifdef EDTTS_WAVELOG
         g_wavelog_base = sb.off[j] * (sb.ws[j].Tp / 32);
 #endif
-        TRY(LN::forward(call(j), (i == 0 ? in.x_T : in.x) + o, wsb + sb.cond + i * row, 0, tail_of(i, sb.off[j], o)));
+        const StepTail tail = tail_of(i, sb.off[j], o);
+        Boundary bd;
+        if (fuse[j] && (tail.kind == TAIL_DDIM || tail.kind == TAIL_DDPM)) {
+          bd.skip_prologue = i > 0;
+          bd.parity = (i * lo.L) & 1;
+          if (i + 1 < num_steps) bd.cond_next = wsb + sb.cond + (size_t)(i + 1) * row;
+        }
+        TRY(launcher_forward<LN>(call(j), (i == 0 ? in.x_T : in.x) + o, wsb + sb.cond + i * row, tail, bd));
       }
   });
   return EDTTS_OK;
@@ -3624,6 +3738,8 @@
   return g_coop.load();
 }
 
+int edtts_set_fuse_boundary(int on) { return g_fuse_boundary.exchange(on != 0); }
+
 int edtts_set_substreams(int n) {
   if (n >= 1 && n <= kMaxSub) return g_substreams.exchange(n);
   return g_substreams.load();
diff --git a/edge-diffusion-tts_amd/edge_diffusion_tts_amd/native.py b/edge-diffusion-tts_amd/edge_diffusion_tts_amd/native.py
--- a/edge-diffusion-tts_amd/edge_diffusion_tts_amd/native.py
+++ b/edge-diffusion-tts_amd/edge_diffusion_tts_amd/native.py
@@ -14,7 +14,7 @@
     "edtts_layer_slot_name", "edtts_packed_bytes", "edtts_pack_weights", "edtts_workspace_bytes", "edtts_decoder_forward",
     "edtts_ddim_step", "edtts_ddpm_step", "edtts_generate", "edtts_sample_ddpm", "edtts_sample_multistep", "edtts_dsconv_forward", "edtts_profile_enable",
     "edtts_profile_collect", "edtts_randn", "edtts_index_errors", "edtts_sample_inpaint",
-    "edtts_mel_to_spec", "edtts_griffin_lim_scratch_floats", "edtts_griffin_lim", "edtts_set_substreams", "edtts_set_coop", "edtts_dsconv_scratch_floats", "edtts_substreams_for",
+    "edtts_mel_to_spec", "edtts_griffin_lim_scratch_floats", "edtts_griffin_lim", "edtts_set_substreams", "edtts_set_coop", "edtts_set_fuse_boundary", "edtts_dsconv_scratch_floats", "edtts_substreams_for",
     "edtts_decoder_forward_len", "edtts_generate_len", "edtts_sample_ddpm_len", "edtts_sample_multistep_len",
     "edtts_sample_inpaint_len", "edtts_randn_rows", "edtts_sample_inpaint_multistep_len",
     "edtts_sem_packed_bytes", "edtts_sem_num_codes", "edtts_sem_pack", "edtts_sem_encode", "edtts_sem_decode", "edtts_sem_stats",
@@ -217,12 +217,14 @@
     L.edtts_set_substreams.restype = i32
     L.edtts_set_coop.argtypes = [i32]
     L.edtts_set_coop.restype = i32
+    L.edtts_set_fuse_boundary.argtypes = [i32]
+    L.edtts_set_fuse_boundary.restype = i32
     L.edtts_substreams_for.argtypes = [C.POINTER(EdttsDims), i32, i32]
     L.edtts_substreams_for.restype = i32
     L.edtts_profile_collect.argtypes = [C.POINTER(C.c_double), C.POINTER(i32)]
     for name in EXPORTED_SYMBOLS:
         fn = getattr(L, name)
-        if fn.restype is C.c_int and name not in ("edtts_version", "edtts_num_global_slots", "edtts_num_layer_slots", "edtts_set_substreams", "edtts_set_coop", "edtts_substreams_for",
+        if fn.restype is C.c_int and name not in ("edtts_version", "edtts_num_global_slots", "edtts_num_layer_slots", "edtts_set_substreams", "edtts_set_coop", "edtts_set_fuse_boundary", "edtts_substreams_for",
                                                   "edtts_train_dw_slab_rows", "edtts_optim_chunk_size"):
             fn.errcheck = _errcheck
     _lib = L
@@ -885,6 +887,10 @@
     return int(lib().edtts_set_coop(int(mode)))
 
 
+def set_fuse_boundary(on: bool) -> int:
+    return int(lib().edtts_set_fuse_boundary(int(bool(on))))
+
+
 def profile_enable(max_records: int) -> None:
     lib().edtts_profile_enable(int(max_records))
 
diff --git a/include/edtts.h b/include/edtts.h
--- a/include/edtts.h
+++ b/include/edtts.h
@@ -178,6 +178,8 @@
 int edtts_substreams_for(const EdttsDims* dims, int B, int T);
 
 int edtts_set_coop(int mode);
+
+int edtts_set_fuse_boundary(int on);
 
 enum { EDTTS_SEM_FSQ = 0, EDTTS_SEM_VQ = 1 };
 typedef struct EdttsSemDims {
```
